# fawnliu/TRIS

Measured on AMD Instinct MI355X. Metric: Stage-1 training images/sec @320px bs48 (TRIS clip-RN50, 3 negatives), higher is better.
Workload: dtype f32 storage/accumulate; products h2 = 2 x f16 pieces; 1 GPU; Stage-1 train step, RefCOCOg-shaped synthetic batch: 48 img/GPU 320x320, 20-token query + 3 negative queries per image, clip-RN50 trunk + frozen aux CLIP ViT-B/32, AdamW (BASELINE.json configs[2]/[3]); per_gpu_batch=48, global_batch=48, size=320, query_len=20, negative_samples=3, parallelism=dp1, sync_bn=False

## Files before the change

### include/tris_hip.h

```cpp
#ifndef TRIS_HIP_H
#define TRIS_HIP_H

#ifdef __cplusplus
extern "C" {
#endif

int tris_gemm_f32(const float* A, const float* B, float* C, int M, int N, int K, long lda, long ldb, long ldc,
                  int transA, int transB, int batch, long strideA, long strideB, long strideC, const float* bias,
                  int bias_mode, const float* resid, long ldr, long strideR, int act, float alpha, float* workspace,
                  long workspace_bytes, void* stream);

int tris_gemm_epilogue_next(float* pre_out, const float* dact_x);

int tris_splitk_tickets_next(int* tickets, int count);
long tris_splitk_fused_launches(void);

int tris_set_gemm_mode(int mode);
int tris_set_gemm_mode_thread(int mode);
int tris_set_option(const char* name, const char* value);
int tris_set_conv_direct_thread(int value);

int tris_set_autotune(int on);
int tris_get_autotune(void);
int tris_get_gemm_mode(void);
// ... 41 lines not shown
int tris_amax_next(unsigned* out);
int tris_h2_next(const unsigned* amaxA, const unsigned* amaxB, float scaleA, float scaleB);
int tris_bn_mask_next(unsigned char* mask);
int tris_h2_planes_f32(const float* x, float* planes_out, long n, const unsigned* word, void* stream);
int tris_h2_planes_segments_f32(const float* base, const long* offs, const long* sizes, const long* slot_index, int nseg,
                                const unsigned* slots, float* out_base, void* stream);
int tris_h2_planes_t_segments_f32(const float* base, const long* offs, const long* rows, const long* cols, const long* slot_index,
                                  int nseg, const unsigned* slots, float* out_base, void* stream);
int tris_h2_unplanes_f32(const float* planes, float* out, long n, const unsigned* word, void* stream);
int tris_h2_next_planes(const unsigned* amaxA, const unsigned* amaxB, int flags);
int tris_bn_apply_pl_f32(const float* X, const float* mean, const float* invstd, const float* gamma, const float* beta,
                         const float* resid, int resid_kind, const unsigned* resid_word, float* Ypl, const unsigned* out_word, long M,
                         int C, int relu, void* stream);
int tris_bn_bwd_reduce_pl_f32(const float* dY, const float* Ypl, const float* X, const float* mean, const float* invstd, long M, int C,
                              float* sum_dz, float* sum_dzx, float* workspace, float* dz_out, void* stream);
int tris_bn_apply_pool_pl_f32(const float* X, const float* mean, const float* invstd, const float* gamma, const float* beta,
                              float* Ypl, const unsigned* out_word, int B, int H, int W, int C, void* stream);
int tris_avgpool2_fwd_pl_f32(const float* Xpl, float* Ypl, const unsigned* word, int B, int H, int W, int C, void* stream);
int tris_bn_bwd_apply_pl_f32(const float* dY, const float* Ypl, const float* X, const float* mean, const float* invstd,
                             const float* gamma, const float* sum_dz, const float* sum_dzx, float inv_count, float* dXpl,
                             const unsigned* out_word, float* dZ, long M, int C, const float* beta_mask, void* stream);
int tris_bn_bwd_apply_pool_pl_f32(const float* dYp, const float* X, const float* mean, const float* invstd, const float* gamma,
                                  const float* beta, const float* sum_dz, const float* sum_dzx, float inv_count, float* dXpl,
                                  const unsigned* out_word, int B, int H, int W, int C, void* stream);
int tris_bn_out_bound2_f32(const float* gamma, const float* beta, int C, float xhat_max, const unsigned* add_word, unsigned* out,
                           void* stream);
int tris_bn_finalize_bound_f32(const double* part, int rows, long M, int C, float eps, float momentum, float* stats,
                               float* running_mean, float* running_var, const float* gamma, const float* beta, float xhat_max,
                               const unsigned* add_word, unsigned* bound_out, void* stream);
int tris_part_finalize_bound_f32(const double* part, int rows, int C, float* out0, float* out1, const float* gamma, const float* invstd,
                                 float inv_count, float xhat_max, const unsigned* dz_word, unsigned* bound_out, void* stream);
int tris_bn_bwd_bound_f32(const float* gamma, const float* invstd, const float* sum_dz, const float* sum_dzx, int C, float inv_count,
                          float xhat_max, const unsigned* dz_word, unsigned* out, void* stream);
int tris_bn_out_bound_f32(const float* gamma, const float* beta, int C, float xhat_max, unsigned* out, void* stream);
int tris_bn_bwd_reduce_f32(const float* dY, const float* Y, const float* X, const float* mean, const float* invstd,
                           long M, int C, float* sum_dz, float* sum_dzx, float* workspace, const float* gamma_mask,
                           const float* beta_mask, float* dz_out, void* stream);
int tris_bn_bwd_apply_f32(const float* dY, const float* Y, const float* X, const float* mean, const float* invstd,
                          const float* gamma, const float* sum_dz, const float* sum_dzx, float inv_count, float* dX,
                          float* dZ, long M, int C, const float* beta_mask, void* stream);
int tris_colsum_f32(const float* X, long M, int N, long ld, float* out, float* workspace, void* stream);

int tris_instnorm_fwd_f32(const float* X, const float* gamma, const float* beta, float* Y, float* mean, float* invstd,
                          int B, int P, int C, float eps, int relu, void* stream);
int tris_instnorm_bwd_f32(const float* dY, const float* Y, const float* X, const float* gamma, const float* mean,
                          const float* invstd, float* dX, float* dgamma_part , float* dbeta_part ,
                          int B, int P, int C, int relu, void* stream);

int tris_layernorm_fwd_f32(const float* X, const float* gamma, const float* beta, float* Y, float* mean, float* rstd,
                           long rows, int W, float eps, void* stream);
long tris_layernorm_bwd_workspace_bytes(long rows, int W);
int tris_layernorm_bwd_f32(const float* dY, const float* X, const float* gamma, const float* mean, const float* rstd,
                           float* dX, float* dgamma, float* dbeta, long rows, int W, float* workspace, const float* extra , void* stream);

int tris_bn_apply_pool_f32(const float* X, const float* mean, const float* invstd, const float* gamma, const float* beta,
                           float* Yp, int B, int H, int W, int C, void* stream);
int tris_bn_bwd_reduce_pool_f32(const float* dYp, const float* X, const float* mean, const float* invstd, int B, int H, int W,
                                int C, float* sum_dz, float* sum_dzx, float* workspace, const float* gamma, const float* beta,
                                void* stream);
int tris_bn_bwd_apply_pool_f32(const float* dYp, const float* X, const float* mean, const float* invstd, const float* gamma,
                               const float* beta, const float* sum_dz, const float* sum_dzx, float inv_count, float* dX, int B,
                               int H, int W, int C, void* stream);
int tris_avgpool2_fwd_f32(const float* X, float* Y, int B, int H, int W, int C, void* stream);
int tris_avgpool2_bwd_f32(const float* dY, float* dX, int B, int H, int W, int C, void* stream);
#define TRIS_EW_ADD 0
#define TRIS_EW_AXPY 1
#define TRIS_EW_RELU_BWD 2
#define TRIS_EW_QGELU 3
#define TRIS_EW_QGELU_BWD 4
#define TRIS_EW_MUL 5
#define TRIS_EW_SCALE 6
#define TRIS_EW_RELU 7
int tris_elementwise_f32(int op, const float* A, const float* B, float* O, long n, float s, void* stream);
int tris_elementwise_bcast_f32(int op, const float* A, const float* B, float* O, long n, long nb, float s, void* stream);
int tris_scale_exp_fwd_f32(const float* X, const float* ls, float* O, float* e_out, long n, void* stream);
long tris_scale_exp_workspace_bytes(void);
int tris_scale_exp_bwd_f32(const float* dO, const float* O, const float* ls, float* dX, float* dls, float* workspace, long n,
                           void* stream);
int tris_nchw_to_nhwc_f32(const float* X, float* Y, int B, int C, int H, int W, void* stream);

int tris_mha_fwd_f32(const float* qkv, float* out, int N, int L, int W, int heads, int causal, void* stream);
int tris_mha_bwd_f32(const float* qkv, const float* dout, float* dqkv, int N, int L, int W, int heads, int causal,
                     void* stream);
int tris_mha_mfma_fwd_f32(const float* qkv, float* out, float* lse, int N, int L, int W, int heads, int causal,
                          void* stream);
int tris_mha_mfma_bwd_f32(const float* qkv, const float* out, const float* dout, const float* lse, float* delta,
                          float* dqkv, int N, int L, int W, int heads, int causal, void* stream);
int tris_mha_h2_fwd_f32(const float* qkv, float* out, float* lse, const unsigned* amax_qkv, int N, int L, int W, int heads,
                        int causal, void* stream);
int tris_mha_h2_bwd_f32(const float* qkv, const float* out, const float* dout, const float* lse, float* delta, float* dqkv,
                        const unsigned* amax_qkv, const unsigned* amax_dout, int N, int L, int W, int heads, int causal,
                        void* stream);
int tris_text_pack_plan_i64(const long* ids, int N, int L, int* plan, void* stream);
int tris_embed_packed_fwd_f32(const long* ids, const float* tok, const float* pos, const int* plan, float* out, int N, int L, int W,
                              void* stream);
int tris_mha_packed_fwd_f32(const float* qkv, float* out, const int* plan, int N, int Lmax, int W, int heads, int causal, void* stream);
int tris_eot_gather_packed_f32(const float* x, const int* plan, float* out, int N, int W, void* stream);
int tris_rows_limit_thread(const int* limit);
int tris_embed_fwd_f32(const long* ids, const float* tok, const float* pos, float* out, int N, int L, int W,
                       void* stream);
int tris_embed_bwd_f32(const long* ids, const float* dout, float* dtok, float* dpos, int N, int L, int W, void* stream);
int tris_embed_rows_bwd_f32(const long* ids, const float* rows, float* dtok, int R, int W, float scale, void* stream);
int tris_concat_i64(const long* a, long na, const long* b, long nb, long* out, void* stream);
int tris_eot_gather_fwd_f32(const long* ids, const float* x, float* out, int N, int L, int W, void* stream);
int tris_eot_gather_bwd_f32(const long* ids, const float* dout, float* dx, int N, int L, int W, void* stream);

int tris_l2norm_fwd_f32(const float* X, float* Y, float* inv_norm, long rows, int C, void* stream);
int tris_l2norm_bwd_f32(const float* dY, const float* Y, const float* inv_norm, float* dX, long rows, int C,
                        void* stream);
int tris_softmax_fwd_f32(const float* X, float* Y, long rows, int n, float scale, void* stream);
int tris_softmax_bwd_f32(const float* dY, const float* Y, float* dX, long rows, int n, float scale, void* stream);
int tris_xattn_fwd_f32(const float* Qv, const float* Kv, const float* Vv, const float* Qt, const float* Kt,
                       const float* Vt, float* new_vis, float* new_lan, float* probs, int B, int P, int N, int C,
                       void* stream);
#define TRIS_DECLINED (-2)
long tris_xattn_fused_ws_bytes(int B, int N, int C);
long tris_xattn_fused_sync_words(int B);
int tris_xattn_fused_fwd_f32(const float* Qv, const float* Kv, const float* Vv, const float* Qt, const float* Kt,
                             const float* Vt, float* new_vis, float* new_lan, float* probs, int B, int P, int N, int C,
                             float* ws, long ws_bytes, unsigned* sync, void* stream);
long tris_xattn_px_ws_bytes(int B, int N, int C);
long tris_xattn_px_sync_words(int B);
long tris_xattn_px_bwd_ws_bytes(int B, int N, int C);
int tris_xattn_px_bwd_f32(const float* d_vis, const float* d_lan, const float* Vv, const float* Qt, const float* Kt,
                          const float* Vt, const float* probs, float* dQv, float* dKv, float* dVv, float* dS, int B, int P,
                          int N, int C, float* ws, long ws_bytes, unsigned* sync, unsigned* amax_dQv, unsigned* amax_dKv,
                          unsigned* amax_dVv, void* stream);
long tris_xattn_px_last_form(void);
int tris_xattn_amax_next(const unsigned* qv, const unsigned* kv, const unsigned* vv, const unsigned* qt, const unsigned* kt,
                         const unsigned* vt);
long tris_xattn_px_slots(int B, int P, int C, int cus);
int tris_xattn_px_fwd_f32(const float* Qv, const float* Kv, const float* Vv, const float* Qt, const float* Kt,
                          const float* Vt, float* new_vis, float* new_lan, float* probs, int B, int P, int N, int C,
                          float* ws, long ws_bytes, unsigned* sync, void* stream);
int tris_softmax_col_bwd_f32(const float* dY, const float* Y, float* dX, int B, int P, int N, float scale,
                             void* stream);
int tris_cls_head_fwd_f32(const float* score, float* cls_out, float* cls_fg, int B, int P, int N, float focal_p,
                          float focal_c, void* stream);
int tris_cls_head_bwd_f32(const float* score, const float* g_cls_out, float* dscore, int B, int P, int N, float focal_p,
                          float focal_c, void* stream);
int tris_maps_fwd_f32(const float* score, float* relu_map, float* sig_map, int B, int h, int w, int N, int S,
                      void* stream);
int tris_maps_bwd_f32(const float* score, const float* d_relu, const float* d_sig, float* dscore, int B, int h, int w,
                      int N, int S, void* stream);
int tris_resize_bilinear_fwd_f32(const float* X, float* Y, int planes, int Hi, int Wi, int Ho, int Wo,
// ... 120 lines not shown
```

### tris_amd/CLIP/clip/model.py

```python
from collections import OrderedDict


import numpy as np
import torch
from torch import nn

from ... import ops
from ...config import cfg


class Conv2d(nn.Module):

    def __init__(self, cin, cout, k, stride=1, bias=False):
        super().__init__()
        self.cin, self.cout, self.k, self.stride = cin, cout, k, stride
        w = torch.empty(cout, cin, k, k).contiguous(memory_format=torch.channels_last)
        nn.init.kaiming_uniform_(w, a=5 ** 0.5)
        self.weight = nn.Parameter(w)
        self.bias = nn.Parameter(torch.zeros(cout)) if bias else None

    def forward(self, x, stats=False, grad_box=None, grad_box_out=None):
        if self.k == 1:
            return ops.linear(x, self.weight, self.bias, stats=stats and self.bias is None, grad_box=grad_box,
                              grad_box_out=grad_box_out)
# ... 171 lines not shown
                hooks[stage]()
        return tuple(outs)

    def forward(self, x):
        outs = [ops.unplanes(o).permute(0, 3, 1, 2) for o in self.forward_cl(x)]
        outs.append(None)
        return tuple(outs)


class LayerNorm(nn.Module):
    def __init__(self, w, eps=1e-5):
        super().__init__()
        self.eps = eps
        self.weight = nn.Parameter(torch.ones(w))
        self.bias = nn.Parameter(torch.zeros(w))

    def forward(self, x, grad_box=None):
        return ops.layer_norm(x, self.weight, self.bias, self.eps, grad_box)


class QuickGELU(nn.Module):
    def forward(self, x):
        return ops.quick_gelu(x)


class MultiheadAttention(nn.Module):

    def __init__(self, d_model, n_head):
        super().__init__()
        self.embed_dim, self.num_heads = d_model, n_head
        self.in_proj_weight = nn.Parameter(torch.empty(3 * d_model, d_model))
        self.in_proj_bias = nn.Parameter(torch.zeros(3 * d_model))
        self.out_proj = Linear(d_model, d_model)
        nn.init.xavier_uniform_(self.in_proj_weight)


class ResidualAttentionBlock(nn.Module):
    def __init__(self, d_model, n_head, attn_mask=None):
        super().__init__()
        self.attn = MultiheadAttention(d_model, n_head)
        self.ln_1 = LayerNorm(d_model)
        self.mlp = nn.Sequential(OrderedDict([
            ("c_fc", Linear(d_model, d_model * 4)),
            ("gelu", QuickGELU()),
            ("c_proj", Linear(d_model * 4, d_model)),
        ]))
        self.ln_2 = LayerNorm(d_model)
        self.causal = attn_mask is not None

    def forward(self, x):
        use_box = torch.is_grad_enabled() and x.requires_grad and cfg.grad_box
        b1 = ops.GradBox() if use_box else None
        b2 = ops.GradBox() if use_box else None
        h = self.ln_1(x, b1)
        qkv = ops.linear(h, self.attn.in_proj_weight, self.attn.in_proj_bias)
        a = ops.mha(qkv, self.attn.num_heads, self.causal)
        x = self.attn.out_proj(a, resid=x, grad_box_res=b1)
        h = self.ln_2(x, b2)
        if torch.is_grad_enabled() and cfg.mlp_fuse:
            f = ops.linear_qgelu(h, self.mlp.c_fc.weight, self.mlp.c_fc.bias)
            return ops.linear(f, self.mlp.c_proj.weight, self.mlp.c_proj.bias, x, 0, grad_box_res=b2, act_link=True)
        if torch.is_grad_enabled():
            return self.mlp.c_proj(self.mlp.gelu(self.mlp.c_fc(h)), resid=x, grad_box_res=b2)
        f = self.mlp.c_fc(h, act=2)
        return self.mlp.c_proj(f, resid=x, grad_box_res=b2)


    def forward_packed(self, x, plan, N, L):
        h = self.ln_1(x)
        qkv = ops.linear(h, self.attn.in_proj_weight, self.attn.in_proj_bias)
        a = ops.mha_packed(qkv, plan, N, L, self.attn.num_heads, self.causal)
        x = self.attn.out_proj(a, resid=x)
        h = self.ln_2(x)
        return self.mlp.c_proj(self.mlp.c_fc(h, act=2), resid=x)

    def forward_token0(self, x):
        h = self.ln_1(x)
        qkv = ops.linear(h, self.attn.in_proj_weight, self.attn.in_proj_bias)
        a = ops.token0(ops.mha(qkv, self.attn.num_heads, self.causal))
        x0 = self.attn.out_proj(a, resid=ops.token0(x))
        h = self.ln_2(x0)
        if torch.is_grad_enabled() and cfg.mlp_fuse:
            f = ops.linear_qgelu(h, self.mlp.c_fc.weight, self.mlp.c_fc.bias)
            return ops.linear(f, self.mlp.c_proj.weight, self.mlp.c_proj.bias, x0, 0, act_link=True)
        if torch.is_grad_enabled():
            return self.mlp.c_proj(self.mlp.gelu(self.mlp.c_fc(h)), resid=x0)
        return self.mlp.c_proj(self.mlp.c_fc(h, act=2), resid=x0)


class Transformer(nn.Module):
    def __init__(self, width, layers, heads, attn_mask=None):
        super().__init__()
        self.width, self.layers = width, layers
        self.resblocks = nn.Sequential(*[ResidualAttentionBlock(width, heads, attn_mask) for _ in range(layers)])

    def forward(self, x):
        for blk in self.resblocks:
            x = ops.cut(blk(x))
        return x

    def forward_token0(self, x):
        blocks = list(self.resblocks)
        for blk in blocks[:-1]:
            x = ops.cut(blk(x))
        return blocks[-1].forward_token0(x)


class VisionTransformer(nn.Module):
    def __init__(self, input_resolution, patch_size, width, layers, heads, output_dim):
        super().__init__()
        self.input_resolution, self.output_dim, self.patch_size = input_resolution, output_dim, patch_size
        self.conv1 = nn.Module()
        self.conv1.weight = nn.Parameter(torch.randn(width, 3, patch_size, patch_size) * 0.02)
        scale = width ** -0.5
        self.class_embedding = nn.Parameter(scale * torch.randn(width))
        self.positional_embedding = nn.Parameter(scale * torch.randn((input_resolution // patch_size) ** 2 + 1, width))
        self.ln_pre = LayerNorm(width)
        self.transformer = Transformer(width, layers, heads)
        for blk in self.transformer.resblocks:
            for w in (blk.attn.in_proj_weight, blk.attn.out_proj.weight, blk.mlp.c_fc.weight, blk.mlp.c_proj.weight):
                w._tris_linear_w = True
        self.ln_post = LayerNorm(width)
        self.proj = nn.Parameter(scale * torch.randn(width, output_dim))
        self.spacial_dim = 7
        self.class_embedding._tris_accumulates = True
        self.positional_embedding._tris_accumulates = True

    def forward_patches(self, patches):
        emb = ops.linear(patches, self.conv1.weight)
        x = ops.vit_assemble(emb, self.class_embedding, self.positional_embedding)
        x = self.ln_pre(x)
        if cfg.vit_token0:
            cls = self.ln_post(self.transformer.forward_token0(x))
        else:
# ... 166 lines not shown
```

### tris_amd/_lib.py

```python
import ctypes
import os
import re

import torch

_HERE = os.path.dirname(os.path.abspath(__file__))
_ROOT = os.path.dirname(_HERE)
HEADER = os.path.join(_ROOT, "include", "tris_hip.h")
LIBPATH = os.environ.get("TRIS_HIP_LIB") or os.path.join(_HERE, "libtris_hip.so")

_CT = {
    "int": ctypes.c_int,
    "long": ctypes.c_long,
    "float": ctypes.c_float,
}


def parse_header(path=HEADER):
    src = open(path).read()
    consts = {m.group(1): int(m.group(2)) for m in re.finditer(r"#define\s+(TRIS_\w+)\s+(\d+)", src)}
    src = re.sub(r"/\*.*?\*/", " ", src, flags=re.S)
    decls = {}
    for m in re.finditer(r"\b(int|long)\s+(tris_\w+)\s*\(([^)]*)\)\s*;", src):
        ret, name, args = m.group(1), m.group(2), m.group(3)
        types = []
        for a in args.split(","):
            a = a.strip()
            if a in ("", "void"):
                continue
            if "*" in a:
                types.append(ctypes.c_void_p)
            else:
                base = a.split()[0] if a.split()[0] != "const" else a.split()[1]
                types.append(_CT[base])
        decls[name] = (_CT[ret], types)
    return decls, consts


DECLS, CONSTS = parse_header()
_lib = None


class TrisHipError(RuntimeError):
    pass


def load():
    global _lib
    if _lib is None:
        if not os.path.exists(LIBPATH):
            raise TrisHipError(
                f"{LIBPATH} not found: build it with `python -c 'import __graft_entry__ as g; g.build()'` "
                "(tris_amd has no CPU or eager fallback by design)")
        lib = ctypes.CDLL(LIBPATH)
        for name, (ret, args) in DECLS.items():
            fn = getattr(lib, name)
            fn.restype = ret
            fn.argtypes = args
        _lib = lib
    return _lib


_FN = {}


def call(name, *args):
    fn = _FN.get(name)
    if fn is None:
        fn = _FN[name] = getattr(load(), name)
    err = fn(*args)
    if err != 0:
        raise TrisHipError(f"{name} failed with hipError_t {err}")


def query(name, *args):
    return getattr(load(), name)(*args)
```

### tris_amd/config.py

```python
import contextlib
import os


def _flag(name, default):
    v = os.environ.get(name)
    return default if v is None or v == "" else v != "0"


class _Config:
    def __setattr__(self, name, value):
        if name == "step_graph" and "step_graph" in self.__dict__:
            self.__dict__["step_graph_chosen"] = True
        self.__dict__[name] = value

    def __init__(self):
        e = os.environ.get
        self.step_graph = e("TRIS_STEP_GRAPH", "0")
        self.step_graph_chosen = "TRIS_STEP_GRAPH" in os.environ
        self.hipgraph = _flag("TRIS_HIPGRAPH", True)
        self.text_stream = _flag("TRIS_TEXT_STREAM", True)
        self.wgrad_stream = _flag("TRIS_WGRAD_STREAM", True)
        self.stream_probe = _flag("TRIS_STREAM_PROBE", True)
        self.stream_probe_log = e("TRIS_STREAM_PROBE_LOG") == "1"
        self.text_at = e("TRIS_TEXT_AT", "layer4")
        self.bn_bwd_fuse = _flag("TRIS_BN_BWD_FUSE", True)
        self.bn_pool = _flag("TRIS_BN_POOL", True)
        self.grad_box = _flag("TRIS_GRAD_BOX", True)
        self.mlp_fuse = _flag("TRIS_MLP_FUSE", True)
        self.mha = e("TRIS_MHA", "auto")
        self.mha_h2 = _flag("TRIS_MHA_H2", True)
        self.ddp_seg_opt = _flag("TRIS_DDP_SEG_OPT", True)
        self.ddp_seg_poison = _flag("TRIS_DDP_SEG_POISON", False)
        self.syncbn_bound = _flag("TRIS_SYNCBN_BOUND", True)
        self.xattn_fused = _flag("TRIS_XATTN_FUSED", True)
        self.xattn_px = _flag("TRIS_XATTN_PX", True)
        self.xattn_h2 = _flag("TRIS_XATTN_H2", True)
        self.xattn_bwd_px = _flag("TRIS_XATTN_BWD_PX", True)
        self.hbm_loader = _flag("TRIS_HBM_LOADER", True)
        self.eval_group = max(1, int(e("TRIS_EVAL_GROUP", "16")))
        self.mbox_spin = int(e("TRIS_MBOX_SPIN", "40000000"))
        self.syncbn_comm = e("TRIS_SYNCBN_COMM", "mailbox")
        self.ddp_check = e("TRIS_DDP_CHECK") == "1"
        self.ddp_sparse_embed = _flag("TRIS_DDP_SPARSE_EMBED", True)
        self.random_init = e("TRIS_RANDOM_INIT") == "1"
        self.h2_planes = _flag("TRIS_H2_PLANES", True)
        self.own_stream = _flag("TRIS_OWN_STREAM", True)
        self.fuse_splitk = _flag("TRIS_FUSE_SPLITK_PY", False)
        self.aux_text_early = _flag("TRIS_AUX_TEXT_EARLY", True)
        self.text_pack = _flag("TRIS_TEXT_PACK", True)
        self.bn_bitmask = _flag("TRIS_BN_BITMASK", True)
        self.gemm_convert = int(e("TRIS_GEMM_CONVERT", "0"))
        self.step_graph_rerecord = int(e("TRIS_STEP_GRAPH_RERECORD", "3"))
        self.side_param_grads = _flag("TRIS_SIDE_PARAM_GRADS", True)
        self.vit_token0 = _flag("TRIS_VIT_TOKEN0", True)

    @contextlib.contextmanager
    def override(self, **kw):
        old = {k: getattr(self, k) for k in kw}
        try:
            for k, v in kw.items():
                setattr(self, k, v)
            yield self
        finally:
            for k, v in old.items():
                setattr(self, k, v)

    def key(self):
        return tuple(sorted((k, v) for k, v in self.__dict__.items() if k not in ("step_graph_chosen", "step_graph_rerecord")))


cfg = _Config()
```

### tris_amd/csrc/attn_h2.hip

```cpp
#include "common.h"
#include "tris_hip.h"
#include "x3_split.h"

namespace {

#include "amax.h"

constexpr int HD = 64;
constexpr int RS = 144;
constexpr int PLB = 64 * RS;
constexpr float PS = 8192.f;

typedef float f4v __attribute__((ext_vector_type(4)));
typedef short s16x4 __attribute__((ext_vector_type(4)));
typedef short s16x8 __attribute__((ext_vector_type(8)));
typedef unsigned u32x4v __attribute__((ext_vector_type(4)));

struct H8 { f16x8 hi, lo; };

__device__ __forceinline__ float4 ldg4(const float* p) { return *reinterpret_cast<const float4*>(p); }
__device__ __forceinline__ H8 split8(const float4 u, const float4 w, const float s) {
  const Split4 p = split4h(u, s), q = split4h(w, s);
  H8 o;
  o.hi = __builtin_bit_cast(f16x8, (u32x4v){p.hi.x, p.hi.y, q.hi.x, q.hi.y});
// ... 92 lines not shown
            const int key = key0 + 8 * kg + i;
            const float v = (sc[i >> 2][i & 3] + sx[i >> 2][i & 3] * (1.0f / 2048.0f)) * inv_s;
            sv[i] = (full || (key < L && !(causal && key > q0 + r))) ? v : -INFINITY;
            mx = fmaxf(mx, sv[i]);
          }
          mx = fmaxf(mx, __shfl_xor(mx, 16, 64));
          mx = fmaxf(mx, __shfl_xor(mx, 32, 64));
          const float mn = fmaxf(m, mx);
          float p[8], rs = 0.f;
#pragma unroll
          for (int i = 0; i < 8; ++i) { p[i] = mn == -INFINITY ? 0.f : __expf(sv[i] - mn); rs += p[i]; }
          rs += __shfl_xor(rs, 16, 64);
          rs += __shfl_xor(rs, 32, 64);
          const float alpha = mn == -INFINITY ? 1.f : __expf(m - mn);
          l = l * alpha + rs;
          m = mn;
          if (__builtin_amdgcn_ballot_w64(alpha != 1.f) != 0ull) {
#pragma unroll
            for (int t = 0; t < 4; ++t) {
              const float ar = __shfl(alpha, 4 * kg + t, 64);
#pragma unroll
              for (int j = 0; j < 4; ++j) { oc[j][t] *= ar; ox[j][t] *= ar; }
            }
          }
          const H8 pf = split8(make_float4(p[0], p[1], p[2], p[3]), make_float4(p[4], p[5], p[6], p[7]), PS);
#pragma unroll
          for (int ct = 0; ct < 4; ++ct) mm3(pf, bfrag(Vp, 32 * pr, ct, r, kg), oc[ct], ox[ct]);
        }
      }
    }
  }
  unsigned am = 0u;
  if (q0 < L) {
    const float linv = 1.f / l;
    float* ob = out + (long)n * L * W + h * HD;
#pragma unroll
    for (int t = 0; t < 4; ++t) {
      const float li = __shfl(linv, 4 * kg + t, 64) * inv_o;
      const int q = q0 + 4 * kg + t;
      if (q < L) {
#pragma unroll
        for (int j = 0; j < 4; ++j) {
          const float o = (oc[j][t] + ox[j][t] * (1.0f / 2048.0f)) * li;
          ob[(long)q * W + 16 * j + r] = o;
          am = max(am, __builtin_bit_cast(unsigned, o) & 0x7fffffffu);
        }
      }
    }
    if (kg == 0 && q0 + r < L) lse[((long)n * H + h) * L + q0 + r] = m + __logf(l);
  }
  if (amax != nullptr) amax_commit(am, amax);
}

__global__ __launch_bounds__(256) void mha_h2_dq_kernel(const float* __restrict__ qkv, const float* __restrict__ out,
                                                        const float* __restrict__ dout, const float* __restrict__ lse,
                                                        float* __restrict__ delta, float* __restrict__ dqkv, int L, int W, int causal,
                                                        float scale, const unsigned* __restrict__ am_qkv,
                                                        const unsigned* __restrict__ am_do, unsigned* __restrict__ amax) {
  __shared__ __attribute__((aligned(16))) char Kp[2 * PLB];
  __shared__ __attribute__((aligned(16))) char Vp[2 * PLB];
  const int tid = threadIdx.x, lane = tid & 63, wave = tid >> 6, r = lane & 15, kg = lane >> 4;
  const int h = blockIdx.y, n = blockIdx.z, H = gridDim.y;
  const int qb = blockIdx.x * 64, q0 = qb + wave * 16;
  const float s = h2_scale_from_bits(h2_amax_of(am_qkv, lane)), sg = h2_scale_from_bits(h2_amax_of(am_do, lane));
  const float inv_s = scale / (s * s), inv_p = 1.0f / (s * sg);
  const float* base = qkv + (long)n * L * 3 * W + h * HD;
  const int qrow = min(q0 + r, L - 1);
  H8 qf[2], gf[2];
  resident(qf, base + (long)qrow * 3 * W + 8 * kg, s);
  float dl = 0.f;
  {
    const float* gp = dout + ((long)n * L + qrow) * W + h * HD + 8 * kg;
    const float* op = out + ((long)n * L + qrow) * W + h * HD + 8 * kg;
#pragma unroll
    for (int ks = 0; ks < 2; ++ks) {
      const float4 g0 = ldg4(gp + 32 * ks), g1 = ldg4(gp + 32 * ks + 4), o0 = ldg4(op + 32 * ks), o1 = ldg4(op + 32 * ks + 4);
      gf[ks] = split8(g0, g1, sg);
      dl += g0.x * o0.x + g0.y * o0.y + g0.z * o0.z + g0.w * o0.w + g1.x * o1.x + g1.y * o1.y + g1.z * o1.z + g1.w * o1.w;
    }
    dl += __shfl_xor(dl, 16, 64);
    dl += __shfl_xor(dl, 32, 64);
    if (kg == 0 && q0 + r < L) delta[((long)n * H + h) * L + q0 + r] = dl;
  }
  const float ls = lse[((long)n * H + h) * L + qrow];
  f4v acc[4];
#pragma unroll
  for (int j = 0; j < 4; ++j) acc[j] = (f4v){0.f, 0.f, 0.f, 0.f};
  const int kend = causal ? min(L, qb + 64) : L;
  for (int kb = 0; kb < kend; kb += 64) {
    __syncthreads();
    stage64(Kp, base + W, 3L * W, kb, L, tid, s);
    stage64(Vp, base + 2 * W, 3L * W, kb, L, tid, s);
    __syncthreads();
    if (q0 < L) {
#pragma unroll
      for (int pr = 0; pr < 2; ++pr) {
        const int key0 = kb + 32 * pr;
        if (key0 < kend && !(causal && key0 > q0 + 15)) {
          f4v sc[2], sx[2], pc[2], px[2];
#pragma unroll
          for (int j = 0; j < 2; ++j) {
            sc[j] = sx[j] = pc[j] = px[j] = (f4v){0.f, 0.f, 0.f, 0.f};
            const int row = 32 * pr + trow(r, j);
#pragma unroll
            for (int ks = 0; ks < 2; ++ks) {
              mm3(afrag(Kp, row, ks, kg), qf[ks], sc[j], sx[j]);
              mm3(afrag(Vp, row, ks, kg), gf[ks], pc[j], px[j]);
            }
          }
          float ds[8], mx = 0.f;
          const bool full = key0 + 32 <= L && !(causal && key0 + 31 > q0);
#pragma unroll
          for (int i = 0; i < 8; ++i) {
            const int key = key0 + 8 * kg + i;
            const bool ok = full || (key < L && !(causal && key > q0 + r));
            const float sv = (sc[i >> 2][i & 3] + sx[i >> 2][i & 3] * (1.0f / 2048.0f)) * inv_s;
            const float dp = (pc[i >> 2][i & 3] + px[i >> 2][i & 3] * (1.0f / 2048.0f)) * inv_p;
            ds[i] = ok ? __expf(sv - ls) * (dp - dl) * scale : 0.f;
            mx = fmaxf(mx, fabsf(ds[i]));
          }
          const float sd = wave_scale_of(mx);
          const H8 df = split8(make_float4(ds[0], ds[1], ds[2], ds[3]), make_float4(ds[4], ds[5], ds[6], ds[7]), sd);
          const float inv_d = 1.0f / (sd * s);
#pragma unroll
          for (int ct = 0; ct < 4; ++ct) {
            f4v tc = {0.f, 0.f, 0.f, 0.f}, tx = {0.f, 0.f, 0.f, 0.f};
            mm3(df, bfrag(Kp, 32 * pr, ct, r, kg), tc, tx);
            acc[ct] += join(tc, tx) * inv_d;
          }
        }
      }
    }
  }
  unsigned am = 0u;
  if (q0 < L) {
    float* ob = dqkv + (long)n * L * 3 * W + h * HD;
#pragma unroll
    for (int t = 0; t < 4; ++t) {
      const int q = q0 + 4 * kg + t;
      if (q < L) {
#pragma unroll
        for (int j = 0; j < 4; ++j) {
          ob[(long)q * 3 * W + 16 * j + r] = acc[j][t];
          am = max(am, __builtin_bit_cast(unsigned, acc[j][t]) & 0x7fffffffu);
        }
      }
    }
  }
  if (amax != nullptr) amax_commit(am, amax);
}

__global__ __launch_bounds__(256) void mha_h2_dkv_kernel(const float* __restrict__ qkv, const float* __restrict__ dout,
                                                         const float* __restrict__ lse, const float* __restrict__ delta,
                                                         float* __restrict__ dqkv, int L, int W, int causal, float scale,
                                                         const unsigned* __restrict__ am_qkv, const unsigned* __restrict__ am_do,
                                                         unsigned* __restrict__ amax) {
  __shared__ __attribute__((aligned(16))) char Qp[2 * PLB];
  __shared__ __attribute__((aligned(16))) char Gp[2 * PLB];
  __shared__ float Ls[64], Ds[64];
  const int tid = threadIdx.x, lane = tid & 63, wave = tid >> 6, r = lane & 15, kg = lane >> 4;
  const int h = blockIdx.y, n = blockIdx.z, H = gridDim.y;
  const int kb0 = blockIdx.x * 64, k0 = kb0 + wave * 16;
  const float s = h2_scale_from_bits(h2_amax_of(am_qkv, lane)), sg = h2_scale_from_bits(h2_amax_of(am_do, lane));
  const float inv_s = scale / (s * s), inv_p = 1.0f / (s * sg), inv_v = 1.0f / (PS * sg);
  const float* base = qkv + (long)n * L * 3 * W + h * HD;
  const int krow = min(k0 + r, L - 1);
  H8 kf[2], vf[2];
  resident(kf, base + W + (long)krow * 3 * W + 8 * kg, s);
  resident(vf, base + 2 * W + (long)krow * 3 * W + 8 * kg, s);
  f4v dk[4], vc[4], vx[4];
#pragma unroll
  for (int j = 0; j < 4; ++j) dk[j] = vc[j] = vx[j] = (f4v){0.f, 0.f, 0.f, 0.f};
  const int qstart = causal ? kb0 : 0;
  for (int qb = qstart; qb < L; qb += 64) {
    __syncthreads();
    stage64(Qp, base, 3L * W, qb, L, tid, s);
    stage64(Gp, dout + (long)n * L * W + h * HD, (long)W, qb, L, tid, sg);
    if (tid < 64) {
      const int q = min(qb + tid, L - 1);
      Ls[tid] = lse[((long)n * H + h) * L + q];
      Ds[tid] = delta[((long)n * H + h) * L + q];
    }
    __syncthreads();
    if (k0 < L) {
#pragma unroll
      for (int pr = 0; pr < 2; ++pr) {
        const int qs0 = qb + 32 * pr;
        if (qs0 < L && !(causal && qs0 + 31 < k0)) {
          f4v sc[2], sx[2], pc[2], px[2];
#pragma unroll
          for (int j = 0; j < 2; ++j) {
            sc[j] = sx[j] = pc[j] = px[j] = (f4v){0.f, 0.f, 0.f, 0.f};
            const int row = 32 * pr + trow(r, j);
#pragma unroll
            for (int ks = 0; ks < 2; ++ks) {
              mm3(afrag(Qp, row, ks, kg), kf[ks], sc[j], sx[j]);
              mm3(afrag(Gp, row, ks, kg), vf[ks], pc[j], px[j]);
            }
          }
          float p[8], ds[8], mx = 0.f;
          const bool full = qs0 + 32 <= L && !(causal && k0 + 15 > qs0);
#pragma unroll
          for (int i = 0; i < 8; ++i) {
            const int ql = 32 * pr + 8 * kg + i, q = qb + ql;
            const bool ok = full || (q < L && !(causal && k0 + r > q));
            const float sv = (sc[i >> 2][i & 3] + sx[i >> 2][i & 3] * (1.0f / 2048.0f)) * inv_s;
            const float dp = (pc[i >> 2][i & 3] + px[i >> 2][i & 3] * (1.0f / 2048.0f)) * inv_p;
            p[i] = ok ? __expf(sv - Ls[ql]) : 0.f;
            ds[i] = p[i] * (dp - Ds[ql]) * scale;
            mx = fmaxf(mx, fabsf(ds[i]));
          }
          const float sd = wave_scale_of(mx);
          const H8 pf = split8(make_float4(p[0], p[1], p[2], p[3]), make_float4(p[4], p[5], p[6], p[7]), PS);
          const H8 df = split8(make_float4(ds[0], ds[1], ds[2], ds[3]), make_float4(ds[4], ds[5], ds[6], ds[7]), sd);
          const float inv_d = 1.0f / (sd * s);
#pragma unroll
          for (int ct = 0; ct < 4; ++ct) {
            mm3(pf, bfrag(Gp, 32 * pr, ct, r, kg), vc[ct], vx[ct]);
            f4v tc = {0.f, 0.f, 0.f, 0.f}, tx = {0.f, 0.f, 0.f, 0.f};
            mm3(df, bfrag(Qp, 32 * pr, ct, r, kg), tc, tx);
            dk[ct] += join(tc, tx) * inv_d;
          }
        }
      }
    }
  }
  unsigned am = 0u;
  if (k0 < L) {
    float* ob = dqkv + (long)n * L * 3 * W + h * HD;
#pragma unroll
    for (int t = 0; t < 4; ++t) {
      const int k = k0 + 4 * kg + t;
      if (k < L) {
#pragma unroll
        for (int j = 0; j < 4; ++j) {
          const float dv = (vc[j][t] + vx[j][t] * (1.0f / 2048.0f)) * inv_v;
          ob[(long)k * 3 * W + W + 16 * j + r] = dk[j][t];
          ob[(long)k * 3 * W + 2 * W + 16 * j + r] = dv;
          am = max(am, max(__builtin_bit_cast(unsigned, dk[j][t]) & 0x7fffffffu, __builtin_bit_cast(unsigned, dv) & 0x7fffffffu));
        }
      }
    }
  }
  if (amax != nullptr) amax_commit(am, amax);
}

}

extern "C" __attribute__((visibility("hidden"))) unsigned* tris_internal_take_amax_next();

extern "C" int tris_mha_h2_fwd_f32(const float* qkv, float* out, float* lse, const unsigned* amax_qkv, int N, int L, int W, int heads,
                                   int causal, void* stream) {
  if (W != heads * HD || L < 1 || N < 1 || (((uintptr_t)qkv) & 15) || amax_qkv == nullptr) return (int)hipErrorInvalidValue;
  hipLaunchKernelGGL(mha_h2_fwd_kernel, dim3(cdiv(L, 64), heads, N), dim3(256), 0, (hipStream_t)stream, qkv, out, lse, L, W, causal,
                     1.0f / sqrtf((float)HD), amax_qkv, tris_internal_take_amax_next());
  TRIS_LAUNCH_CHECK();
  return 0;
}

extern "C" int tris_mha_h2_bwd_f32(const float* qkv, const float* out, const float* dout, const float* lse, float* delta, float* dqkv,
                                   const unsigned* amax_qkv, const unsigned* amax_dout, int N, int L, int W, int heads, int causal,
                                   void* stream) {
  if (W != heads * HD || L < 1 || N < 1 || amax_qkv == nullptr || amax_dout == nullptr || (((uintptr_t)qkv) & 15) ||
      (((uintptr_t)dout) & 15) || (((uintptr_t)out) & 15))
    return (int)hipErrorInvalidValue;
  const float scale = 1.0f / sqrtf((float)HD);
  const dim3 grid(cdiv(L, 64), heads, N);
  unsigned* amax = tris_internal_take_amax_next();
  hipLaunchKernelGGL(mha_h2_dq_kernel, grid, dim3(256), 0, (hipStream_t)stream, qkv, out, dout, lse, delta, dqkv, L, W, causal, scale,
                     amax_qkv, amax_dout, amax);
  TRIS_LAUNCH_CHECK();
  hipLaunchKernelGGL(mha_h2_dkv_kernel, grid, dim3(256), 0, (hipStream_t)stream, qkv, dout, lse, delta, dqkv, L, W, causal, scale,
                     amax_qkv, amax_dout, amax);
  TRIS_LAUNCH_CHECK();
  return 0;
}
```

### tris_amd/csrc/conv_direct.hip

```cpp
#include <algorithm>
#include <cstdlib>
#include <cstring>

#include "common.h"
#include "tris_hip.h"

namespace {

#include "gemm_params.h"
#include "gemm_fast.h"
#include "conv_direct_cfg.h"

__global__ __launch_bounds__(256) void stem_conv1_kernel(const float* __restrict__ X, const float* __restrict__ Wt,
                                                         float* __restrict__ Y, double* __restrict__ stat_part, int Bn, int H,
                                                         int W, int Cin, int Cout, int Ho, int Wo, int stride, int tiles_per_wave) {
  __shared__ double red[4][2][32];
  const int lane = threadIdx.x & 63, wave = threadIdx.x >> 6;
  const int mn = lane & 31, kh = lane >> 5;
  const int K = 9 * Cin;
  const long total = (long)Bn * Ho * Wo;
  float wreg[14];
  int ky[14], kx[14], kc[14];
#pragma unroll
  for (int s = 0; s < 14; ++s) {
    const int k = 2 * s + kh;
    const int tap = k / Cin;
    wreg[s] = (k < K && mn < Cout) ? Wt[mn * K + k] : 0.f;
    ky[s] = k < K ? tap / 3 : -100000;
    kx[s] = tap - (tap / 3) * 3;
    kc[s] = k - tap * Cin;
  }
  double s1 = 0.0, s2 = 0.0;
  const long tile0 = ((long)blockIdx.x * 4 + wave) * tiles_per_wave;
  for (int t = 0; t < tiles_per_wave; ++t) {
    const long p0 = (tile0 + t) * 32;
    if (p0 >= total) break;
    const long p = min(p0 + mn, total - 1);
    const int b = (int)(p / ((long)Ho * Wo));
    const int r = (int)(p - (long)b * Ho * Wo);
    const int oy = r / Wo, ox = r - oy * Wo;
    const int iy0 = oy * stride - 1, ix0 = ox * stride - 1;
    float a[14];
#pragma unroll
    for (int s = 0; s < 14; ++s) {
      const int iy = iy0 + ky[s], ix = ix0 + kx[s];
      const bool inb = (unsigned)iy < (unsigned)H && (unsigned)ix < (unsigned)W;
      a[s] = inb ? X[(((long)b * H + iy) * W + ix) * Cin + kc[s]] : 0.f;
    }
    f32x16 acc;
#pragma unroll
    for (int q = 0; q < 16; ++q) acc[q] = 0.f;
#pragma unroll
    for (int s = 0; s < 14; ++s) acc = __builtin_amdgcn_mfma_f32_32x32x2f32(a[s], wreg[s], acc, 0, 0, 0);
#pragma unroll
    for (int q = 0; q < 16; ++q) {
      const long pix = p0 + (q & 3) + 8 * (q >> 2) + 4 * kh;
      if (pix < total && mn < Cout) {
        const float v = acc[q];
// ... 345 lines not shown
```

### tris_amd/csrc/gemm_conv.hip

```cpp
#include <algorithm>
#include <cstdlib>
#include <cstring>
#include <map>
#include <mutex>
#include <tuple>

#include "common.h"
#include "tris_hip.h"

extern "C" {
extern __attribute__((visibility("hidden"))) int tris_internal_stream_form;
extern __attribute__((visibility("hidden"))) int tris_internal_col_blocks;
extern __attribute__((visibility("hidden"))) int tris_internal_ln_bwd_blocks;
extern __attribute__((visibility("hidden"))) int tris_internal_fin_block;
__attribute__((visibility("hidden"))) int tris_internal_reduce_wide = 4;
__attribute__((visibility("hidden"))) int tris_internal_xcd_order = -1;
__attribute__((visibility("hidden"))) int tris_internal_red_grid = 0;
__attribute__((visibility("hidden"))) int tris_internal_fuse_splitk = 16;
__attribute__((visibility("hidden"))) long tris_internal_fused_count = 0;
extern __attribute__((visibility("hidden"))) int tris_internal_xattn_px_slots;
}

namespace {

#include "gemm_params.h"

static int stream_nt(const GemmParams& p, int batch) {
  if (!tris_internal_stream_form) return 0;
  const long streams = 1 + (p.resid ? 1 : 0) + (p.bnb_x ? 1 : 0) + (p.bnb_y ? 1 : 0);
  return (long)p.M * p.N * 4 * batch * streams > ((long)tris_internal_stream_form << 20) ? 1 : 0;
}

struct Options {
  int force_tile = 0;
  int force_pipe = -1;
  int pipe_default = -1;
  int conv_direct = -1;
  int wgrad_direct = -1;
  int bn_fold = 1;
  int stem_conv1 = 1;
  int wg_blocks = 256;
  char tune_log[256] = {0};
};
static int parse_tile(const char* e) {
  return !e ? 0 : (!strcmp(e, "128x128") ? 1 : !strcmp(e, "128x64") ? 2 : !strcmp(e, "64x64") ? 3 : !strcmp(e, "128x32") ? 4
                   : !strcmp(e, "256x128") ? 5 : 0);
}
static bool set_option(Options& o, const char* name, const char* v) {
  const bool unset = (v == nullptr || v[0] == 0);
  if (!strcmp(name, "FORCE_TILE")) o.force_tile = parse_tile(v);
  else if (!strcmp(name, "FORCE_PIPE")) o.force_pipe = unset ? -1 : std::min(5, std::max(0, atoi(v)));
  else if (!strcmp(name, "PIPE")) o.pipe_default = unset ? -1 : (v[0] == '0' ? 0 : 1);
  else if (!strcmp(name, "CONV_DIRECT")) o.conv_direct = unset ? -1 : atoi(v);
  else if (!strcmp(name, "WGRAD_DIRECT")) o.wgrad_direct = unset ? -1 : atoi(v);
  else if (!strcmp(name, "BN_FOLD")) o.bn_fold = unset ? 1 : (v[0] != '0');
  else if (!strcmp(name, "STEM_CONV1")) o.stem_conv1 = unset ? 1 : (v[0] != '0');
  else if (!strcmp(name, "WG_BLOCKS")) o.wg_blocks = unset ? 256 : std::max(1, atoi(v));
  else if (!strcmp(name, "STREAM_FORM")) tris_internal_stream_form = unset ? 256 : (atoi(v) == 1 ? 256 : std::max(0, atoi(v)));
  else if (!strcmp(name, "COL_BLOCKS")) tris_internal_col_blocks = unset ? 512 : std::max(1, atoi(v));
  else if (!strcmp(name, "LN_BWD_BLOCKS")) tris_internal_ln_bwd_blocks = unset ? 512 : std::min(512, std::max(1, atoi(v)));
  else if (!strcmp(name, "FIN_BLOCK")) tris_internal_fin_block = unset ? 256 : (atoi(v) >= 1024 ? 1024 : atoi(v) >= 512 ? 512 : 256);
  else if (!strcmp(name, "REDUCE_WIDE")) tris_internal_reduce_wide = unset ? 4 : std::max(0, atoi(v));
  else if (!strcmp(name, "RED_GRID")) tris_internal_red_grid = unset ? 0 : std::max(0, atoi(v));
  else if (!strcmp(name, "XCD_ORDER")) tris_internal_xcd_order = unset ? -1 : std::min(2, std::max(0, atoi(v)));
  else if (!strcmp(name, "FUSE_SPLITK")) tris_internal_fuse_splitk = unset ? TRIS_FUSE_SPLITK_DEFAULT : std::max(0, atoi(v));
  else if (!strcmp(name, "XATTN_PX_SLOTS")) tris_internal_xattn_px_slots = unset ? 0 : std::max(0, atoi(v));
  else if (!strcmp(name, "TUNE_LOG")) { strncpy(o.tune_log, unset ? "" : v, sizeof(o.tune_log) - 1); o.tune_log[sizeof(o.tune_log) - 1] = 0; }
  else return false;
  return true;
}
static Options init_options() {
  Options o;
  for (const char* n : {"FORCE_TILE", "FORCE_PIPE", "PIPE", "CONV_DIRECT", "WGRAD_DIRECT", "BN_FOLD", "STEM_CONV1", "WG_BLOCKS", "STREAM_FORM", "COL_BLOCKS", "XATTN_PX_SLOTS", "LN_BWD_BLOCKS", "FIN_BLOCK", "REDUCE_WIDE", "XCD_ORDER", "FUSE_SPLITK", "RED_GRID", "TUNE_LOG"}) {
    char env[64];
    snprintf(env, sizeof(env), "TRIS_%s", n);
    if (const char* v = getenv(env)) set_option(o, n, v);
  }
  return o;
}
static Options g_opt = init_options();

static int g_mode_default = 1;
static thread_local int g_mode_thread = -1;
#define g_gemm_mode (g_mode_thread >= 0 ? g_mode_thread : g_mode_default)
static inline bool mode_h2() { return g_gemm_mode == 3 || g_gemm_mode == 4; }

}
extern "C" __attribute__((visibility("hidden"))) unsigned* tris_internal_take_amax_next();
#define TRIS_RUN_DECL(AK_, BK_)                                                                                                   \
  extern "C" __attribute__((visibility("hidden"))) int tris_internal_run_cfg_##AK_##BK_(const void* params, int batch, float* ws, \
                                                                                         void* stream, const void* cfg, int mode);
TRIS_RUN_DECL(0, 0) TRIS_RUN_DECL(0, 1) TRIS_RUN_DECL(1, 0) TRIS_RUN_DECL(1, 1) TRIS_RUN_DECL(2, 0) TRIS_RUN_DECL(2, 2) TRIS_RUN_DECL(1, 3)
#undef TRIS_RUN_DECL
namespace {
template <int AK, int BKIND>
int run_cfg(const GemmParams& p0, int batch, float* ws, hipStream_t st, const Cfg& cfg) {
  const int mode = g_gemm_mode;
  GemmParams p = p0;
  p.nt = stream_nt(p, batch);
  if (AK == A_ROWK && BKIND == B_NK) return tris_internal_run_cfg_00(&p, batch, ws, st, &cfg, mode);
  if (AK == A_ROWK && BKIND == B_KN) return tris_internal_run_cfg_01(&p, batch, ws, st, &cfg, mode);
  if (AK == A_COLK && BKIND == B_NK) return tris_internal_run_cfg_10(&p, batch, ws, st, &cfg, mode);
  if (AK == A_COLK && BKIND == B_KN) return tris_internal_run_cfg_11(&p, batch, ws, st, &cfg, mode);
  if (AK == A_IM2COL && BKIND == B_NK) return tris_internal_run_cfg_20(&p, batch, ws, st, &cfg, mode);
  if (AK == A_IM2COL && BKIND == B_KN_DGRAD) return tris_internal_run_cfg_22(&p, batch, ws, st, &cfg, mode);
  if (AK == A_COLK && BKIND == B_KN_IM2COL) return tris_internal_run_cfg_13(&p, batch, ws, st, &cfg, mode);
  return (int)hipErrorInvalidValue;
}

struct H2Next { const unsigned* a; const unsigned* b; float sa, sb; bool armed; bool planes; int flags; };
static thread_local H2Next g_h2_next = {nullptr, nullptr, 0.f, 0.f, false, false, 0};
static H2Next h2_take() {
  H2Next n = g_h2_next;
  g_h2_next.armed = false;
  return n;
}
struct H2Guard {
  int saved;
  bool on;
  bool bad;
  H2Guard(GemmParams& p, const H2Next& n) : saved(g_mode_thread), on(false), bad(false) {
    if (!n.armed) return;
    if (!gemm_fast_ok(p)) { bad = n.planes; return; }
    p.h2_amaxA = n.a; p.h2_amaxB = n.b; p.h2_sA = n.sa; p.h2_sB = n.sb;
    g_mode_thread = n.planes ? 4 : 3;
    p.bnb_y_pl = (n.planes && (n.flags & 4)) ? 2 : (n.planes && (n.flags & 1)) ? 1 : 0;
// ... 6 lines not shown
static int default_pipe(const GemmParams& p, int bm, int bn, int splitk) {
  if (!pipe_ok(p) || bn == 32) return 0;
  if (g_opt.force_pipe >= 0) return g_opt.force_pipe;
  if (g_opt.pipe_default >= 0) return g_opt.pipe_default;
  if (mode_h2()) return 0;
  return p.gC >= 128 ? 1 : 0;
}

static Cfg heuristic_cfg(const GemmParams& p, int batch, const float* ws, long ws_bytes) {
  const bool can_split = (batch == 1 && ws != nullptr && p.K >= 512);
  int bm = 64, bn = 64, splitk = 1;
  if (p.stat_part != nullptr) {
    bm = 128;
    bn = p.N <= 32 ? 32 : p.N <= 64 ? 64 : 128;
  } else if (can_split && p.K >= 4096) {
    if (p.N <= 64) { bn = 64; bm = p.M >= 128 ? 128 : 64; }
    else if (p.M >= 128 && p.N >= 128) { bm = bn = 128; }
    const long tiles = (long)cdiv(p.M, bm) * cdiv(p.N, bn);
    splitk = (int)min((long)cdiv(512, tiles), (long)(p.K / 256));
    const long per = (long)p.M * p.N * (long)sizeof(float);
    if ((long)splitk * per > ws_bytes) splitk = (int)(ws_bytes / per);
    if (splitk < 2) splitk = 1;
  } else {
    static const int cand[4][2] = {{128, 128}, {128, 64}, {64, 64}, {128, 32}};
    static const double pen[4] = {1.0, 1.08, 1.2, 1.15};
    const bool fastk = gemm_fast_ok(p);
    double best = 1e30;
    for (int c = 0; c < 4; ++c) {
      const int cbm = cand[c][0], cbn = cand[c][1];
      if (c != 2 && p.M < 96) continue;
      if (c == 0 && p.N <= 64) continue;
      if (c == 3 && !(p.N <= 32 && fastk)) continue;
      const long tiles = (long)cdiv(p.M, cbm) * cdiv(p.N, cbn) * batch;
      const double per_k32 = (cbm / 64) * (cbn / 64.0) * (g_gemm_mode == 1 ? 384.0 + 250.0 : mode_h2() ? 192.0 + 200.0 : 1024.0) * pen[c];
      const int smax = can_split ? (int)min((long)64, (long)(p.K / 256)) : 1;
      for (int sk = 1; sk <= smax; sk = (sk < 4 ? sk + 1 : sk + sk / 2)) {
        if (sk > 1 && (long)sk * p.M * p.N * (long)sizeof(float) > ws_bytes) break;
        const double ksteps = (double)cdiv(cdiv(p.K, sk), 32);
        const double blocks = (double)tiles * sk;
        double t = (ksteps * per_k32 + 3000.0) * (blocks <= 256.0 ? 1.0 : blocks / 256.0);
        if (sk > 1) t += 14000.0 + 2.0 * sk * (double)p.M * p.N * 4.0 / 2000.0;
        if (t < best) { best = t; bm = cbm; bn = cbn; splitk = sk; }
      }
    }
  }
  {
    const int forced = g_opt.force_tile;
    if (forced == 1 && p.N > 64) { bm = 128; bn = 128; }
    if (forced == 2) { bm = 128; bn = 64; }
    if (forced == 3) { bm = 64; bn = 64; }
    if (forced == 4 && p.N <= 32) { bm = 128; bn = 32; }
    if (forced == 5 && p.N > 64 && p.M >= 256 && p.stat_part == nullptr) { bm = 256; bn = 128; }
  }
  Cfg c = {bm, bn, splitk, default_pipe(p, bm, bn, splitk)};
  return c;
}

struct TuneKey {
  int ak, bk, M, N, K, batch, mode;
  bool operator<(const TuneKey& o) const {
    return std::tie(ak, bk, M, N, K, batch, mode) < std::tie(o.ak, o.bk, o.M, o.N, o.K, o.batch, o.mode);
  }
};
static std::map<TuneKey, Cfg> g_tuned;
static std::mutex g_tune_mu;

static int g_autotune = -1;
static bool autotune_enabled() {
  if (g_autotune < 0) { const char* e = getenv("TRIS_AUTOTUNE"); g_autotune = (e && e[0] == '0') ? 0 : 1; }
  return g_autotune == 1;
}

template <int AK, int BKIND>
int launch_cfg(GemmParams& p, int batch, float* ws, long ws_bytes, hipStream_t st) {
  Cfg h = heuristic_cfg(p, batch, ws, ws_bytes);
  if (!autotune_enabled() || g_opt.force_tile) return run_cfg<AK, BKIND>(p, batch, ws, st, h);
  const bool stat = p.stat_part != nullptr;
  const TuneKey key = {AK, BKIND + (stat ? 16 : 0) + (p.bnb_x != nullptr ? 32 : 0), p.M, p.N, p.K, batch, g_gemm_mode};
  {
    std::lock_guard<std::mutex> lk(g_tune_mu);
    auto it = g_tuned.find(key);
    if (it != g_tuned.end()) return run_cfg<AK, BKIND>(p, batch, ws, st, it->second);
  }
  hipStreamCaptureStatus cap = hipStreamCaptureStatusNone;
  if (hipStreamIsCapturing(st, &cap) != hipSuccess || cap != hipStreamCaptureStatusNone)
    return run_cfg<AK, BKIND>(p, batch, ws, st, h);
  static const int tiles[5][2] = {{128, 128}, {128, 64}, {64, 64}, {128, 32}, {256, 128}};
  const bool fastk = gemm_fast_ok(p);
  static const int sks[] = {1, 2, 3, 4, 6, 8, 12, 16, 24, 32, 48, 64, 96, 128};
  const bool can_split = (batch == 1 && ws != nullptr && p.K >= 512) && !stat;
  const bool can_pipe = pipe_ok(p) && g_opt.force_pipe != 0;
  hipEvent_t e0, e1;
  if (hipEventCreate(&e0) != hipSuccess || hipEventCreate(&e1) != hipSuccess) return run_cfg<AK, BKIND>(p, batch, ws, st, h);
  (void)hipDeviceSynchronize();
  Cfg best = h;
  float best_ms = 1e30f;
  auto time_cfg = [&](Cfg c) -> float {
    float ms_min = 1e30f;
    for (int rep = 0; rep < 2; ++rep) {
      (void)hipEventRecord(e0, st);
      if (run_cfg<AK, BKIND>(p, batch, ws, st, c) != 0) return 1e30f;
      (void)hipEventRecord(e1, st);
      if (hipEventSynchronize(e1) != hipSuccess) return 1e30f;
      float ms = 1e30f;
      (void)hipEventElapsedTime(&ms, e0, e1);
      ms_min = ms < ms_min ? ms : ms_min;
    }
    return ms_min;
  };
  for (int t = 0; t < 5; ++t) {
    const int cbm = tiles[t][0], cbn = tiles[t][1];
    if (t != 2 && p.M < 96) continue;
    if ((t == 0 || t == 4) && p.N <= 64) continue;
    if (t == 3 && !(p.N <= 32 && fastk)) continue;
    if (t == 4 && (!can_pipe || p.M < 256)) continue;
    if (stat && cbm != 128) continue;
    const long ntiles = (long)cdiv(p.M, cbm) * cdiv(p.N, cbn) * batch;
    for (int sk : sks) {
      if (sk > 1 && (!can_split || sk > p.K / 256 || (long)sk * p.M * p.N * (long)sizeof(float) > ws_bytes)) break;
      if (sk > 1 && ntiles * sk > 1536) break;
      if (sk * 8 < h.splitk && ntiles * sk < 256) continue;
      for (int pipe = (can_pipe && t != 3) ? 1 : 0; pipe >= (t == 4 || g_opt.force_pipe == 1 ? (can_pipe && t != 3 ? 1 : 0) : 0); --pipe) {
        const Cfg c = {cbm, cbn, sk, pipe};
        const float ms = time_cfg(c);
        if (ms < best_ms) { best_ms = ms; best = c; }
      }
      if (g_gemm_mode == 4 && AK == A_ROWK && BKIND == B_NK && t != 3 && fastk && g_opt.force_pipe < 0) {
        for (int gp : {2, 3, 4, 5}) {
          if ((gp == 3 || gp == 5) && t != 0) continue;
          const Cfg c = {cbm, cbn, sk, gp};
          const float ms = time_cfg(c);
          if (ms < best_ms) { best_ms = ms; best = c; }
        }
      }
    }
  }
  (void)hipEventDestroy(e0);
  (void)hipEventDestroy(e1);
  {
    std::lock_guard<std::mutex> lk(g_tune_mu);
    g_tuned[key] = best;
    if (g_opt.tune_log[0]) {
      if (FILE* f = fopen(g_opt.tune_log, "a")) {
        fprintf(f, "ak=%d bkind=%d M=%d N=%d K=%d batch=%d mode=%d -> %dx%d sk=%d pipe=%d  %.1f us  %.1f TFLOP/s\n", AK, key.bk,
                p.M, p.N, p.K, batch, g_gemm_mode, best.bm, best.bn, best.splitk, best.pipe, best_ms * 1e3f,
                2.0 * p.M * p.N * p.K * batch / (best_ms * 1e-3) * 1e-12);
        fclose(f);
      }
    }
  }
  return run_cfg<AK, BKIND>(p, batch, ws, st, best);
}





static long g_direct_launches[2] = {0, 0};
static thread_local int g_conv_direct_thread = -1;
#include "conv_direct_cfg.h"

}
#define TRIS_DIRECT_DECL(P_)                                                                                                          \
  extern "C" __attribute__((visibility("hidden"))) int tris_internal_run_halo_p##P_(const void* params, int id, int dgrad, void* stream); \
  extern "C" __attribute__((visibility("hidden"))) int tris_internal_run_wgrad_direct_p##P_(                                            \
      int id, const float* X, const float* dY, float* dW, int B, int H, int W, int Ci, int Co, float* ws, long ws_bytes, int blocks,    \
      void* stream, const float* mean, const float* invstd, const float* gamma, const float* beta, const unsigned* amax_dy,            \
      const unsigned* amax_x);
TRIS_DIRECT_DECL(1) TRIS_DIRECT_DECL(3) TRIS_DIRECT_DECL(4)
#undef TRIS_DIRECT_DECL
extern "C" __attribute__((visibility("hidden"))) int tris_internal_stem_conv1(const float* X, const float* Wt, float* Y, int B, int H, int W,
    int Cin, int Cout, int stride, double* stat_part, void* stream);
namespace {
template <int BKIND>
int run_halo(const GemmParams& p0, int id, hipStream_t st) {
  const int dg = BKIND == B_KN_DGRAD ? 1 : 0;
  GemmParams p = p0;
  p.nt = stream_nt(p, 1);
  const int rc = g_gemm_mode == 4 ? tris_internal_run_halo_p4(&p, id, dg, st)
                 : g_gemm_mode == 3 ? tris_internal_run_halo_p3(&p, id, dg, st) : tris_internal_run_halo_p1(&p, id, dg, st);
  if (rc == 0) ++g_direct_launches[0];
  return rc;
}
static int run_wgrad_direct(int id, const float* X, const float* dY, float* dW, int B, int H, int W, int Ci, int Co, float* ws,
                            long ws_bytes, hipStream_t st, BnIn bn = BnIn{nullptr, nullptr, nullptr, nullptr},
                            const unsigned* amax_dy = nullptr, const unsigned* amax_x = nullptr) {
  const int rc = g_gemm_mode == 4 ? tris_internal_run_wgrad_direct_p4(id, X, dY, dW, B, H, W, Ci, Co, ws, ws_bytes, g_opt.wg_blocks, st,
                                                                      nullptr, nullptr, nullptr, nullptr, amax_dy, amax_x)
                 : g_gemm_mode == 3 ? tris_internal_run_wgrad_direct_p3(id, X, dY, dW, B, H, W, Ci, Co, ws, ws_bytes, g_opt.wg_blocks, st,
                                                                      bn.mean, bn.invstd, bn.gamma, bn.beta, amax_dy, amax_x)
                                  : tris_internal_run_wgrad_direct_p1(id, X, dY, dW, B, H, W, Ci, Co, ws, ws_bytes, g_opt.wg_blocks, st,
                                                                      bn.mean, bn.invstd, bn.gamma, bn.beta, nullptr, nullptr);
  if (rc == 0) ++g_direct_launches[1];
  return rc;
}
static int run_stem_conv1(const float* X, const float* Wt, float* Y, int B, int H, int W, int Cin, int Cout, int stride,
                          double* stat_part, hipStream_t st) {
  if (!g_opt.stem_conv1) return 0;
  return tris_internal_stem_conv1(X, Wt, Y, B, H, W, Cin, Cout, stride, stat_part, st);
}

static bool halo_shape_ok(const GemmParams& p) {
  return (g_gemm_mode == 1 || mode_h2()) && p.gStride == 1 && p.gC % 16 == 0 && p.fastB && al16(p.A) && al16(p.B) && p.N % 4 == 0 &&
         p.gHo == p.gH && p.gWo == p.gW && (long)p.gB * p.gH * p.gW * p.gC < (1L << 31);
// ... 52 lines not shown
      if (hipEventSynchronize(e1) != hipSuccess) return 1e30f;
      float ms = 1e30f;
      (void)hipEventElapsedTime(&ms, e0, e1);
      best = ms < best ? ms : best;
    }
    return best;
  };
  int best_id = 0;
  const float t_im2col = timed(0);
  float best_ms = t_im2col;
  for (int id = 1; id < kHaloN; ++id) {
    if (!halo_ok(p, id)) continue;
    const float ms = timed(id);
    if (ms < best_ms) { best_ms = ms; best_id = id; }
  }
  (void)hipEventDestroy(e0);
  (void)hipEventDestroy(e1);
  {
    std::lock_guard<std::mutex> lk(g_tune_mu);
    g_tuned[key] = Cfg{best_id, 0, 1, 0};
    if (g_opt.tune_log[0]) {
      if (FILE* f = fopen(g_opt.tune_log, "a")) {
        fprintf(f, "conv3x3 bkind=%d M=%d N=%d K=%d HxW=%dx%d -> %s %d  %.1f us  %.1f TFLOP/s  (implicit GEMM %.1f us) mode=%d\n", key.bk,
                p.M, p.N, p.K, p.gH, p.gW, best_id ? "direct" : "implicit", best_id, best_ms * 1e3f,
                2.0 * p.M * p.N * p.K / (best_ms * 1e-3) * 1e-12, t_im2col * 1e3f, g_gemm_mode);
        fclose(f);
      }
    }
  }
  return best_id ? direct(best_id) : im2col();
}


}

static bool stats_eligible(const GemmParams& p) { return gemm_fast_ok(p) && p.M >= 128; }

struct EpiNext { float* pre; const float* dact; bool armed; };
static thread_local EpiNext g_epi_next = {nullptr, nullptr, false};
extern "C" __attribute__((visibility("hidden"))) const int* tris_internal_rows_limit();
extern "C" int tris_gemm_epilogue_next(float* pre_out, const float* dact_x) {
  g_epi_next = {pre_out, dact_x, pre_out != nullptr || dact_x != nullptr};
  return 0;
}

struct TicketsNext { int* t; int n; };
static thread_local TicketsNext g_tickets_next = {nullptr, 0};
extern "C" long tris_splitk_fused_launches(void) { return __atomic_load_n(&tris_internal_fused_count, __ATOMIC_RELAXED); }
extern "C" int tris_splitk_tickets_next(int* tickets, int count) {
  g_tickets_next = {count > 0 ? tickets : nullptr, count > 0 ? count : 0};
  return 0;
}

extern "C" int tris_gemm_f32(const float* A, const float* B, float* C, int M, int N, int K, long lda, long ldb,
                             long ldc, int transA, int transB, int batch, long sA, long sB, long sC,
                             const float* bias, int bias_mode, const float* resid, long ldr, long sR, int act,
                             float alpha, float* workspace, long ws_bytes, void* stream) {
  const H2Next h2n = h2_take();
  unsigned* amax_out = tris_internal_take_amax_next();
  const EpiNext epi = g_epi_next;
  g_epi_next.armed = false;
  const TicketsNext tkn = g_tickets_next;
  g_tickets_next = {nullptr, 0};
  if (M <= 0 || N <= 0 || batch <= 0) return 0;
  if (K <= 0) return (int)hipErrorInvalidValue;
  GemmParams p = {};
  p.amax_out = amax_out;
  p.tickets = tkn.t;
  p.tickets_n = tkn.n;
  if (!transA && batch == 1) p.m_limit = tris_internal_rows_limit();
  if (epi.armed) { p.pre_out = epi.pre; p.dact_x = epi.dact; }
  p.A = A; p.B = B; p.C = C; p.M = M; p.N = N; p.K = K;
  p.lda = lda; p.ldb = ldb; p.ldc = ldc; p.sA = sA; p.sB = sB; p.sC = sC;
  p.bias = bias; p.bias_mode = bias ? bias_mode : 0;
  p.resid = resid; p.ldr = ldr; p.sR = sR; p.act = act; p.alpha = alpha;
  p.vecA = al16(A) && (lda % 4 == 0) && (sA % 4 == 0);
  p.vecB = al16(B) && (ldb % 4 == 0) && (sB % 4 == 0);
  p.fastA = p.vecA && (!transA || M % 4 == 0);
  p.fastB = p.vecB && (transB || N % 4 == 0);
  if (transA && !transB && K % 32 != 0 && K > 32 && p.fastA && p.fastB && M >= 4 && N >= 4 && !epi.armed) {
    p.Kv = K;
    p.K = (K + 31) & ~31;
  }
  hipStream_t st = (hipStream_t)stream;
  if (epi.armed) {
    if (batch != 1 || transA || !gemm_fast_ok(p)) return TRIS_DECLINED;
    workspace = nullptr;
    ws_bytes = 0;
  }
  H2Guard h2(p, h2n);
  if (h2.bad) return (int)hipErrorInvalidValue;
  if (!transA && transB) return launch_cfg<A_ROWK, B_NK>(p, batch, workspace, ws_bytes, st);
  if (!transA && !transB) return launch_cfg<A_ROWK, B_KN>(p, batch, workspace, ws_bytes, st);
  if (transA && !transB) return launch_cfg<A_COLK, B_KN>(p, batch, workspace, ws_bytes, st);
  return launch_cfg<A_COLK, B_NK>(p, batch, workspace, ws_bytes, st);
}

extern "C" int tris_conv3x3_fwd_f32(const float* X, const float* Wt, float* Y, int B, int H, int W, int Cin, int Cout,
                                    int stride, void* stream) {
  const H2Next h2n = h2_take();
  int Ho = (H + 2 - 3) / stride + 1, Wo = (W + 2 - 3) / stride + 1;
  GemmParams p = {};
  p.A = X; p.B = Wt; p.C = Y;
  p.M = B * Ho * Wo; p.N = Cout; p.K = 9 * Cin;
  p.ldb = 9L * Cin; p.ldc = Cout; p.alpha = 1.f;
  p.gH = H; p.gW = W; p.gC = Cin; p.gHo = Ho; p.gWo = Wo; p.gStride = stride; p.gB = B;
  p.vecA = al16(X) && (Cin % 16 == 0);
  p.vecB = al16(Wt) && ((9 * Cin) % 4 == 0);
  p.fastA = al16(X) && (Cin % 32 == 0);
  p.fastB = p.vecB;
  if (const int rows = run_stem_conv1(X, Wt, Y, B, H, W, Cin, Cout, stride, nullptr, (hipStream_t)stream))
    return rows > 0 ? 0 : (int)hipErrorLaunchFailure;
  H2Guard h2(p, h2n);
  if (h2.bad) return (int)hipErrorInvalidValue;
  return conv3_dispatch<B_NK>(p, (hipStream_t)stream, nullptr);
}

extern "C" int tris_conv3x3_dgrad_f32(const float* dY, const float* Wt, float* dX, int B, int H, int W, int Cin,
                                      int Cout, void* stream) {
  const H2Next h2n = h2_take();
  GemmParams p = {};
  p.A = dY; p.B = Wt; p.C = dX;
  p.M = B * H * W; p.N = Cin; p.K = 9 * Cout;
  p.ldc = Cin; p.alpha = 1.f;
  p.gH = H; p.gW = W; p.gC = Cout; p.gHo = H; p.gWo = W; p.gStride = 1; p.gB = B;
  p.wCin = Cin; p.wCout = Cout;
  p.vecA = al16(dY) && (Cout % 16 == 0);
  p.vecB = al16(Wt) && (Cin % 4 == 0);
  p.fastA = al16(dY) && (Cout % 32 == 0);
  p.fastB = p.vecB;
  if (Cout % 16 != 0) return (int)hipErrorInvalidValue;
  H2Guard h2(p, h2n);
  if (h2.bad) return (int)hipErrorInvalidValue;
  return conv3_dispatch<B_KN_DGRAD>(p, (hipStream_t)stream, nullptr);
}

extern "C" int tris_conv3x3_dgrad_bnbwd_f32(const float* dY, const float* Wt, float* dZ, int B, int H, int W, int Cin, int Cout,
                                            const float* bn_x, const float* mean, const float* invstd, const float* gamma,
                                            const float* beta, double* part, int* part_rows, void* stream) {
  const H2Next h2n = h2_take();
  unsigned* amax_out = tris_internal_take_amax_next();
  *part_rows = 0;
  if (bn_x == nullptr || part == nullptr || gamma == nullptr || beta == nullptr) return (int)hipErrorInvalidValue;
  GemmParams p = {};
// ... 382 lines not shown
```

### tris_amd/csrc/gemm_core.h

```cpp
#pragma once
#include <algorithm>
#include <cstdlib>
#include <cstring>

#include "common.h"
#include "tris_hip.h"

namespace {

#include "gemm_params.h"
#include "amax.h"

constexpr int BK = 16;
constexpr int PAD = 4;

template <int BM, int BN, int AK, int BKIND, int EPI>
__global__ __launch_bounds__(256) void gemm_kernel(GemmParams p) {
  constexpr int WM = BM / 2, WN = BN / 2;
  constexpr int FM = WM / 32, FN = WN / 32;
  constexpr int PA = BM / 64, PB = BN / 64;
  __shared__ float As[BK][BM + PAD];
  __shared__ float Bs[BK][BN + PAD];

  const int tid = threadIdx.x;
  const int lane = tid & 63, wave = tid >> 6;
  const int wm = wave >> 1, wn = wave & 1;
  const int tile = blockIdx.x;
  const int m0 = (tile / p.tiles_n) * BM;
  const int n0 = (tile % p.tiles_n) * BN;
  if (p.m_limit != nullptr && m0 >= *p.m_limit) return;
  const int zb = blockIdx.z / p.splitk;
  const int zs = blockIdx.z % p.splitk;
  const int kbeg = zs * p.kchunk;
  const int kend = min(p.K, kbeg + p.kchunk);

  const float* __restrict__ A = p.A + (long)zb * p.sA;
  const float* __restrict__ Bp = p.B + (long)zb * p.sB;

  int a_b[PA], a_iy0[PA], a_ix0[PA];
  bool a_ok[PA];
  if (AK == A_IM2COL) {
#pragma unroll
    for (int q = 0; q < PA; ++q) {
      int m = m0 + (tid >> 2) + q * 64;
      a_ok[q] = m < p.M;
      int mm = a_ok[q] ? m : 0;
      int hw = p.gHo * p.gWo;
      a_b[q] = mm / hw;
      int r = mm - a_b[q] * hw;
      int oy = r / p.gWo, ox = r - oy * p.gWo;
      a_iy0[q] = oy * p.gStride - 1;
      a_ix0[q] = ox * p.gStride - 1;
    }
  }
  int bj_tap = 0, bj_ci = 0;
  if (BKIND == B_KN_IM2COL) {
    constexpr int F4 = BN / 4;
    int j = n0 + (tid % F4) * 4;
    bj_tap = j / p.gC;
// ... 468 lines not shown
    }                                                            \
  } while (0)
#define TRIS_GLDS_GO(BM_, BN_, NW_, NWM_)                                                                                          \
  do {                                                                                                                           \
    if (splitk > 1) {                                                                                                            \
      p.C = ws;                                                                                                                  \
      hipLaunchKernelGGL((gemm_fast_kernel<BM_, BN_, AK, BKIND, EPI_SLAB, 4, NW_, 32, 4, NWM_>), grid, dim3(NW_ * 64), 0, st, p); \
    } else {                                                                                                                     \
      hipLaunchKernelGGL((gemm_fast_kernel<BM_, BN_, AK, BKIND, EPI_STD, 4, NW_, 32, 4, NWM_>), grid, dim3(NW_ * 64), 0, st, p);  \
    }                                                                                                                            \
  } while (0)
  bool launched = false;
  if constexpr (AK == A_ROWK && BKIND == B_NK) {
    if (glds) {
      launched = true;
      if (bm == 256 && bn == 128) TRIS_GLDS_GO(256, 128, 8, 4);
      else if (bm == 128 && bn == 128 && gform == 3) TRIS_GLDS_GO(128, 128, 4, 2);
      else if (bm == 128 && bn == 128) TRIS_GLDS_GO(128, 128, 8, 2);
      else if (bm == 128 && bn == 64) TRIS_GLDS_GO(128, 64, 4, 2);
      else TRIS_GLDS_GO(64, 64, 4, 2);
    }
  }
#undef TRIS_GLDS_GO
  if (launched) {
  } else
  if (pipe) {
    if (bm == 256 && bn == 128) TRIS_PIPE_GO(256, 128, 8, 4);
    else if (bm == 128 && bn == 128) TRIS_PIPE_GO(128, 128, 8, 2);
    else if (bm == 128 && bn == 64) TRIS_PIPE_GO(128, 64, 4, 2);
    else TRIS_PIPE_GO(64, 64, 4, 2);
  } else if (bm == 128 && bn == 128) TRIS_GO(128, 128, true);
  else if (bm == 128 && bn == 64) TRIS_GO(128, 64, true);
  else if (bm == 128 && bn == 32) TRIS_GO(128, 32, false);
  else TRIS_GO(64, 64, true);
#undef TRIS_GO
#undef TRIS_PIPE_GO
#undef TRIS_PIPE_ONE
#undef TRIS_FAST_EPI
#undef TRIS_FAST
#undef TRIS_NW
  TRIS_LAUNCH_CHECK();
  if (splitk > 1 && !fuse) {
    p.C = Cfinal;
    long total = (long)p.M * p.N;
    if ((p.N & 3) == 0 && al16(ws) && al16(p.C) && splitk >= 8 && total / 4 < 128 * 256 && tris_internal_reduce_wide)
    {
      if (tris_internal_reduce_wide >= 16)
        hipLaunchKernelGGL(splitk_reduce_wide_kernel<16>, dim3(cdiv(total / 4, 64)), dim3(1024), 0, st, ws, splitk, p);
      else if (tris_internal_reduce_wide >= 8)
        hipLaunchKernelGGL(splitk_reduce_wide_kernel<8>, dim3(cdiv(total / 4, 64)), dim3(512), 0, st, ws, splitk, p);
      else
        hipLaunchKernelGGL(splitk_reduce_wide_kernel<4>, dim3(cdiv(total / 4, 64)), dim3(256), 0, st, ws, splitk, p);
    }
    else if ((p.N & 3) == 0 && al16(ws) && al16(p.C))
      hipLaunchKernelGGL(splitk_reduce_kernel<4>, dim3(red_blocks(cdiv(total / 4, 256))), dim3(256), 0, st, ws, splitk, p);
    else
      hipLaunchKernelGGL(splitk_reduce_kernel<1>, dim3(red_blocks(cdiv(total, 256))), dim3(256), 0, st, ws, splitk, p);
    TRIS_LAUNCH_CHECK();
  }
  return 0;
}

}
```

### tris_amd/csrc/gemm_params.h

```cpp
#pragma once

enum { A_ROWK = 0, A_COLK = 1, A_IM2COL = 2, A_HALO = 3 };
enum { B_NK = 0, B_KN = 1, B_KN_DGRAD = 2, B_KN_IM2COL = 3 };
enum { EPI_STD = 0, EPI_SLAB = 1, EPI_XTRA = 2 };

struct GemmParams {
  const float* A;
  const float* B;
  float* C;
  int M, N, K;
  int Kv;
  long lda, ldb, ldc;
  long sA, sB, sC;
  const float* bias;
  int bias_mode;
  const float* resid;
  long ldr, sR;
  int act;
  float alpha;
  int vecA, vecB;
  int fastA, fastB;
  int vecC;
  double* stat_part;
  int kchunk, splitk;
  int tiles_n;
  int gH, gW, gC, gHo, gWo, gStride;
  int xcd_remap;
  int gB;
  int wCin, wCout;
  int hmode;
  const float *in_mean, *in_invstd, *in_gamma, *in_beta;
  const float *bnb_x, *bnb_y, *bnb_mean, *bnb_invstd, *bnb_gamma, *bnb_beta;
  int bnb_y_pl;
  const unsigned *h2_amaxA, *h2_amaxB;
  float h2_sA, h2_sB;
  unsigned* amax_out;
  float* pre_out;
  const float* dact_x;
  int nt;
  const int* m_limit;
  int* tickets;
  int tickets_n;
  float* Cfin;
  int vecCfin;
  int fin_groups;
};
#define TRIS_FUSE_SPLITK_MAX 16
#define TRIS_FUSE_SPLITK_DEFAULT 16

__device__ __forceinline__ float4 ld4(const float* p) { return *reinterpret_cast<const float4*>(p); }
typedef float gp_f32x4 __attribute__((ext_vector_type(4)));
__device__ __forceinline__ float4 ld4s(const float* p, bool nt) {
  if (nt) { const gp_f32x4 v = __builtin_nontemporal_load(reinterpret_cast<const gp_f32x4*>(p)); return make_float4(v.x, v.y, v.z, v.w); }
  return ld4(p);
}
__device__ __forceinline__ void st4s(float* p, float4 v, bool nt) {
  if (nt) { const gp_f32x4 w = {v.x, v.y, v.z, v.w}; __builtin_nontemporal_store(w, reinterpret_cast<gp_f32x4*>(p)); }
  else *reinterpret_cast<float4*>(p) = v;
}
inline bool al16(const void* p) { return (((uintptr_t)p) & 15) == 0; }

__device__ __forceinline__ float qgelu_grad(float b) {
  const float sg = 1.0f / (1.0f + expf(-1.702f * b));
  return sg + 1.702f * b * sg * (1.f - sg);
}
struct Cfg { int bm, bn, splitk, pipe; };
inline bool gemm_fast_ok(const GemmParams& p) { return p.fastA && p.fastB && (p.K % 32 == 0) && p.M >= 4 && p.N >= 4; }
```

### tris_amd/csrc/norm.hip

```cpp
#include <cstdlib>

#include "common.h"
#include "tris_hip.h"

extern "C" {
__attribute__((visibility("hidden"))) int tris_internal_stream_form = 256;
__attribute__((visibility("hidden"))) int tris_internal_col_blocks = 512;
}

namespace {

#include "amax.h"

__device__ __forceinline__ float4 ld4(const float* p) { return *reinterpret_cast<const float4*>(p); }
__device__ __forceinline__ void st4(float* p, float4 v) { *reinterpret_cast<float4*>(p) = v; }
typedef float f32x4_t __attribute__((ext_vector_type(4)));
__device__ __forceinline__ float4 ld4nt(const float* p) {
  const f32x4_t v = __builtin_nontemporal_load(reinterpret_cast<const f32x4_t*>(p));
  return make_float4(v.x, v.y, v.z, v.w);
}
__device__ __forceinline__ void st4nt(float* p, float4 v) {
  const f32x4_t w = {v.x, v.y, v.z, v.w};
  __builtin_nontemporal_store(w, reinterpret_cast<f32x4_t*>(p));
}
constexpr int BIG_U = 4;
constexpr long BIG_PIECE = 256L * BIG_U;
inline bool big_form(long n4, int C, int streams) { return tris_internal_stream_form && C >= 4 && 1024 % C == 0 && n4 * 16 * streams > ((long)tris_internal_stream_form << 20) && n4 >= 4 * BIG_PIECE; }
inline int big_grid(long n4) { return (int)((n4 + BIG_PIECE - 1) / BIG_PIECE); }

struct d4 { double x, y, z, w; };
__device__ __forceinline__ d4 d4zero() { d4 r; r.x = r.y = r.z = r.w = 0.0; return r; }
__device__ __forceinline__ void st4d(double* p, d4 v) { p[0] = v.x; p[1] = v.y; p[2] = v.z; p[3] = v.w; }

__device__ __forceinline__ long pooled_row(long r, int H, int W) {
  const int w = (int)(r % W);
  const long t = r / W;
  const int h = (int)(t % H);
  const long b = t / H;
  return (b * (H >> 1) + (h >> 1)) * (W >> 1) + (w >> 1);
}

template <int MODE, bool POOL = false>
__global__ __launch_bounds__(256) void col_partial_kernel(const float* __restrict__ X, const float* __restrict__ dY,
                                                          const float* __restrict__ Y, const float* __restrict__ mean,
                                                          const float* __restrict__ invstd, long M, int C, long ld,
                                                          long rows_per_block, double* __restrict__ part,
                                                          const float* __restrict__ gamma = nullptr,
                                                          const float* __restrict__ beta = nullptr,
                                                          float* __restrict__ dZ = nullptr, int pool_h = 0, int pool_w = 0,
                                                          int y_pl = 0, unsigned* __restrict__ amax = nullptr) {
  unsigned am = 0u;
  auto ldy = [&](long o) -> float4 {
    if (!y_pl) return ld4(Y + o);
    const char* yb = reinterpret_cast<const char*>(Y + (o & ~7L)) + (o & 4) * 2;
    const uint2 h = *reinterpret_cast<const uint2*>(yb), l = *reinterpret_cast<const uint2*>(yb + 16);
    const unsigned m0 = (h.x | l.x) & 0x7fff7fffu, m1 = (h.y | l.y) & 0x7fff7fffu;
// ... 406 lines not shown
    float* y = Y + (long)b * P * C + c;
    for (int p = pg; p < P; p += 4) {
      float o = (x[(long)p * C] - mean) * is * g + be;
      if (relu) o = fmaxf(o, 0.f);
      y[(long)p * C] = o;
      am = max(am, __builtin_bit_cast(unsigned, o) & 0x7fffffffu);
    }
    if (pg == 0) { mean_out[(long)b * C + c] = mean; invstd_out[(long)b * C + c] = is; }
  }
  if (amax != nullptr) amax_commit(am, amax);
}

__global__ __launch_bounds__(256) void instnorm_bwd_kernel(const float* __restrict__ dY, const float* __restrict__ Y,
                                                           const float* __restrict__ X, const float* __restrict__ gamma,
                                                           const float* __restrict__ mean_in,
                                                           const float* __restrict__ invstd_in, float* __restrict__ dX,
                                                           float* __restrict__ dgamma_part, float* __restrict__ dbeta_part,
                                                           int P, int C, int relu, unsigned* __restrict__ amax = nullptr) {
  __shared__ float r0[4][64];
  __shared__ float r1[4][64];
  const int b = blockIdx.y, cl = threadIdx.x & 63, c = blockIdx.x * 64 + cl, pg = threadIdx.x >> 6;
  const bool ok = c < C;
  const long base = (long)b * P * C + c;
  float mean = ok ? mean_in[(long)b * C + c] : 0.f, is = ok ? invstd_in[(long)b * C + c] : 0.f;
  float s0 = 0.f, s1 = 0.f;
  if (ok)
    for (int p = pg; p < P; p += 4) {
      float g = dY[base + (long)p * C];
      if (relu && !(Y[base + (long)p * C] > 0.f)) g = 0.f;
      s0 += g;
      s1 += g * (X[base + (long)p * C] - mean) * is;
    }
  r0[pg][cl] = s0;
  r1[pg][cl] = s1;
  __syncthreads();
  s0 = r0[0][cl] + r0[1][cl] + r0[2][cl] + r0[3][cl];
  s1 = r1[0][cl] + r1[1][cl] + r1[2][cl] + r1[3][cl];
  unsigned am = 0u;
  if (ok) {
    float ga = gamma[c], ip = 1.0f / (float)P;
    for (int p = pg; p < P; p += 4) {
      float g = dY[base + (long)p * C];
      if (relu && !(Y[base + (long)p * C] > 0.f)) g = 0.f;
      float xh = (X[base + (long)p * C] - mean) * is;
      const float d = ga * is * (g - s0 * ip - xh * s1 * ip);
      dX[base + (long)p * C] = d;
      am = max(am, __builtin_bit_cast(unsigned, d) & 0x7fffffffu);
    }
    if (pg == 0) { dgamma_part[(long)b * C + c] = s1; dbeta_part[(long)b * C + c] = s0; }
  }
  if (amax != nullptr) amax_commit(am, amax);
}

__global__ __launch_bounds__(256) void layernorm_fwd_kernel(const float* __restrict__ X, const float* __restrict__ gamma,
                                                            const float* __restrict__ beta, float* __restrict__ Y,
                                                            float* __restrict__ mean_out, float* __restrict__ rstd_out,
                                                            long rows, int W, float eps, unsigned* __restrict__ amax = nullptr,
                                                            const int* __restrict__ limit = nullptr) {
  const int lane = threadIdx.x & 63;
  const long row = (long)blockIdx.x * 4 + (threadIdx.x >> 6);
  if (row >= rows) return;
  if (limit != nullptr && row >= (long)*limit) return;
  unsigned am = 0u;
  const int W4 = W >> 2;
  float4 v[4];
  float s = 0.f;
#pragma unroll
  for (int q = 0; q < 4; ++q) {
    int i = lane + q * 64;
    v[q] = make_float4(0, 0, 0, 0);
    if (i < W4) { v[q] = ld4(X + row * W + i * 4); s += v[q].x + v[q].y + v[q].z + v[q].w; }
  }
  float mean = wave_sum(s) / (float)W;
  float s2 = 0.f;
#pragma unroll
  for (int q = 0; q < 4; ++q) {
    int i = lane + q * 64;
    if (i < W4) {
      float a = v[q].x - mean, b = v[q].y - mean, c = v[q].z - mean, d = v[q].w - mean;
      s2 += a * a + b * b + c * c + d * d;
    }
  }
  float rstd = rsqrtf(wave_sum(s2) / (float)W + eps);
#pragma unroll
  for (int q = 0; q < 4; ++q) {
    int i = lane + q * 64;
    if (i < W4) {
      float4 g = ld4(gamma + i * 4), b = ld4(beta + i * 4), o;
      o.x = (v[q].x - mean) * rstd * g.x + b.x;
      o.y = (v[q].y - mean) * rstd * g.y + b.y;
      o.z = (v[q].z - mean) * rstd * g.z + b.z;
      o.w = (v[q].w - mean) * rstd * g.w + b.w;
      st4(Y + row * W + i * 4, o);
      am = max(am, abits4(o));
    }
  }
  if (amax != nullptr) amax_commit(am, amax);
  if (lane == 0 && mean_out) { mean_out[row] = mean; rstd_out[row] = rstd; }
}

__global__ __launch_bounds__(256) void layernorm_bwd_kernel(const float* __restrict__ dY, const float* __restrict__ X,
                                                            const float* __restrict__ gamma,
                                                            const float* __restrict__ mean_in,
                                                            const float* __restrict__ rstd_in, float* __restrict__ dX,
                                                            float* __restrict__ part, long rows, int W,
                                                            long rows_per_block, const float* __restrict__ extra,
                                                            unsigned* __restrict__ amax = nullptr) {
  unsigned am = 0u;
  __shared__ float4 lg[4][256];
  __shared__ float4 lb[4][256];
  const int lane = threadIdx.x & 63, wv = threadIdx.x >> 6;
  const int W4 = W >> 2;
  float4 ag[4], ab[4];
#pragma unroll
  for (int q = 0; q < 4; ++q) ag[q] = ab[q] = make_float4(0, 0, 0, 0);
  const long rbeg = (long)blockIdx.x * rows_per_block, rend = min(rows, rbeg + rows_per_block);
  for (long row = rbeg + wv; row < rend; row += 4) {
    const float mean = mean_in[row], rstd = rstd_in[row];
    float4 xh[4], dh[4];
    float c1 = 0.f, c2 = 0.f;
#pragma unroll
    for (int q = 0; q < 4; ++q) {
      int i = lane + q * 64;
      xh[q] = dh[q] = make_float4(0, 0, 0, 0);
      if (i < W4) {
        float4 x = ld4(X + row * W + i * 4), dy = ld4(dY + row * W + i * 4), g = ld4(gamma + i * 4);
        xh[q] = make_float4((x.x - mean) * rstd, (x.y - mean) * rstd, (x.z - mean) * rstd, (x.w - mean) * rstd);
        dh[q] = make_float4(dy.x * g.x, dy.y * g.y, dy.z * g.z, dy.w * g.w);
        c1 += dh[q].x + dh[q].y + dh[q].z + dh[q].w;
        c2 += dh[q].x * xh[q].x + dh[q].y * xh[q].y + dh[q].z * xh[q].z + dh[q].w * xh[q].w;
        ag[q].x += dy.x * xh[q].x; ag[q].y += dy.y * xh[q].y; ag[q].z += dy.z * xh[q].z; ag[q].w += dy.w * xh[q].w;
        ab[q].x += dy.x; ab[q].y += dy.y; ab[q].z += dy.z; ab[q].w += dy.w;
      }
    }
    c1 = wave_sum(c1) / (float)W;
    c2 = wave_sum(c2) / (float)W;
    if (dX) {
#pragma unroll
      for (int q = 0; q < 4; ++q) {
        int i = lane + q * 64;
        if (i < W4) {
          float4 o;
          o.x = rstd * (dh[q].x - c1 - xh[q].x * c2);
          o.y = rstd * (dh[q].y - c1 - xh[q].y * c2);
          o.z = rstd * (dh[q].z - c1 - xh[q].z * c2);
          o.w = rstd * (dh[q].w - c1 - xh[q].w * c2);
          if (extra) {
            const float4 e = ld4(extra + row * W + i * 4);
            o.x += e.x; o.y += e.y; o.z += e.z; o.w += e.w;
          }
          st4(dX + row * W + i * 4, o);
          am = max(am, abits4(o));
        }
      }
    }
  }
  if (amax != nullptr) amax_commit_block(am, amax);
  if (!part) return;
#pragma unroll
  for (int q = 0; q < 4; ++q) { lg[wv][lane + q * 64] = ag[q]; lb[wv][lane + q * 64] = ab[q]; }
  __syncthreads();
  if (wv == 0) {
    float* o = part + (long)blockIdx.x * 2 * W;
#pragma unroll
    for (int q = 0; q < 4; ++q) {
      int i = lane + q * 64;
      if (i < W4) {
        float4 g = lg[0][i], b = lb[0][i];
        for (int w = 1; w < 4; ++w) {
          float4 g2 = lg[w][i], b2 = lb[w][i];
          g.x += g2.x; g.y += g2.y; g.z += g2.z; g.w += g2.w;
          b.x += b2.x; b.y += b2.y; b.z += b2.z; b.w += b2.w;
        }
        st4(o + i * 4, g);
        st4(o + W + i * 4, b);
      }
    }
  }
}

__global__ void avgpool2_fwd_kernel(const float* __restrict__ X, float* __restrict__ Y, int B, int H, int W, int C) {
  const int Ho = H >> 1, Wo = W >> 1, C4 = C >> 2;
  long n = (long)B * Ho * Wo * C4;
  long i = (long)blockIdx.x * blockDim.x + threadIdx.x;
  const long stride = (long)gridDim.x * blockDim.x;
  for (; i < n; i += stride) {
    int c4 = (int)(i % C4);
    long t = i / C4;
    int ox = (int)(t % Wo);
    t /= Wo;
    int oy = (int)(t % Ho);
    int b = (int)(t / Ho);
    const float* p = X + (((long)b * H + oy * 2) * W + ox * 2) * C + c4 * 4;
    float4 a = ld4(p), b4 = ld4(p + C), c = ld4(p + (long)W * C), d = ld4(p + (long)W * C + C);
    st4(Y + i * 4, make_float4(0.25f * (a.x + b4.x + c.x + d.x), 0.25f * (a.y + b4.y + c.y + d.y),
                               0.25f * (a.z + b4.z + c.z + d.z), 0.25f * (a.w + b4.w + c.w + d.w)));
  }
}

__global__ void avgpool2_bwd_kernel(const float* __restrict__ dY, float* __restrict__ dX, int B, int H, int W, int C) {
  const int Ho = H >> 1, Wo = W >> 1, C4 = C >> 2;
  long n = (long)B * H * W * C4;
  long i = (long)blockIdx.x * blockDim.x + threadIdx.x;
  const long stride = (long)gridDim.x * blockDim.x;
  for (; i < n; i += stride) {
    int c4 = (int)(i % C4);
    long t = i / C4;
    int x = (int)(t % W);
    t /= W;
    int y = (int)(t % H);
// ... 324 lines not shown
  return 0;
}

extern "C" int tris_bn_bwd_apply_f32(const float* dY, const float* Y, const float* X, const float* mean,
                                     const float* invstd, const float* gamma, const float* sum_dz, const float* sum_dzx,
                                     float inv_count, float* dX, float* dZ, long M, int C, const float* beta_mask,
                                     void* stream) {
  long n4 = M * C / 4;
  const int streams = 3 + ((Y && !beta_mask) ? 1 : 0) + (dZ ? 1 : 0);
  if (big_form(n4, C, streams))
    hipLaunchKernelGGL((bn_bwd_apply_kernel<false, true>), dim3(big_grid(n4)), dim3(256), 0, (hipStream_t)stream, dY, Y, X, mean,
                       invstd, gamma, sum_dz, sum_dzx, inv_count, dX, dZ, n4, C, beta_mask, 0, 0, take_amax_next());
  else
    hipLaunchKernelGGL((bn_bwd_apply_kernel<false, false>), dim3(bn_grid(n4, C)), dim3(256), 0, (hipStream_t)stream, dY, Y, X, mean,
                       invstd, gamma, sum_dz, sum_dzx, inv_count, dX, dZ, n4, C, beta_mask, 0, 0, take_amax_next());
  TRIS_LAUNCH_CHECK();
  return 0;
}

extern "C" int tris_colsum_f32(const float* X, long M, int N, long ld, float* out, float* workspace, void* stream) {
  hipStream_t st = (hipStream_t)stream;
  if (N % 4 || ld % 4 || (((uintptr_t)X) & 15)) {
    hipLaunchKernelGGL(colsum_scalar_kernel, dim3(cdiv(N, 256)), dim3(256), 0, st, X, M, N, ld, out);
    TRIS_LAUNCH_CHECK();
    return 0;
  }
  ColPlan p = col_plan(M, N);
  hipLaunchKernelGGL(col_partial_kernel<2>, dim3(p.nb), dim3(256), 0, st, X, nullptr, nullptr, nullptr, nullptr, M, N,
                     ld, p.rpb, (double*)workspace);
  TRIS_LAUNCH_CHECK();
  hipLaunchKernelGGL(part_finalize_kernel<double>, dim3(fin_grid(N, p.nb)), dim3(fin_block(p.nb)), 0, st, (const double*)workspace, p.nb, N,
                     out, (float*)nullptr);
  TRIS_LAUNCH_CHECK();
  return 0;
}

extern "C" int tris_instnorm_fwd_f32(const float* X, const float* gamma, const float* beta, float* Y, float* mean,
                                     float* invstd, int B, int P, int C, float eps, int relu, void* stream) {
  hipLaunchKernelGGL(instnorm_fwd_kernel, dim3(cdiv(C, 64), B), dim3(256), 0, (hipStream_t)stream, X, gamma, beta, Y,
                     mean, invstd, P, C, eps, relu, take_amax_next());
  TRIS_LAUNCH_CHECK();
  return 0;
}

extern "C" int tris_instnorm_bwd_f32(const float* dY, const float* Y, const float* X, const float* gamma,
                                     const float* mean, const float* invstd, float* dX, float* dgamma_part,
                                     float* dbeta_part, int B, int P, int C, int relu, void* stream) {
  hipLaunchKernelGGL(instnorm_bwd_kernel, dim3(cdiv(C, 64), B), dim3(256), 0, (hipStream_t)stream, dY, Y, X, gamma,
                     mean, invstd, dX, dgamma_part, dbeta_part, P, C, relu, take_amax_next());
  TRIS_LAUNCH_CHECK();
  return 0;
}

extern "C" int tris_layernorm_fwd_f32(const float* X, const float* gamma, const float* beta, float* Y, float* mean,
                                      float* rstd, long rows, int W, float eps, void* stream) {
  if (W % 4 || W > 1024) return (int)hipErrorInvalidValue;
  hipLaunchKernelGGL(layernorm_fwd_kernel, dim3(cdiv(rows, 4)), dim3(256), 0, (hipStream_t)stream, X, gamma, beta, Y,
                     mean, rstd, rows, W, eps, take_amax_next(), g_rows_limit);
  TRIS_LAUNCH_CHECK();
  return 0;
}

extern "C" { __attribute__((visibility("hidden"))) int tris_internal_ln_bwd_blocks = 512; }
static long ln_bwd_rpb(long rows) {
  const long target = tris_internal_ln_bwd_blocks;
  long rpb = (rows + target - 1) / target;
  const long floor_ = target > 128 ? 4 : 8;
  return rpb < floor_ ? floor_ : rpb;
}
extern "C" long tris_layernorm_bwd_workspace_bytes(long rows, int W) {
  const long rpb = ln_bwd_rpb(rows);
  long nb = (rows + rpb - 1) / rpb;
  if (nb < 512) nb = 512;
  return nb * 2 * W * (long)sizeof(float);
}

extern "C" int tris_layernorm_bwd_f32(const float* dY, const float* X, const float* gamma, const float* mean,
                                      const float* rstd, float* dX, float* dgamma, float* dbeta, long rows, int W,
                                      float* workspace, const float* extra, void* stream) {
  if (W % 4 || W > 1024) return (int)hipErrorInvalidValue;
  hipStream_t st = (hipStream_t)stream;
  const long rpb = ln_bwd_rpb(rows);
  int nb = (int)((rows + rpb - 1) / rpb);
  float* part = dgamma ? workspace : nullptr;
  hipLaunchKernelGGL(layernorm_bwd_kernel, dim3(nb), dim3(256), 0, st, dY, X, gamma, mean, rstd, dX, part, rows, W,
                     rpb, extra, take_amax_next());
  TRIS_LAUNCH_CHECK();
  if (dgamma) {
    hipLaunchKernelGGL(part_finalize_kernel<float>, dim3(fin_grid(W, nb)), dim3(fin_block(nb)), 0, st, (const float*)workspace, nb, W, dgamma, dbeta);
    TRIS_LAUNCH_CHECK();
  }
  return 0;
}

extern "C" int tris_avgpool2_fwd_f32(const float* X, float* Y, int B, int H, int W, int C, void* stream) {
  if (C % 4) return (int)hipErrorInvalidValue;
  long n = (long)B * (H / 2) * (W / 2) * (C / 4);
  hipLaunchKernelGGL(avgpool2_fwd_kernel, dim3(grid_for(n)), dim3(256), 0, (hipStream_t)stream, X, Y, B, H, W, C);
  TRIS_LAUNCH_CHECK();
  return 0;
}

extern "C" int tris_avgpool2_bwd_f32(const float* dY, float* dX, int B, int H, int W, int C, void* stream) {
  if (C % 4) return (int)hipErrorInvalidValue;
  long n = (long)B * H * W * (C / 4);
  hipLaunchKernelGGL(avgpool2_bwd_kernel, dim3(grid_for(n)), dim3(256), 0, (hipStream_t)stream, dY, dX, B, H, W, C);
  TRIS_LAUNCH_CHECK();
  return 0;
}

extern "C" int tris_elementwise_f32(int op, const float* A, const float* B, float* O, long n, float s, void* stream) {
  hipLaunchKernelGGL(ew_kernel, dim3(grid_for((n + 3) / 4)), dim3(256), 0, (hipStream_t)stream, op, A, B, O, n, s,
                     take_amax_next());
  TRIS_LAUNCH_CHECK();
  return 0;
}

extern "C" int tris_elementwise_bcast_f32(int op, const float* A, const float* B, float* O, long n, long nb, float s,
                                          void* stream) {
  if (B == nullptr || nb < 4 || (nb & 3) || (n & 3) || n % nb) return (int)hipErrorInvalidValue;
  hipLaunchKernelGGL(ew_kernel, dim3(grid_for(n / 4)), dim3(256), 0, (hipStream_t)stream, op, A, B, O, n, s, take_amax_next(), nb);
  TRIS_LAUNCH_CHECK();
  return 0;
}

namespace {
__global__ __launch_bounds__(256) void scale_exp_fwd_kernel(const float* __restrict__ X, const float* __restrict__ ls,
                                                            float* __restrict__ O, float* __restrict__ e_out, long n) {
  const float e = expf(ls[0]);
  if (blockIdx.x == 0 && threadIdx.x == 0) e_out[0] = e;
  const long stride = (long)gridDim.x * blockDim.x;
  for (long i = (long)blockIdx.x * blockDim.x + threadIdx.x; i < n; i += stride) O[i] = X[i] * e;
}
__global__ __launch_bounds__(256) void scale_exp_bwd_kernel(const float* __restrict__ dO, const float* __restrict__ O,
                                                            const float* __restrict__ ls, float* __restrict__ dX,
                                                            double* __restrict__ part, long n) {
  __shared__ double red[256];
  const float e = expf(ls[0]);
  const long stride = (long)gridDim.x * blockDim.x;
  float acc = 0.f;
  for (long i = (long)blockIdx.x * blockDim.x + threadIdx.x; i < n; i += stride) {
    const float g = dO[i];
    if (dX) dX[i] = g * e;
    acc += g * O[i];
  }
// ... 39 lines not shown
```

### tris_amd/ops.py

```python
import math
import os

import torch

from . import _lib
from ._lib import CONSTS, call, query
from .config import cfg

EW = CONSTS


class NoGpuError(RuntimeError):
    pass


_RAW_STREAM = getattr(torch._C, "_cuda_getCurrentRawStream", None)


def _stream():
    if _RAW_STREAM is not None:
        return _RAW_STREAM(torch.cuda.current_device())
    return torch.cuda.current_stream().cuda_stream


# ... 320 lines not shown
_PROF_SHAPES = False


def profile_begin():
    global _PROF
    _PROF = []


def profile_end():
    global _PROF
    rec, _PROF = _PROF, None
    torch.cuda.synchronize()
    return [(k, f, a.elapsed_time(b), nb) for k, f, a, b, nb in rec]


def _shape_tag(text):
    return text if _PROF_SHAPES else None


def _timed(kind, flops, fn, tag=None, nbytes=0):
    if _PROF is None:
        return fn()
    a, b = torch.cuda.Event(enable_timing=True), torch.cuda.Event(enable_timing=True)
    a.record()
    r = fn()
    b.record()
    if r is not False:
        _PROF.append((kind if tag is None else f"{kind}:{tag}", flops, a, b, nbytes))
    return r


_BATCH_INVARIANT = 0


class batch_invariant:
    def __enter__(self):
        global _BATCH_INVARIANT
        _BATCH_INVARIANT += 1
        if _BATCH_INVARIANT == 1:
            call("tris_set_conv_direct_thread", 0)
        _H2["paused"] += 1
        return self

    def __exit__(self, *exc):
        global _BATCH_INVARIANT
        _BATCH_INVARIANT -= 1
        _H2["paused"] -= 1
        if _BATCH_INVARIANT == 0:
            call("tris_set_conv_direct_thread", -1)
        return False


def gemm(A, B, C, M, N, K, lda, ldb, ldc, tA, tB, batch=1, sA=0, sB=0, sC=0, bias=None, bias_mode=0, resid=None,
         ldr=0, sR=0, act=0, alpha=1.0, use_ws=True, pre_out=None, dact=None, w_a=False, w_b=False, w_bt=False, mark=True):
    _chk(A, B, C, bias, resid)
    if pre_out is not None or dact is not None or batch != 1 or _BATCH_INVARIANT:
        A, B = unplanes(A), unplanes(B)
    if pre_out is not None or dact is not None:
        if _BATCH_INVARIANT or batch != 1:
            return False
        h2_arm(A, B)
        h2_mark_next(C)
        call("tris_gemm_epilogue_next", P(pre_out), P(dact))
        return _timed("gemm", 2.0 * M * N * K, lambda: _declinable(
            "tris_gemm_f32", P(A), P(B), P(C), M, N, K, lda, ldb, ldc, int(tA), int(tB), 1, 0, 0, 0, P(bias), bias_mode, P(resid),
            ldr, sR, act, float(alpha), None, 0, _stream()),
            nbytes=4.0 * (M * K + K * N + M * N * (2 + int(resid is not None))))
    if _BATCH_INVARIANT and batch == 1 and not tA and M < 4 and lda == K and ldc == N and (resid is None or ldr == N) and bias_mode != 2:
        A4 = A.new_zeros(4, K)
        A4[:M].copy_(A.reshape(M, K))
        R4 = None
        if resid is not None:
            R4 = resid.new_zeros(4, N)
            R4[:M].copy_(resid.reshape(M, N))
        C4 = C.new_empty(4, N)
        gemm(A4, B, C4, 4, N, K, K, ldb, N, False, tB, bias=bias, bias_mode=bias_mode, resid=R4, ldr=N, act=act, alpha=alpha,
             use_ws=use_ws)
        C.reshape(M, N).copy_(C4[:M])
        return C
    ws = workspace(0) if (use_ws and batch == 1 and not _BATCH_INVARIANT) else None
    blind = _rows_limit_blind(A, tA, batch)
    if (w_b and batch == 1 and not tA and M >= cfg.gemm_convert and cfg.gemm_convert > 0 and K % 32 == 0 and lda == K and getattr(B, "_tris_linear_w", False)
            and planes_on() and pl_word(A) is None and A.is_contiguous() and A.data_ptr() % 16 == 0 and _pl_weight_ok(B) and not blind):
        A = _a_planes(A, M, K)
    if blind:
        PL_STATS["last"] = PL_STATS["last_t"] = False
        pA, pB = P(A), P(unplanes(B))
    else:
        pA, pB = h2_pp(A, B, w_a=w_a, w_b=w_b, k_red=K, w_bt=w_bt and not tB) if batch == 1 else (P(A), P(B))
    if batch == 1 and PL_STATS["last_t"]:
        tB, ldb = True, K
    if mark:
        h2_mark_next(C)
    if ws is not None and cfg.fuse_splitk:
        tk = splitk_tickets()
        if tk is not None:
            call("tris_splitk_tickets_next", tk.data_ptr(), tk.numel())
    _timed("gemm", 2.0 * M * N * K * batch, lambda: call(
        "tris_gemm_f32", pA, pB, P(C), M, N, K, lda, ldb, ldc, int(tA), int(tB), batch, sA, sB, sC, P(bias),
        bias_mode, P(resid), ldr, sR, act, float(alpha), P(ws), 0 if ws is None else ws.numel() * 4, _stream()),
        tag=(f"{'T' if tA else 'N'}{'T' if tB else 'N'} M{M} N{N} K{K} b{batch}" if _PROF_SHAPES else None),
        nbytes=4.0 * ((M * K if (sA == 0 and batch > 1) else batch * M * K) + batch * K * N
                      + batch * M * N * (2 if resid is not None else 1)))
    return C


def colsum(X, M, N, out):
    ws = workspace(query("tris_col_workspace_bytes", M, N))
    call("tris_colsum_f32", P(X), M, N, N, P(out), P(ws), _stream())
    return out


def ew(op, A, B=None, s=0.0, out=None):
    _chk(A, B)
    out = torch.empty_like(A) if out is None else out
    h2_mark_next(out)
    call("tris_elementwise_f32", EW[op], P(A), P(B), P(out), A.numel(), float(s), _stream())
    return out


def nchw_to_nhwc(x):
    _chk(x)
    if x.dim() == 4 and x.permute(0, 2, 3, 1).is_contiguous():
        return x.permute(0, 2, 3, 1)
    x = x.contiguous()
    B, C, H, W = x.shape
    y = torch.empty(B, H, W, C, device=x.device, dtype=x.dtype)
    call("tris_nchw_to_nhwc_f32", P(x), P(y), B, C, H, W, _stream())
    return y


def _launch_with_stats(y, M, N, launch):
    import ctypes
    part = torch.empty(((M + 127) // 128) * 2 * N, device=y.device, dtype=torch.float64)
    rows = ctypes.c_int(0)
    launch(part, ctypes.byref(rows))
    if rows.value > 0:
        y._bn_part = (part, rows.value)


def _declinable(name, *args):
    err = getattr(_lib.load(), name)(*args)
    if err == -2:
        return False
    if err != 0:
        raise _lib.TrisHipError(f"{name} failed with hipError_t {err}")
    return True


class GradBox:
    __slots__ = ("value", "consumed")

    def __init__(self):
        self.value = None
        self.consumed = False

# ... 454 lines not shown
    if A is None or B is None or a_slot is not None or b_slot is not None or not planes_on() or k_red % 32 != 0:
        if pl_word(A) is not None or pl_word(B) is not None:
            A, B = unplanes(A), unplanes(B)
        h2_arm(A, B, a_slot, b_slot)
        return P(A), P(B)
    wa, wb = pl_word(A), pl_word(B)
    if wa is not None or wb is not None:
        pa = (P(A), wa) if wa is not None else (_pl_weight(A) if w_a else None)
        pb = (P(B), wb) if wb is not None else (_pl_weight(B) if w_b else None)
        if w_bt and wb is None and pa is not None:
            tt = getattr(B, "_plwt", None)
            if tt is not None and tt[0] == _H2["step"]:
                pb = (tt[1], tt[2])
                PL_STATS["last_t"] = True
        if pa is not None and pb is not None:
            call("tris_h2_next_planes", pa[1], pb[1], (1 if y_planes else 0) | (2 if PL_STATS["last_t"] else 0) | (4 if y_mask else 0))
            PL_STATS["products"] += 1
            PL_STATS["last"] = True
            return pa[0], pb[0]
        PL_STATS["mixed"] += 1
        A, B = unplanes(A), unplanes(B)
    h2_arm(A, B)
    return P(A), P(B)


class _BnBwdLink:
    __slots__ = ("x", "mean", "invstd", "gamma", "beta", "from_y", "dz", "part", "rows", "dzw", "mask")

    def __init__(self, x, mean, invstd, gamma, beta, from_y):
        self.x, self.mean, self.invstd, self.gamma, self.beta, self.from_y = x, mean, invstd, gamma, beta, from_y
        self.dz = self.part = self.dzw = None
        self.rows = 0
        self.mask = None

    def fill(self, dz, part, rows, dzw=None):
        self.dz, self.part, self.rows, self.dzw = (dz.data_ptr(), dz._version, tuple(dz.shape)), part, rows, dzw

    def take(self, dy):
        dz, part, rows, dzw = self.dz, self.part, self.rows, self.dzw
        self.dz = self.part = self.dzw = None
        if dz is None or (dy.data_ptr(), dy._version, tuple(dy.shape)) != dz:
            return None
        return part, rows, dzw


def _bn_bwd_fuse_enabled():
    return cfg.bn_bwd_fuse


class LinearFn(torch.autograd.Function):

    @staticmethod
    def forward(ctx, x, w, b, resid, act, stats=False, grad_box=None, grad_box_out=None, grad_box_res=None, bn_link=None,
                act_link=None):
        _chk(x, w, b, resid)
        ctx.grad_box, ctx.grad_box_out, ctx.grad_box_res = grad_box, grad_box_out, grad_box_res
        ctx.act_link = act_link
        ctx.bn_link = bn_link if (bn_link is not None and x.is_contiguous() and bn_link.x.shape == x.shape) else None
        x = x.contiguous()
        K = x.shape[-1]
        N = w.numel() // K
        M = x.numel() // K
        y = torch.empty(*x.shape[:-1], N, device=x.device, dtype=torch.float32)
        if resid is not None:
            resid = resid.contiguous()
        want_stats = stats and b is None and resid is None and act == 0
        if want_stats:
            _launch_with_stats(y, M, N, lambda part, rows: _timed(
                "gemm", 2.0 * M * N * K, lambda: (lambda pp: call("tris_gemm_bnstat_f32", pp[0], pp[1], P(y), M, N, K,
                                                                  part.data_ptr(), rows, _stream()))(h2_pp(x, w, w_b=True, k_red=K)),
                nbytes=4.0 * (M * K + K * N + M * N), tag=_shape_tag(f"bnstat M{M} N{N} K{K}")))
        else:
            gemm(x, w, y, M, N, K, K, K, N, False, True, bias=b, bias_mode=1 if b is not None else 0, resid=resid,
                 ldr=N, act=act, w_b=True)
        ctx.act, ctx.dims = act, (M, N, K)
        ctx.has_b, ctx.has_r = b is not None, resid is not None
        ctx.params = (w, b)
        ctx.x_pl = getattr(x, "_pl", None)
        ctx.save_for_backward(x, w, b, y if act == 1 else None)
        return y

    @staticmethod
    def backward(ctx, dy):
        if ctx.act == 2:
            raise RuntimeError("fused QuickGELU epilogue is forward-only; use QGeluFn when gradients are needed")
        if ctx.act == 1 and ctx.has_r:
            raise RuntimeError("relu + residual epilogue is forward-only")
        x, w, b, y = ctx.saved_tensors
        pw, pb = ctx.params
        M, N, K = ctx.dims
        dy = pl_grad_in(dy.contiguous())
        _retag(x, ctx.x_pl)
        if pl_word(dy) is not None and (ctx.has_r or ctx.has_b or ctx.act == 1):
            dy = unplanes(dy)
        if pl_word(dy) is None:
            x = unplanes(x)
        d_res = dy if ctx.has_r and ctx.needs_input_grad[3] else None
        if d_res is not None and ctx.grad_box_res is not None and ctx.grad_box_res.deposit(d_res):
            d_res = None
        if d_res is not None and _wgrad_enabled() and ctx.needs_input_grad[1]:
            d_res = dy.clone()
        if ctx.act == 1:
            dy = ew("TRIS_EW_RELU_BWD", dy, y)
        dx = None
        box = ctx.grad_box
        extra = None
        if box is not None:
            box.consumed = True
            if box.value is not None:
                extra, box.value = box.value, None
        if ctx.needs_input_grad[0]:
            dx = torch.empty_like(x)
            link, fused = ctx.bn_link, False
            if link is not None and (box is None or extra is not None):
                import ctypes
                part = torch.empty(((M + 127) // 128) * 2 * K, device=x.device, dtype=torch.float64)
                rows = ctypes.c_int(0)
                ypl = link.from_y and pl_word(x) is not None
                if not ypl or pl_word(dy) is not None:
                    dzw = _h2_slot() if planes_on() else None

                    def launch():
                        bits = ypl and link.mask is not None
                        pp = h2_pp(dy, w, w_b=True, y_planes=ypl, k_red=N, w_bt=True, y_mask=bits)
                        if dzw is not None:
                            call("tris_amax_next", dzw)
                        by = (P(x) if (PL_STATS["last"] or not ypl) else P(unplanes(x))) if link.from_y else None
                        if bits and PL_STATS["last"]:
                            by = link.mask.data_ptr()
                        call("tris_gemm_bnbwd_f32", pp[0], pp[1], P(dx), M, K, N, P(extra), K, P(link.x), by,
                             P(link.mean), P(link.invstd), P(link.gamma), P(link.beta), part.data_ptr(), ctypes.byref(rows), _stream())
                        return rows.value > 0
                    _timed("gemm_bnbwd", 2.0 * M * N * K, launch, tag=_shape_tag(f"M{M} N{K} K{N}"),
                           nbytes=4.0 * (M * N + N * K + M * K * (2 + int(link.from_y) + int(extra is not None))))
                    if rows.value > 0:
                        fused = True
                        link.fill(dx, part, rows.value, dzw)
            alink = ctx.act_link
            if not fused and alink is not None and extra is None:
                if gemm(dy, w, dx, M, K, N, N, K, K, False, False, dact=alink.pre) is not False:
                    fused = alink.applied = True
            if not fused:
                gemm(dy, w, dx, M, K, N, N, K, K, False, False, resid=extra, ldr=K, w_b=True, w_bt=True)
        elif extra is not None:
            raise RuntimeError("a residual gradient was handed to a layer whose input needs no gradient")
        if dx is not None and ctx.grad_box_out is not None and ctx.grad_box_out.deposit(dx):
            dx = None
        dw = None
        if ctx.needs_input_grad[1]:
            if _sink(pw) is not None:
                on_wgrad_stream(lambda: gemm(dy, x, _sink(pw), N, K, M, N, K, K, True, False, mark=False), dy, x, sink=_sink(pw))
            else:
                dw = _emit(pw, lambda o: gemm(dy, x, o, N, K, M, N, K, K, True, False, mark=False), True)
        db = None
        if ctx.has_b:
            db = _emit(pb, lambda o: colsum(dy, M, N, o), ctx.needs_input_grad[2], reads=(dy,))
        return dx, dw, db, d_res, None, None, None, None, None, None, None


def linear(x, w, b=None, resid=None, act=0, stats=False, grad_box=None, grad_box_out=None, grad_box_res=None, act_link=False):
    link = getattr(x, "_bn_link", None)
    if link is not None and not (torch.is_grad_enabled() and x.requires_grad and _bn_bwd_fuse_enabled()):
        link = None
    alink = getattr(x, "_act_link", None) if (act_link and torch.is_grad_enabled() and x.requires_grad) else None
    return LinearFn.apply(x, w, b, resid, act, stats, grad_box, grad_box_out, grad_box_res, link, alink)


class _ActLink:
    __slots__ = ("pre", "applied")

    def __init__(self, pre):
        self.pre, self.applied = pre, False


class LinearQGeluFn(torch.autograd.Function):

    @staticmethod
    def forward(ctx, x, w, b):
        _chk(x, w, b)
        x = x.contiguous()
        K = x.shape[-1]
        N = w.numel() // K
        M = x.numel() // K
        y = torch.empty(*x.shape[:-1], N, device=x.device, dtype=torch.float32)
        pre = torch.empty_like(y)
        if gemm(x, w, y, M, N, K, K, K, N, False, True, bias=b, bias_mode=1 if b is not None else 0, act=2, pre_out=pre) is False:
            gemm(x, w, pre, M, N, K, K, K, N, False, True, bias=b, bias_mode=1 if b is not None else 0)
            ew("TRIS_EW_QGELU", pre, out=y)
        ctx.dims, ctx.has_b, ctx.params = (M, N, K), b is not None, (w, b)
        ctx.link = y._act_link = _ActLink(pre)
        ctx.save_for_backward(x, w, pre)
        return y

    @staticmethod
    def backward(ctx, dy):
        x, w, pre = ctx.saved_tensors
        pw, pb = ctx.params
        M, N, K = ctx.dims
        dy = dy.contiguous()
        dpre = dy if ctx.link.applied else ew("TRIS_EW_QGELU_BWD", dy, pre)
        dx = None
        if ctx.needs_input_grad[0]:
            dx = torch.empty_like(x)
            gemm(dpre, w, dx, M, K, N, N, K, K, False, False)
        dw = None
        if ctx.needs_input_grad[1]:
            if _sink(pw) is not None:
                on_wgrad_stream(lambda: gemm(dpre, x, _sink(pw), N, K, M, N, K, K, True, False, mark=False), dpre, x, sink=_sink(pw))
            else:
                dw = _emit(pw, lambda o: gemm(dpre, x, o, N, K, M, N, K, K, True, False, mark=False), True)
        db = None
        if ctx.has_b:
            db = _emit(pb, lambda o: colsum(dpre, M, N, o), ctx.needs_input_grad[2], reads=(dpre,))
        return dx, dw, db


def linear_qgelu(x, w, b=None):
    return LinearQGeluFn.apply(x, w, b)


class MatmulFn(torch.autograd.Function):

    @staticmethod
    def forward(ctx, A, B, tB):
        _chk(A, B)
        A, B = A.contiguous(), B.contiguous()
        K = A.shape[-1]
        M = A.numel() // K
        N = B.shape[0] if tB else B.shape[1]
        C = torch.empty(*A.shape[:-1], N, device=A.device, dtype=torch.float32)
        gemm(A, B, C, M, N, K, K, B.shape[1], N, False, tB)
        ctx.tB, ctx.dims = tB, (M, N, K)
        ctx.params = (B,)
        ctx.save_for_backward(A, B)
        return C

    @staticmethod
    def backward(ctx, dC):
        A, B = ctx.saved_tensors
        M, N, K = ctx.dims
        dC = dC.contiguous()
        dA = dB = None
        if ctx.needs_input_grad[0]:
            dA = torch.empty_like(A)
            if ctx.tB:
                gemm(dC, B, dA, M, K, N, N, K, K, False, False)
            else:
                gemm(dC, B, dA, M, K, N, N, N, K, False, True)
        if ctx.needs_input_grad[1]:
            if ctx.tB:
                dB = _emit(ctx.params[0], lambda o: gemm(dC, A, o, N, K, M, N, K, K, True, False, mark=False), True)
            else:
                dB = _emit(ctx.params[0], lambda o: gemm(A, dC, o, K, N, M, K, N, N, True, False, mark=False), True)
        return dA, dB, None


def matmul(A, B, tB=False):
    return MatmulFn.apply(A, B, tB)


class BmmFn(torch.autograd.Function):

    @staticmethod
    def forward(ctx, A, B, tB, alpha):
        _chk(A, B)
        A, B = A.contiguous(), B.contiguous()
        Bt = B.shape[0]
        shared = A.dim() == 2
        M, K = A.shape[-2], A.shape[-1]
        N = B.shape[1] if tB else B.shape[2]
        C = torch.empty(Bt, M, N, device=B.device, dtype=torch.float32)
# ... 447 lines not shown
class AvgPool2Fn(torch.autograd.Function):
    @staticmethod
    def forward(ctx, x, grad_box_out=None):
        _chk(x)
        ctx.grad_box_out = grad_box_out
        x = x.contiguous()
        B, H, W, C = x.shape
        y = torch.empty(B, H // 2, W // 2, C, device=x.device, dtype=torch.float32)
        w = pl_word(x)
        if w is not None and C % 8 == 0:
            call("tris_avgpool2_fwd_pl_f32", P(x), P(y), w, B, H, W, C, _stream())
            pl_tag(y, w)
        else:
            call("tris_avgpool2_fwd_f32", P(unplanes(x)), P(y), B, H, W, C, _stream())
        ctx.shape = (B, H, W, C)
        return y

    @staticmethod
    def backward(ctx, dy):
        B, H, W, C = ctx.shape
        dy = unplanes(pl_grad_in(dy.contiguous()))
        dx = torch.empty(B, H, W, C, device=dy.device, dtype=torch.float32)
        call("tris_avgpool2_bwd_f32", P(dy), P(dx), B, H, W, C, _stream())
        if ctx.grad_box_out is not None and ctx.grad_box_out.deposit(dx):
            dx = None
        return dx, None


def avgpool2(x, grad_box_out=None):
    return AvgPool2Fn.apply(x, grad_box_out)


class LayerNormFn(torch.autograd.Function):
    @staticmethod
    def forward(ctx, x, g, b, eps, grad_box=None):
        _chk(x, g, b)
        ctx.grad_box = grad_box
        x = x.contiguous()
        W = x.shape[-1]
        rows = x.numel() // W
        y = torch.empty_like(x)
        st = torch.empty(2, rows, device=x.device, dtype=torch.float32)
        h2_mark_next(y)
        call("tris_layernorm_fwd_f32", P(x), P(g), P(b), P(y), P(st), P(st, rows), rows, W, eps, _stream())
        ctx.dims = (rows, W)
        ctx.params = (g, b)
        ctx.save_for_backward(x, g, b, st)
        return y

    @staticmethod
    def backward(ctx, dy):
        x, g, b, st = ctx.saved_tensors
        rows, W = ctx.dims
        dy = dy.contiguous()
        dx = torch.empty_like(x) if ctx.needs_input_grad[0] else None
        box, extra = ctx.grad_box, None
        if box is not None:
            box.consumed = True
            if box.value is not None:
                extra, box.value = box.value.contiguous(), None
                if dx is None:
                    raise RuntimeError("a residual gradient was handed to a LayerNorm whose input needs no gradient")
        need_p = ctx.needs_input_grad[1] or ctx.needs_input_grad[2]
        ws = workspace(query("tris_layernorm_bwd_workspace_bytes", rows, W))
        sg, sb = _sink(ctx.params[0]), _sink(ctx.params[1])
        if need_p and sg is not None and sb is not None and sg.is_contiguous() and sb.is_contiguous():
            h2_mark_next(dx)
            call("tris_layernorm_bwd_f32", P(dy), P(x), P(g), P(st), P(st, rows), P(dx), P(sg), P(sb), rows, W, P(ws),
                 P(extra), _stream())
            return dx, None, None, None, None
        dgb = torch.empty(2, W, device=x.device, dtype=torch.float32) if need_p else None
        h2_mark_next(dx)
        call("tris_layernorm_bwd_f32", P(dy), P(x), P(g), P(st), P(st, rows), P(dx), P(dgb), P(dgb, W),
             rows, W, P(ws), P(extra), _stream())
        dg = _emit(ctx.params[0], lambda o: o.copy_(dgb[0]), ctx.needs_input_grad[1])
        db = _emit(ctx.params[1], lambda o: o.copy_(dgb[1]), ctx.needs_input_grad[2])
        return dx, dg, db, None, None


def layer_norm(x, g, b, eps=1e-5, grad_box=None):
    return LayerNormFn.apply(x, g, b, eps, grad_box)


class MhaFn(torch.autograd.Function):

    @staticmethod
    def forward(ctx, qkv, heads, causal):
        _chk(qkv)
        qkv = qkv.contiguous()
        N, L, W3 = qkv.shape
        W = W3 // 3
        out = torch.empty(N, L, W, device=qkv.device, dtype=torch.float32)
        h2_mark_next(out)
        call("tris_mha_fwd_f32", P(qkv), P(out), N, L, W, heads, int(causal), _stream())
        ctx.cfg = (N, L, W, heads, int(causal))
        ctx.save_for_backward(qkv)
        return out

    @staticmethod
    def backward(ctx, do):
        (qkv,) = ctx.saved_tensors
        N, L, W, heads, causal = ctx.cfg
        do = do.contiguous()
        dqkv = torch.empty_like(qkv)
        h2_mark_next(dqkv)
        call("tris_mha_bwd_f32", P(qkv), P(do), P(dqkv), N, L, W, heads, causal, _stream())
        return dqkv, None, None


MHA_STATS = {"last": None}


class MhaMfmaFn(torch.autograd.Function):

    @staticmethod
    def forward(ctx, qkv, heads, causal):
        _chk(qkv)
        qkv = qkv.contiguous()
        N, L, W3 = qkv.shape
        W = W3 // 3
        out = torch.empty(N, L, W, device=qkv.device, dtype=torch.float32)
        lse = torch.empty(N, heads, L, device=qkv.device, dtype=torch.float32)
        w_qkv = _h2_amax(qkv) if (h2_on() and cfg.mha_h2 and L >= 32) else None
        h2_mark_next(out)
        if w_qkv is not None:
            _timed("mha_fwd", 4.0 * N * heads * L * L * 64 * (0.5 if causal else 1.0),
                   lambda: call("tris_mha_h2_fwd_f32", P(qkv), P(out), P(lse), w_qkv, N, L, W, heads, int(causal), _stream()))
        else:
            _timed("mha_fwd", 4.0 * N * heads * L * L * 64 * (0.5 if causal else 1.0),
                   lambda: call("tris_mha_mfma_fwd_f32", P(qkv), P(out), P(lse), N, L, W, heads, int(causal), _stream()))
        MHA_STATS["last"] = "h2" if w_qkv is not None else "f32"
        ctx.h2 = w_qkv is not None
        ctx.cfg = (N, L, W, heads, int(causal))
        ctx.save_for_backward(qkv, out, lse)
        return out

    @staticmethod
    def backward(ctx, do):
        qkv, out, lse = ctx.saved_tensors
        N, L, W, heads, causal = ctx.cfg
        do = do.contiguous()
        dqkv = torch.empty_like(qkv)
        delta = torch.empty_like(lse)
        w_qkv = w_do = None
        if ctx.h2 and h2_on():
            w_qkv, w_do = _h2_amax(qkv), _h2_amax(do)
        h2_mark_next(dqkv)
        if w_qkv is not None and w_do is not None:
            call("tris_mha_h2_bwd_f32", P(qkv), P(out), P(do), P(lse), P(delta), P(dqkv), w_qkv, w_do, N, L, W, heads, causal, _stream())
        else:
            call("tris_mha_mfma_bwd_f32", P(qkv), P(out), P(do), P(lse), P(delta), P(dqkv), N, L, W, heads, causal, _stream())
        return dqkv, None, None


def _mha_impl(L):
    import os
    mode = cfg.mha
    if L > 64 or mode == "mfma":
        return "mfma"
    if mode == "valu":
        return "valu"
    return "valu" if L < 40 else "mfma"


def mha(qkv, heads, causal):
    if _mha_impl(qkv.shape[1]) == "valu":
        return MhaFn.apply(qkv, heads, causal)
    return MhaMfmaFn.apply(qkv, heads, causal)


class QGeluFn(torch.autograd.Function):
    @staticmethod
    def forward(ctx, x):
        x = x.contiguous()
        ctx.save_for_backward(x)
        return ew("TRIS_EW_QGELU", x)

    @staticmethod
    def backward(ctx, dy):
        (x,) = ctx.saved_tensors
        return ew("TRIS_EW_QGELU_BWD", dy.contiguous(), x)


def quick_gelu(x):
    return QGeluFn.apply(x)


class EmbedFn(torch.autograd.Function):

    @staticmethod
    def forward(ctx, ids, tok, pos, reducer=None):
        _chk(ids, tok, pos)
        ids = ids.contiguous()
        N, L = ids.shape
        W = tok.shape[1]
        out = torch.empty(N, L, W, device=tok.device, dtype=torch.float32)
        call("tris_embed_fwd_f32", P(ids), P(tok), P(pos), P(out), N, L, W, _stream())
        ctx.params = (tok, pos)
        ctx.reducer = reducer
        ctx.save_for_backward(ids, tok, pos)
        return out
# ... 1202 lines not shown
```

Measured before the change: 1359 img/s.

## Defer split-K slab reduction into LayerNorm and fuse MHA h2 backward kernels

```diff
diff --git a/include/tris_hip.h b/include/tris_hip.h
--- a/include/tris_hip.h
+++ b/include/tris_hip.h
@@ -117,6 +117,13 @@
 long tris_layernorm_bwd_workspace_bytes(long rows, int W);
 int tris_layernorm_bwd_f32(const float* dY, const float* X, const float* gamma, const float* mean, const float* rstd,
                            float* dX, float* dgamma, float* dbeta, long rows, int W, float* workspace, const float* extra , void* stream);
+int tris_splitk_defer_next(int arm);
+long tris_splitk_deferred(void);
+int tris_layernorm_fwd_slabs_f32(float* X, const float* gamma, const float* beta, float* Y, float* mean, float* rstd, long rows, int W,
+                                 float eps, void* stream);
+int tris_layernorm_bwd_slabs_f32(const float* dY, const float* X, const float* gamma, const float* mean, const float* rstd, float* dX,
+                                 float* dgamma, float* dbeta, long rows, int W, const float* extra, void* stream);
+long tris_chain_fused_launches(void);
 
 int tris_bn_apply_pool_f32(const float* X, const float* mean, const float* invstd, const float* gamma, const float* beta,
                            float* Yp, int B, int H, int W, int C, void* stream);
@@ -156,6 +163,7 @@
 int tris_mha_h2_bwd_f32(const float* qkv, const float* out, const float* dout, const float* lse, float* delta, float* dqkv,
                         const unsigned* amax_qkv, const unsigned* amax_dout, int N, int L, int W, int heads, int causal,
                         void* stream);
+int tris_mha_h2_bwd_split_next(void);
 int tris_text_pack_plan_i64(const long* ids, int N, int L, int* plan, void* stream);
 int tris_embed_packed_fwd_f32(const long* ids, const float* tok, const float* pos, const int* plan, float* out, int N, int L, int W,
                               void* stream);
diff --git a/tris_amd/CLIP/clip/model.py b/tris_amd/CLIP/clip/model.py
--- a/tris_amd/CLIP/clip/model.py
+++ b/tris_amd/CLIP/clip/model.py
@@ -247,11 +247,11 @@
         use_box = torch.is_grad_enabled() and x.requires_grad and cfg.grad_box
         b1 = ops.GradBox() if use_box else None
         b2 = ops.GradBox() if use_box else None
-        h = self.ln_1(x, b1)
+        h = ops.ln_sole(self.ln_1(x, b1))
         qkv = ops.linear(h, self.attn.in_proj_weight, self.attn.in_proj_bias)
         a = ops.mha(qkv, self.attn.num_heads, self.causal)
         x = self.attn.out_proj(a, resid=x, grad_box_res=b1)
-        h = self.ln_2(x, b2)
+        h = ops.ln_sole(self.ln_2(x, b2))
         if torch.is_grad_enabled() and cfg.mlp_fuse:
             f = ops.linear_qgelu(h, self.mlp.c_fc.weight, self.mlp.c_fc.bias)
             return ops.linear(f, self.mlp.c_proj.weight, self.mlp.c_proj.bias, x, 0, grad_box_res=b2, act_link=True)
@@ -270,11 +270,11 @@
         return self.mlp.c_proj(self.mlp.c_fc(h, act=2), resid=x)
 
     def forward_token0(self, x):
-        h = self.ln_1(x)
+        h = ops.ln_sole(self.ln_1(x))
         qkv = ops.linear(h, self.attn.in_proj_weight, self.attn.in_proj_bias)
         a = ops.token0(ops.mha(qkv, self.attn.num_heads, self.causal))
         x0 = self.attn.out_proj(a, resid=ops.token0(x))
-        h = self.ln_2(x0)
+        h = ops.ln_sole(self.ln_2(x0))
         if torch.is_grad_enabled() and cfg.mlp_fuse:
             f = ops.linear_qgelu(h, self.mlp.c_fc.weight, self.mlp.c_fc.bias)
             return ops.linear(f, self.mlp.c_proj.weight, self.mlp.c_proj.bias, x0, 0, act_link=True)
diff --git a/tris_amd/_lib.py b/tris_amd/_lib.py
--- a/tris_amd/_lib.py
+++ b/tris_amd/_lib.py
@@ -63,11 +63,26 @@
 
 _FN = {}
 
+DEFER = __import__("threading").local()
+_DEFER_CONSUMERS = frozenset(("tris_layernorm_fwd_slabs_f32", "tris_layernorm_bwd_slabs_f32"))
+_DEFER_PASS = frozenset(("tris_amax_next", "tris_splitk_defer_next"))
+
+
+def defer_fail(what):
+    DEFER.deferred = 0
+    load().tris_splitk_defer_next(0)
+    raise TrisHipError(f"{what} while a split-K product waits for the LayerNorm that sums its slabs: its output is unwritten "
+                       "(tris_splitk_defer_next)")
+
 
 def call(name, *args):
     fn = _FN.get(name)
     if fn is None:
         fn = _FN[name] = getattr(load(), name)
+    if getattr(DEFER, "deferred", 0) and name not in _DEFER_PASS:
+        if name not in _DEFER_CONSUMERS:
+            defer_fail(name)
+        DEFER.deferred = 0
     err = fn(*args)
     if err != 0:
         raise TrisHipError(f"{name} failed with hipError_t {err}")
diff --git a/tris_amd/config.py b/tris_amd/config.py
--- a/tris_amd/config.py
+++ b/tris_amd/config.py
@@ -53,6 +53,7 @@
         self.step_graph_rerecord = int(e("TRIS_STEP_GRAPH_RERECORD", "3"))
         self.side_param_grads = _flag("TRIS_SIDE_PARAM_GRADS", True)
         self.vit_token0 = _flag("TRIS_VIT_TOKEN0", True)
+        self.chain_fuse = _flag("TRIS_CHAIN_FUSE", True)
 
     @contextlib.contextmanager
     def override(self, **kw):
diff --git a/tris_amd/csrc/attn_h2.hip b/tris_amd/csrc/attn_h2.hip
--- a/tris_amd/csrc/attn_h2.hip
+++ b/tris_amd/csrc/attn_h2.hip
@@ -168,6 +168,209 @@
   if (amax != nullptr) amax_commit(am, amax);
 }
 
+__device__ __forceinline__ float delta_of_row(const float* gp, const float* op, float4 (&g)[4]) {
+  float dl = 0.f;
+#pragma unroll
+  for (int ks = 0; ks < 2; ++ks) {
+    const float4 g0 = ldg4(gp + 32 * ks), g1 = ldg4(gp + 32 * ks + 4), o0 = ldg4(op + 32 * ks), o1 = ldg4(op + 32 * ks + 4);
+    g[2 * ks] = g0;
+    g[2 * ks + 1] = g1;
+    dl += g0.x * o0.x + g0.y * o0.y + g0.z * o0.z + g0.w * o0.w + g1.x * o1.x + g1.y * o1.y + g1.z * o1.z + g1.w * o1.w;
+  }
+  dl += __shfl_xor(dl, 16, 64);
+  dl += __shfl_xor(dl, 32, 64);
+  return dl;
+}
+
+__device__ __forceinline__ void mha_h2_dq_block(const float* __restrict__ qkv, const float* __restrict__ out,
+                                                const float* __restrict__ dout, const float* __restrict__ lse,
+                                                float* __restrict__ delta, float* __restrict__ dqkv, int L, int W, int causal,
+                                                float scale, const unsigned* __restrict__ am_qkv,
+                                                const unsigned* __restrict__ am_do, unsigned* __restrict__ amax, int bx, char* Kp,
+                                                char* Vp) {
+  const int tid = threadIdx.x, lane = tid & 63, wave = tid >> 6, r = lane & 15, kg = lane >> 4;
+  const int h = blockIdx.y, n = blockIdx.z, H = gridDim.y;
+  const int qb = bx * 64, q0 = qb + wave * 16;
+  const float s = h2_scale_from_bits(h2_amax_of(am_qkv, lane)), sg = h2_scale_from_bits(h2_amax_of(am_do, lane));
+  const float inv_s = scale / (s * s), inv_p = 1.0f / (s * sg);
+  const float* base = qkv + (long)n * L * 3 * W + h * HD;
+  const int qrow = min(q0 + r, L - 1);
+  H8 qf[2], gf[2];
+  resident(qf, base + (long)qrow * 3 * W + 8 * kg, s);
+  float4 g[4];
+  const float dl = delta_of_row(dout + ((long)n * L + qrow) * W + h * HD + 8 * kg, out + ((long)n * L + qrow) * W + h * HD + 8 * kg, g);
+#pragma unroll
+  for (int ks = 0; ks < 2; ++ks) gf[ks] = split8(g[2 * ks], g[2 * ks + 1], sg);
+  if (kg == 0 && q0 + r < L) delta[((long)n * H + h) * L + q0 + r] = dl;
+  const float ls = lse[((long)n * H + h) * L + qrow];
+  f4v acc[4];
+#pragma unroll
+  for (int j = 0; j < 4; ++j) acc[j] = (f4v){0.f, 0.f, 0.f, 0.f};
+  const int kend = causal ? min(L, qb + 64) : L;
+  for (int kb = 0; kb < kend; kb += 64) {
+    __syncthreads();
+    stage64(Kp, base + W, 3L * W, kb, L, tid, s);
+    stage64(Vp, base + 2 * W, 3L * W, kb, L, tid, s);
+    __syncthreads();
+    if (q0 < L) {
+#pragma unroll
+      for (int pr = 0; pr < 2; ++pr) {
+        const int key0 = kb + 32 * pr;
+        if (key0 < kend && !(causal && key0 > q0 + 15)) {
+          f4v sc[2], sx[2], pc[2], px[2];
+#pragma unroll
+          for (int j = 0; j < 2; ++j) {
+            sc[j] = sx[j] = pc[j] = px[j] = (f4v){0.f, 0.f, 0.f, 0.f};
+            const int row = 32 * pr + trow(r, j);
+#pragma unroll
+            for (int ks = 0; ks < 2; ++ks) {
+              mm3(afrag(Kp, row, ks, kg), qf[ks], sc[j], sx[j]);
+              mm3(afrag(Vp, row, ks, kg), gf[ks], pc[j], px[j]);
+            }
+          }
+          float ds[8], mx = 0.f;
+          const bool full = key0 + 32 <= L && !(causal && key0 + 31 > q0);
+#pragma unroll
+          for (int i = 0; i < 8; ++i) {
+            const int key = key0 + 8 * kg + i;
+            const bool ok = full || (key < L && !(causal && key > q0 + r));
+            const float sv = (sc[i >> 2][i & 3] + sx[i >> 2][i & 3] * (1.0f / 2048.0f)) * inv_s;
+            const float dp = (pc[i >> 2][i & 3] + px[i >> 2][i & 3] * (1.0f / 2048.0f)) * inv_p;
+            ds[i] = ok ? __expf(sv - ls) * (dp - dl) * scale : 0.f;
+            mx = fmaxf(mx, fabsf(ds[i]));
+          }
+          const float sd = wave_scale_of(mx);
+          const H8 df = split8(make_float4(ds[0], ds[1], ds[2], ds[3]), make_float4(ds[4], ds[5], ds[6], ds[7]), sd);
+          const float inv_d = 1.0f / (sd * s);
+#pragma unroll
+          for (int ct = 0; ct < 4; ++ct) {
+            f4v tc = {0.f, 0.f, 0.f, 0.f}, tx = {0.f, 0.f, 0.f, 0.f};
+            mm3(df, bfrag(Kp, 32 * pr, ct, r, kg), tc, tx);
+            acc[ct] += join(tc, tx) * inv_d;
+          }
+        }
+      }
+    }
+  }
+  unsigned am = 0u;
+  if (q0 < L) {
+    float* ob = dqkv + (long)n * L * 3 * W + h * HD;
+#pragma unroll
+    for (int t = 0; t < 4; ++t) {
+      const int q = q0 + 4 * kg + t;
+      if (q < L) {
+#pragma unroll
+        for (int j = 0; j < 4; ++j) {
+          ob[(long)q * 3 * W + 16 * j + r] = acc[j][t];
+          am = max(am, __builtin_bit_cast(unsigned, acc[j][t]) & 0x7fffffffu);
+        }
+      }
+    }
+  }
+  if (amax != nullptr) amax_commit(am, amax);
+}
+
+template <bool OWN_DELTA>
+__device__ __forceinline__ void mha_h2_dkv_block(const float* __restrict__ qkv, const float* __restrict__ out,
+                                                 const float* __restrict__ dout, const float* __restrict__ lse,
+                                                 const float* __restrict__ delta, float* __restrict__ dqkv, int L, int W, int causal,
+                                                 float scale, const unsigned* __restrict__ am_qkv,
+                                                 const unsigned* __restrict__ am_do, unsigned* __restrict__ amax, int bx, char* Qp,
+                                                 char* Gp, float* Ls, float* Ds) {
+  const int tid = threadIdx.x, lane = tid & 63, wave = tid >> 6, r = lane & 15, kg = lane >> 4;
+  const int h = blockIdx.y, n = blockIdx.z, H = gridDim.y;
+  const int kb0 = bx * 64, k0 = kb0 + wave * 16;
+  const float s = h2_scale_from_bits(h2_amax_of(am_qkv, lane)), sg = h2_scale_from_bits(h2_amax_of(am_do, lane));
+  const float inv_s = scale / (s * s), inv_p = 1.0f / (s * sg), inv_v = 1.0f / (PS * sg);
+  const float* base = qkv + (long)n * L * 3 * W + h * HD;
+  const int krow = min(k0 + r, L - 1);
+  H8 kf[2], vf[2];
+  resident(kf, base + W + (long)krow * 3 * W + 8 * kg, s);
+  resident(vf, base + 2 * W + (long)krow * 3 * W + 8 * kg, s);
+  f4v dk[4], vc[4], vx[4];
+#pragma unroll
+  for (int j = 0; j < 4; ++j) dk[j] = vc[j] = vx[j] = (f4v){0.f, 0.f, 0.f, 0.f};
+  float own_dl = 0.f;
+  if (OWN_DELTA) {
+    const int qrow = min(wave * 16 + r, L - 1);
+    float4 g[4];
+    own_dl = delta_of_row(dout + ((long)n * L + qrow) * W + h * HD + 8 * kg, out + ((long)n * L + qrow) * W + h * HD + 8 * kg, g);
+  }
+  const int qstart = causal ? kb0 : 0;
+  for (int qb = qstart; qb < L; qb += 64) {
+    __syncthreads();
+    stage64(Qp, base, 3L * W, qb, L, tid, s);
+    stage64(Gp, dout + (long)n * L * W + h * HD, (long)W, qb, L, tid, sg);
+    if (tid < 64) {
+      const int q = min(qb + tid, L - 1);
+      Ls[tid] = lse[((long)n * H + h) * L + q];
+      if (!OWN_DELTA) Ds[tid] = delta[((long)n * H + h) * L + q];
+    }
+    if (OWN_DELTA && kg == 0) Ds[wave * 16 + r] = own_dl;
+    __syncthreads();
+    if (k0 < L) {
+#pragma unroll
+      for (int pr = 0; pr < 2; ++pr) {
+        const int qs0 = qb + 32 * pr;
+        if (qs0 < L && !(causal && qs0 + 31 < k0)) {
+          f4v sc[2], sx[2], pc[2], px[2];
+#pragma unroll
+          for (int j = 0; j < 2; ++j) {
+            sc[j] = sx[j] = pc[j] = px[j] = (f4v){0.f, 0.f, 0.f, 0.f};
+            const int row = 32 * pr + trow(r, j);
+#pragma unroll
+            for (int ks = 0; ks < 2; ++ks) {
+              mm3(afrag(Qp, row, ks, kg), kf[ks], sc[j], sx[j]);
+              mm3(afrag(Gp, row, ks, kg), vf[ks], pc[j], px[j]);
+            }
+          }
+          float p[8], ds[8], mx = 0.f;
+          const bool full = qs0 + 32 <= L && !(causal && k0 + 15 > qs0);
+#pragma unroll
+          for (int i = 0; i < 8; ++i) {
+            const int ql = 32 * pr + 8 * kg + i, q = qb + ql;
+            const bool ok = full || (q < L && !(causal && k0 + r > q));
+            const float sv = (sc[i >> 2][i & 3] + sx[i >> 2][i & 3] * (1.0f / 2048.0f)) * inv_s;
+            const float dp = (pc[i >> 2][i & 3] + px[i >> 2][i & 3] * (1.0f / 2048.0f)) * inv_p;
+            p[i] = ok ? __expf(sv - Ls[ql]) : 0.f;
+            ds[i] = p[i] * (dp - Ds[ql]) * scale;
+            mx = fmaxf(mx, fabsf(ds[i]));
+          }
+          const float sd = wave_scale_of(mx);
+          const H8 pf = split8(make_float4(p[0], p[1], p[2], p[3]), make_float4(p[4], p[5], p[6], p[7]), PS);
+          const H8 df = split8(make_float4(ds[0], ds[1], ds[2], ds[3]), make_float4(ds[4], ds[5], ds[6], ds[7]), sd);
+          const float inv_d = 1.0f / (sd * s);
+#pragma unroll
+          for (int ct = 0; ct < 4; ++ct) {
+            mm3(pf, bfrag(Gp, 32 * pr, ct, r, kg), vc[ct], vx[ct]);
+            f4v tc = {0.f, 0.f, 0.f, 0.f}, tx = {0.f, 0.f, 0.f, 0.f};
+            mm3(df, bfrag(Qp, 32 * pr, ct, r, kg), tc, tx);
+            dk[ct] += join(tc, tx) * inv_d;
+          }
+        }
+      }
+    }
+  }
+  unsigned am = 0u;
+  if (k0 < L) {
+    float* ob = dqkv + (long)n * L * 3 * W + h * HD;
+#pragma unroll
+    for (int t = 0; t < 4; ++t) {
+      const int k = k0 + 4 * kg + t;
+      if (k < L) {
+#pragma unroll
+        for (int j = 0; j < 4; ++j) {
+          const float dv = (vc[j][t] + vx[j][t] * (1.0f / 2048.0f)) * inv_v;
+          ob[(long)k * 3 * W + W + 16 * j + r] = dk[j][t];
+          ob[(long)k * 3 * W + 2 * W + 16 * j + r] = dv;
+          am = max(am, max(__builtin_bit_cast(unsigned, dk[j][t]) & 0x7fffffffu, __builtin_bit_cast(unsigned, dv) & 0x7fffffffu));
+        }
+      }
+    }
+  }
+  if (amax != nullptr) amax_commit(am, amax);
+}
+
 __global__ __launch_bounds__(256) void mha_h2_dq_kernel(const float* __restrict__ qkv, const float* __restrict__ out,
                                                         const float* __restrict__ dout, const float* __restrict__ lse,
                                                         float* __restrict__ delta, float* __restrict__ dqkv, int L, int W, int causal,
@@ -175,95 +378,7 @@
                                                         const unsigned* __restrict__ am_do, unsigned* __restrict__ amax) {
   __shared__ __attribute__((aligned(16))) char Kp[2 * PLB];
   __shared__ __attribute__((aligned(16))) char Vp[2 * PLB];
-  const int tid = threadIdx.x, lane = tid & 63, wave = tid >> 6, r = lane & 15, kg = lane >> 4;
-  const int h = blockIdx.y, n = blockIdx.z, H = gridDim.y;
-  const int qb = blockIdx.x * 64, q0 = qb + wave * 16;
-  const float s = h2_scale_from_bits(h2_amax_of(am_qkv, lane)), sg = h2_scale_from_bits(h2_amax_of(am_do, lane));
-  const float inv_s = scale / (s * s), inv_p = 1.0f / (s * sg);
-  const float* base = qkv + (long)n * L * 3 * W + h * HD;
-  const int qrow = min(q0 + r, L - 1);
-  H8 qf[2], gf[2];
-  resident(qf, base + (long)qrow * 3 * W + 8 * kg, s);
-  float dl = 0.f;
-  {
-    const float* gp = dout + ((long)n * L + qrow) * W + h * HD + 8 * kg;
-    const float* op = out + ((long)n * L + qrow) * W + h * HD + 8 * kg;
-#pragma unroll
-    for (int ks = 0; ks < 2; ++ks) {
-      const float4 g0 = ldg4(gp + 32 * ks), g1 = ldg4(gp + 32 * ks + 4), o0 = ldg4(op + 32 * ks), o1 = ldg4(op + 32 * ks + 4);
-      gf[ks] = split8(g0, g1, sg);
-      dl += g0.x * o0.x + g0.y * o0.y + g0.z * o0.z + g0.w * o0.w + g1.x * o1.x + g1.y * o1.y + g1.z * o1.z + g1.w * o1.w;
-    }
-    dl += __shfl_xor(dl, 16, 64);
-    dl += __shfl_xor(dl, 32, 64);
-    if (kg == 0 && q0 + r < L) delta[((long)n * H + h) * L + q0 + r] = dl;
-  }
-  const float ls = lse[((long)n * H + h) * L + qrow];
-  f4v acc[4];
-#pragma unroll
-  for (int j = 0; j < 4; ++j) acc[j] = (f4v){0.f, 0.f, 0.f, 0.f};
-  const int kend = causal ? min(L, qb + 64) : L;
-  for (int kb = 0; kb < kend; kb += 64) {
-    __syncthreads();
-    stage64(Kp, base + W, 3L * W, kb, L, tid, s);
-    stage64(Vp, base + 2 * W, 3L * W, kb, L, tid, s);
-    __syncthreads();
-    if (q0 < L) {
-#pragma unroll
-      for (int pr = 0; pr < 2; ++pr) {
-        const int key0 = kb + 32 * pr;
-        if (key0 < kend && !(causal && key0 > q0 + 15)) {
-          f4v sc[2], sx[2], pc[2], px[2];
-#pragma unroll
-          for (int j = 0; j < 2; ++j) {
-            sc[j] = sx[j] = pc[j] = px[j] = (f4v){0.f, 0.f, 0.f, 0.f};
-            const int row = 32 * pr + trow(r, j);
-#pragma unroll
-            for (int ks = 0; ks < 2; ++ks) {
-              mm3(afrag(Kp, row, ks, kg), qf[ks], sc[j], sx[j]);
-              mm3(afrag(Vp, row, ks, kg), gf[ks], pc[j], px[j]);
-            }
-          }
-          float ds[8], mx = 0.f;
-          const bool full = key0 + 32 <= L && !(causal && key0 + 31 > q0);
-#pragma unroll
-          for (int i = 0; i < 8; ++i) {
-            const int key = key0 + 8 * kg + i;
-            const bool ok = full || (key < L && !(causal && key > q0 + r));
-            const float sv = (sc[i >> 2][i & 3] + sx[i >> 2][i & 3] * (1.0f / 2048.0f)) * inv_s;
-            const float dp = (pc[i >> 2][i & 3] + px[i >> 2][i & 3] * (1.0f / 2048.0f)) * inv_p;
-            ds[i] = ok ? __expf(sv - ls) * (dp - dl) * scale : 0.f;
-            mx = fmaxf(mx, fabsf(ds[i]));
-          }
-          const float sd = wave_scale_of(mx);
-          const H8 df = split8(make_float4(ds[0], ds[1], ds[2], ds[3]), make_float4(ds[4], ds[5], ds[6], ds[7]), sd);
-          const float inv_d = 1.0f / (sd * s);
-#pragma unroll
-          for (int ct = 0; ct < 4; ++ct) {
-            f4v tc = {0.f, 0.f, 0.f, 0.f}, tx = {0.f, 0.f, 0.f, 0.f};
-            mm3(df, bfrag(Kp, 32 * pr, ct, r, kg), tc, tx);
-            acc[ct] += join(tc, tx) * inv_d;
-          }
-        }
-      }
-    }
-  }
-  unsigned am = 0u;
-  if (q0 < L) {
-    float* ob = dqkv + (long)n * L * 3 * W + h * HD;
-#pragma unroll
-    for (int t = 0; t < 4; ++t) {
-      const int q = q0 + 4 * kg + t;
-      if (q < L) {
-#pragma unroll
-        for (int j = 0; j < 4; ++j) {
-          ob[(long)q * 3 * W + 16 * j + r] = acc[j][t];
-          am = max(am, __builtin_bit_cast(unsigned, acc[j][t]) & 0x7fffffffu);
-        }
-      }
-    }
-  }
-  if (amax != nullptr) amax_commit(am, amax);
+  mha_h2_dq_block(qkv, out, dout, lse, delta, dqkv, L, W, causal, scale, am_qkv, am_do, amax, blockIdx.x, Kp, Vp);
 }
 
 __global__ __launch_bounds__(256) void mha_h2_dkv_kernel(const float* __restrict__ qkv, const float* __restrict__ dout,
@@ -274,96 +389,31 @@
   __shared__ __attribute__((aligned(16))) char Qp[2 * PLB];
   __shared__ __attribute__((aligned(16))) char Gp[2 * PLB];
   __shared__ float Ls[64], Ds[64];
-  const int tid = threadIdx.x, lane = tid & 63, wave = tid >> 6, r = lane & 15, kg = lane >> 4;
-  const int h = blockIdx.y, n = blockIdx.z, H = gridDim.y;
-  const int kb0 = blockIdx.x * 64, k0 = kb0 + wave * 16;
-  const float s = h2_scale_from_bits(h2_amax_of(am_qkv, lane)), sg = h2_scale_from_bits(h2_amax_of(am_do, lane));
-  const float inv_s = scale / (s * s), inv_p = 1.0f / (s * sg), inv_v = 1.0f / (PS * sg);
-  const float* base = qkv + (long)n * L * 3 * W + h * HD;
-  const int krow = min(k0 + r, L - 1);
-  H8 kf[2], vf[2];
-  resident(kf, base + W + (long)krow * 3 * W + 8 * kg, s);
-  resident(vf, base + 2 * W + (long)krow * 3 * W + 8 * kg, s);
-  f4v dk[4], vc[4], vx[4];
-#pragma unroll
-  for (int j = 0; j < 4; ++j) dk[j] = vc[j] = vx[j] = (f4v){0.f, 0.f, 0.f, 0.f};
-  const int qstart = causal ? kb0 : 0;
-  for (int qb = qstart; qb < L; qb += 64) {
-    __syncthreads();
-    stage64(Qp, base, 3L * W, qb, L, tid, s);
-    stage64(Gp, dout + (long)n * L * W + h * HD, (long)W, qb, L, tid, sg);
-    if (tid < 64) {
-      const int q = min(qb + tid, L - 1);
-      Ls[tid] = lse[((long)n * H + h) * L + q];
-      Ds[tid] = delta[((long)n * H + h) * L + q];
-    }
-    __syncthreads();
-    if (k0 < L) {
-#pragma unroll
-      for (int pr = 0; pr < 2; ++pr) {
-        const int qs0 = qb + 32 * pr;
-        if (qs0 < L && !(causal && qs0 + 31 < k0)) {
-          f4v sc[2], sx[2], pc[2], px[2];
-#pragma unroll
-          for (int j = 0; j < 2; ++j) {
-            sc[j] = sx[j] = pc[j] = px[j] = (f4v){0.f, 0.f, 0.f, 0.f};
-            const int row = 32 * pr + trow(r, j);
-#pragma unroll
-            for (int ks = 0; ks < 2; ++ks) {
-              mm3(afrag(Qp, row, ks, kg), kf[ks], sc[j], sx[j]);
-              mm3(afrag(Gp, row, ks, kg), vf[ks], pc[j], px[j]);
-            }
-          }
-          float p[8], ds[8], mx = 0.f;
-          const bool full = qs0 + 32 <= L && !(causal && k0 + 15 > qs0);
-#pragma unroll
-          for (int i = 0; i < 8; ++i) {
-            const int ql = 32 * pr + 8 * kg + i, q = qb + ql;
-            const bool ok = full || (q < L && !(causal && k0 + r > q));
-            const float sv = (sc[i >> 2][i & 3] + sx[i >> 2][i & 3] * (1.0f / 2048.0f)) * inv_s;
-            const float dp = (pc[i >> 2][i & 3] + px[i >> 2][i & 3] * (1.0f / 2048.0f)) * inv_p;
-            p[i] = ok ? __expf(sv - Ls[ql]) : 0.f;
-            ds[i] = p[i] * (dp - Ds[ql]) * scale;
-            mx = fmaxf(mx, fabsf(ds[i]));
-          }
-          const float sd = wave_scale_of(mx);
-          const H8 pf = split8(make_float4(p[0], p[1], p[2], p[3]), make_float4(p[4], p[5], p[6], p[7]), PS);
-          const H8 df = split8(make_float4(ds[0], ds[1], ds[2], ds[3]), make_float4(ds[4], ds[5], ds[6], ds[7]), sd);
-          const float inv_d = 1.0f / (sd * s);
-#pragma unroll
-          for (int ct = 0; ct < 4; ++ct) {
-            mm3(pf, bfrag(Gp, 32 * pr, ct, r, kg), vc[ct], vx[ct]);
-            f4v tc = {0.f, 0.f, 0.f, 0.f}, tx = {0.f, 0.f, 0.f, 0.f};
-            mm3(df, bfrag(Qp, 32 * pr, ct, r, kg), tc, tx);
-            dk[ct] += join(tc, tx) * inv_d;
-          }
-        }
-      }
-    }
-  }
-  unsigned am = 0u;
-  if (k0 < L) {
-    float* ob = dqkv + (long)n * L * 3 * W + h * HD;
-#pragma unroll
-    for (int t = 0; t < 4; ++t) {
-      const int k = k0 + 4 * kg + t;
-      if (k < L) {
-#pragma unroll
-        for (int j = 0; j < 4; ++j) {
-          const float dv = (vc[j][t] + vx[j][t] * (1.0f / 2048.0f)) * inv_v;
-          ob[(long)k * 3 * W + W + 16 * j + r] = dk[j][t];
-          ob[(long)k * 3 * W + 2 * W + 16 * j + r] = dv;
-          am = max(am, max(__builtin_bit_cast(unsigned, dk[j][t]) & 0x7fffffffu, __builtin_bit_cast(unsigned, dv) & 0x7fffffffu));
-        }
-      }
-    }
-  }
-  if (amax != nullptr) amax_commit(am, amax);
+  mha_h2_dkv_block<false>(qkv, nullptr, dout, lse, delta, dqkv, L, W, causal, scale, am_qkv, am_do, amax, blockIdx.x, Qp, Gp, Ls, Ds);
+}
+
+__global__ __launch_bounds__(256, 3) void mha_h2_bwd1_kernel(const float* __restrict__ qkv, const float* __restrict__ out,
+                                                          const float* __restrict__ dout, const float* __restrict__ lse,
+                                                          float* __restrict__ delta, float* __restrict__ dqkv, int L, int W, int causal,
+                                                          float scale, const unsigned* __restrict__ am_qkv,
+                                                          const unsigned* __restrict__ am_do, unsigned* __restrict__ amax) {
+  __shared__ __attribute__((aligned(16))) char Ap[2 * PLB];
+  __shared__ __attribute__((aligned(16))) char Bp[2 * PLB];
+  __shared__ float Ls[64], Ds[64];
+  if (blockIdx.x == 0) mha_h2_dq_block(qkv, out, dout, lse, delta, dqkv, L, W, causal, scale, am_qkv, am_do, amax, 0, Ap, Bp);
+  else mha_h2_dkv_block<true>(qkv, out, dout, lse, nullptr, dqkv, L, W, causal, scale, am_qkv, am_do, amax, 0, Ap, Bp, Ls, Ds);
 }
 
 }
 
 extern "C" __attribute__((visibility("hidden"))) unsigned* tris_internal_take_amax_next();
+extern "C" __attribute__((visibility("hidden"))) void tris_internal_chain_fused();
+
+static thread_local bool g_bwd_split_next = false;
+extern "C" int tris_mha_h2_bwd_split_next(void) {
+  g_bwd_split_next = true;
+  return 0;
+}
 
 extern "C" int tris_mha_h2_fwd_f32(const float* qkv, float* out, float* lse, const unsigned* amax_qkv, int N, int L, int W, int heads,
                                    int causal, void* stream) {
@@ -383,6 +433,15 @@
   const float scale = 1.0f / sqrtf((float)HD);
   const dim3 grid(cdiv(L, 64), heads, N);
   unsigned* amax = tris_internal_take_amax_next();
+  const bool split = g_bwd_split_next;
+  g_bwd_split_next = false;
+  if (grid.x == 1 && !split) {
+    hipLaunchKernelGGL(mha_h2_bwd1_kernel, dim3(2, heads, N), dim3(256), 0, (hipStream_t)stream, qkv, out, dout, lse, delta, dqkv, L, W,
+                       causal, scale, amax_qkv, amax_dout, amax);
+    TRIS_LAUNCH_CHECK();
+    tris_internal_chain_fused();
+    return 0;
+  }
   hipLaunchKernelGGL(mha_h2_dq_kernel, grid, dim3(256), 0, (hipStream_t)stream, qkv, out, dout, lse, delta, dqkv, L, W, causal, scale,
                      amax_qkv, amax_dout, amax);
   TRIS_LAUNCH_CHECK();
diff --git a/tris_amd/csrc/conv_direct.hip b/tris_amd/csrc/conv_direct.hip
--- a/tris_amd/csrc/conv_direct.hip
+++ b/tris_amd/csrc/conv_direct.hip
@@ -4,6 +4,7 @@
 
 #include "common.h"
 #include "tris_hip.h"
+#include "splitk_defer.h"
 
 namespace {
 
diff --git a/tris_amd/csrc/gemm_conv.hip b/tris_amd/csrc/gemm_conv.hip
--- a/tris_amd/csrc/gemm_conv.hip
+++ b/tris_amd/csrc/gemm_conv.hip
@@ -7,6 +7,7 @@
 
 #include "common.h"
 #include "tris_hip.h"
+#include "splitk_defer.h"
 
 extern "C" {
 extern __attribute__((visibility("hidden"))) int tris_internal_stream_form;
@@ -34,6 +35,7 @@
 struct Options {
   int force_tile = 0;
   int force_pipe = -1;
+  int force_splitk = 0;
   int pipe_default = -1;
   int conv_direct = -1;
   int wgrad_direct = -1;
@@ -50,6 +52,7 @@
   const bool unset = (v == nullptr || v[0] == 0);
   if (!strcmp(name, "FORCE_TILE")) o.force_tile = parse_tile(v);
   else if (!strcmp(name, "FORCE_PIPE")) o.force_pipe = unset ? -1 : std::min(5, std::max(0, atoi(v)));
+  else if (!strcmp(name, "FORCE_SPLITK")) o.force_splitk = unset ? 0 : std::max(0, atoi(v));
   else if (!strcmp(name, "PIPE")) o.pipe_default = unset ? -1 : (v[0] == '0' ? 0 : 1);
   else if (!strcmp(name, "CONV_DIRECT")) o.conv_direct = unset ? -1 : atoi(v);
   else if (!strcmp(name, "WGRAD_DIRECT")) o.wgrad_direct = unset ? -1 : atoi(v);
@@ -71,7 +74,7 @@
 }
 static Options init_options() {
   Options o;
-  for (const char* n : {"FORCE_TILE", "FORCE_PIPE", "PIPE", "CONV_DIRECT", "WGRAD_DIRECT", "BN_FOLD", "STEM_CONV1", "WG_BLOCKS", "STREAM_FORM", "COL_BLOCKS", "XATTN_PX_SLOTS", "LN_BWD_BLOCKS", "FIN_BLOCK", "REDUCE_WIDE", "XCD_ORDER", "FUSE_SPLITK", "RED_GRID", "TUNE_LOG"}) {
+  for (const char* n : {"FORCE_TILE", "FORCE_PIPE", "FORCE_SPLITK", "PIPE", "CONV_DIRECT", "WGRAD_DIRECT", "BN_FOLD", "STEM_CONV1", "WG_BLOCKS", "STREAM_FORM", "COL_BLOCKS", "XATTN_PX_SLOTS", "LN_BWD_BLOCKS", "FIN_BLOCK", "REDUCE_WIDE", "XCD_ORDER", "FUSE_SPLITK", "RED_GRID", "TUNE_LOG"}) {
     char env[64];
     snprintf(env, sizeof(env), "TRIS_%s", n);
     if (const char* v = getenv(env)) set_option(o, n, v);
@@ -184,6 +187,9 @@
     if (forced == 4 && p.N <= 32) { bm = 128; bn = 32; }
     if (forced == 5 && p.N > 64 && p.M >= 256 && p.stat_part == nullptr) { bm = 256; bn = 128; }
   }
+  if (g_opt.force_splitk > 0 && batch == 1 && ws != nullptr && p.stat_part == nullptr && p.K >= 64 * g_opt.force_splitk &&
+      (long)g_opt.force_splitk * p.M * p.N * (long)sizeof(float) <= ws_bytes)
+    splitk = g_opt.force_splitk;
   Cfg c = {bm, bn, splitk, default_pipe(p, bm, bn, splitk)};
   return c;
 }
@@ -206,24 +212,27 @@
 template <int AK, int BKIND>
 int launch_cfg(GemmParams& p, int batch, float* ws, long ws_bytes, hipStream_t st) {
   Cfg h = heuristic_cfg(p, batch, ws, ws_bytes);
-  if (!autotune_enabled() || g_opt.force_tile) return run_cfg<AK, BKIND>(p, batch, ws, st, h);
+  TrisSplitkDefer* const dfr = p.defer;
+  p.defer = nullptr;
+  auto run_final = [&](const Cfg& c) { p.defer = dfr; return run_cfg<AK, BKIND>(p, batch, ws, st, c); };
+  if (!autotune_enabled() || g_opt.force_tile || g_opt.force_splitk) return run_final(h);
   const bool stat = p.stat_part != nullptr;
   const TuneKey key = {AK, BKIND + (stat ? 16 : 0) + (p.bnb_x != nullptr ? 32 : 0), p.M, p.N, p.K, batch, g_gemm_mode};
   {
     std::lock_guard<std::mutex> lk(g_tune_mu);
     auto it = g_tuned.find(key);
-    if (it != g_tuned.end()) return run_cfg<AK, BKIND>(p, batch, ws, st, it->second);
+    if (it != g_tuned.end()) return run_final(it->second);
   }
   hipStreamCaptureStatus cap = hipStreamCaptureStatusNone;
   if (hipStreamIsCapturing(st, &cap) != hipSuccess || cap != hipStreamCaptureStatusNone)
-    return run_cfg<AK, BKIND>(p, batch, ws, st, h);
+    return run_final(h);
   static const int tiles[5][2] = {{128, 128}, {128, 64}, {64, 64}, {128, 32}, {256, 128}};
   const bool fastk = gemm_fast_ok(p);
   static const int sks[] = {1, 2, 3, 4, 6, 8, 12, 16, 24, 32, 48, 64, 96, 128};
   const bool can_split = (batch == 1 && ws != nullptr && p.K >= 512) && !stat;
   const bool can_pipe = pipe_ok(p) && g_opt.force_pipe != 0;
   hipEvent_t e0, e1;
-  if (hipEventCreate(&e0) != hipSuccess || hipEventCreate(&e1) != hipSuccess) return run_cfg<AK, BKIND>(p, batch, ws, st, h);
+  if (hipEventCreate(&e0) != hipSuccess || hipEventCreate(&e1) != hipSuccess) return run_final(h);
   (void)hipDeviceSynchronize();
   Cfg best = h;
   float best_ms = 1e30f;
@@ -281,7 +290,7 @@
       }
     }
   }
-  return run_cfg<AK, BKIND>(p, batch, ws, st, best);
+  return run_final(best);
 }
 
 
@@ -440,6 +449,18 @@
   return 0;
 }
 
+static thread_local TrisSplitkDefer g_defer = {};
+extern "C" __attribute__((visibility("hidden"))) TrisSplitkDefer* tris_internal_splitk_defer() { return &g_defer; }
+static long g_chain_fused = 0;
+extern "C" __attribute__((visibility("hidden"))) void tris_internal_chain_fused() { __atomic_fetch_add(&g_chain_fused, 1L, __ATOMIC_RELAXED); }
+extern "C" long tris_chain_fused_launches(void) { return __atomic_load_n(&g_chain_fused, __ATOMIC_RELAXED); }
+extern "C" int tris_splitk_defer_next(int arm) {
+  g_defer.armed = arm ? 1 : 0;
+  if (!arm) g_defer.pending = 0;
+  return 0;
+}
+extern "C" long tris_splitk_deferred(void) { return g_defer.pending ? (long)(uintptr_t)g_defer.C : 0L; }
+
 extern "C" int tris_gemm_f32(const float* A, const float* B, float* C, int M, int N, int K, long lda, long ldb,
                              long ldc, int transA, int transB, int batch, long sA, long sB, long sC,
                              const float* bias, int bias_mode, const float* resid, long ldr, long sR, int act,
@@ -450,6 +471,12 @@
   g_epi_next.armed = false;
   const TicketsNext tkn = g_tickets_next;
   g_tickets_next = {nullptr, 0};
+  const bool defer = g_defer.armed != 0;
+  g_defer.armed = 0;
+  if (g_defer.pending) {
+    g_defer.pending = 0;
+    return (int)hipErrorIllegalState;
+  }
   if (M <= 0 || N <= 0 || batch <= 0) return 0;
   if (K <= 0) return (int)hipErrorInvalidValue;
   GemmParams p = {};
@@ -478,6 +505,10 @@
   }
   H2Guard h2(p, h2n);
   if (h2.bad) return (int)hipErrorInvalidValue;
+  if (defer && batch == 1 && workspace != nullptr) {
+    g_defer.ws_bytes = ws_bytes;
+    p.defer = &g_defer;
+  }
   if (!transA && transB) return launch_cfg<A_ROWK, B_NK>(p, batch, workspace, ws_bytes, st);
   if (!transA && !transB) return launch_cfg<A_ROWK, B_KN>(p, batch, workspace, ws_bytes, st);
   if (transA && !transB) return launch_cfg<A_COLK, B_KN>(p, batch, workspace, ws_bytes, st);
diff --git a/tris_amd/csrc/gemm_core.h b/tris_amd/csrc/gemm_core.h
--- a/tris_amd/csrc/gemm_core.h
+++ b/tris_amd/csrc/gemm_core.h
@@ -5,6 +5,7 @@
 
 #include "common.h"
 #include "tris_hip.h"
+#include "splitk_defer.h"
 
 namespace {
 
@@ -579,8 +580,18 @@
       else
         hipLaunchKernelGGL(splitk_reduce_wide_kernel<4>, dim3(cdiv(total / 4, 64)), dim3(256), 0, st, ws, splitk, p);
     }
-    else if ((p.N & 3) == 0 && al16(ws) && al16(p.C))
-      hipLaunchKernelGGL(splitk_reduce_kernel<4>, dim3(red_blocks(cdiv(total / 4, 256))), dim3(256), 0, st, ws, splitk, p);
+    else if ((p.N & 3) == 0 && al16(ws) && al16(p.C)) {
+      TrisSplitkDefer* const d = p.defer;
+      if (d != nullptr && batch == 1 && vec_fin && p.ldc == p.N && p.N <= 1024 && p.bias_mode != 2 &&
+          ((long)splitk * total + (1L << 20)) * (long)sizeof(float) <= d->ws_bytes) {
+        d->ws = ws; d->S = splitk; d->M = p.M; d->N = p.N; d->ldc = p.ldc; d->alpha = p.alpha; d->bias = p.bias;
+        d->bias_mode = p.bias_mode; d->act = p.act; d->resid = p.resid; d->ldr = p.ldr; d->C = p.C; d->amax = p.amax_out;
+        d->m_limit = p.m_limit; d->stream = (void*)st;
+        d->pending = 1;
+      } else {
+        hipLaunchKernelGGL(splitk_reduce_kernel<4>, dim3(red_blocks(cdiv(total / 4, 256))), dim3(256), 0, st, ws, splitk, p);
+      }
+    }
     else
       hipLaunchKernelGGL(splitk_reduce_kernel<1>, dim3(red_blocks(cdiv(total, 256))), dim3(256), 0, st, ws, splitk, p);
     TRIS_LAUNCH_CHECK();
diff --git a/tris_amd/csrc/gemm_params.h b/tris_amd/csrc/gemm_params.h
--- a/tris_amd/csrc/gemm_params.h
+++ b/tris_amd/csrc/gemm_params.h
@@ -44,6 +44,7 @@
   float* Cfin;
   int vecCfin;
   int fin_groups;
+  TrisSplitkDefer* defer;
 };
 #define TRIS_FUSE_SPLITK_MAX 16
 #define TRIS_FUSE_SPLITK_DEFAULT 16
diff --git a/tris_amd/csrc/norm.hip b/tris_amd/csrc/norm.hip
--- a/tris_amd/csrc/norm.hip
+++ b/tris_amd/csrc/norm.hip
@@ -2,6 +2,7 @@
 
 #include "common.h"
 #include "tris_hip.h"
+#include "splitk_defer.h"
 
 extern "C" {
 __attribute__((visibility("hidden"))) int tris_internal_stream_form = 256;
@@ -514,16 +515,17 @@
   if (amax != nullptr) amax_commit(am, amax);
 }
 
+template <bool SLABS>
 __global__ __launch_bounds__(256) void layernorm_fwd_kernel(const float* __restrict__ X, const float* __restrict__ gamma,
                                                             const float* __restrict__ beta, float* __restrict__ Y,
                                                             float* __restrict__ mean_out, float* __restrict__ rstd_out,
-                                                            long rows, int W, float eps, unsigned* __restrict__ amax = nullptr,
-                                                            const int* __restrict__ limit = nullptr) {
+                                                            long rows, int W, float eps, unsigned* __restrict__ amax,
+                                                            const int* __restrict__ limit, const TrisSlabIn sl) {
   const int lane = threadIdx.x & 63;
   const long row = (long)blockIdx.x * 4 + (threadIdx.x >> 6);
   if (row >= rows) return;
   if (limit != nullptr && row >= (long)*limit) return;
-  unsigned am = 0u;
+  unsigned am = 0u, am_c = 0u;
   const int W4 = W >> 2;
   float4 v[4];
   float s = 0.f;
@@ -531,8 +533,18 @@
   for (int q = 0; q < 4; ++q) {
     int i = lane + q * 64;
     v[q] = make_float4(0, 0, 0, 0);
-    if (i < W4) { v[q] = ld4(X + row * W + i * 4); s += v[q].x + v[q].y + v[q].z + v[q].w; }
-  }
+    if (i < W4) {
+      if (SLABS) {
+        v[q] = slab_row4(sl, row, i * 4);
+        st4(sl.C + row * W + i * 4, v[q]);
+        am_c = max(am_c, abits4(v[q]));
+      } else {
+        v[q] = ld4(X + row * W + i * 4);
+      }
+      s += v[q].x + v[q].y + v[q].z + v[q].w;
+    }
+  }
+  if (SLABS && sl.amax != nullptr) amax_commit(am_c, sl.amax);
   float mean = wave_sum(s) / (float)W;
   float s2 = 0.f;
 #pragma unroll
@@ -561,14 +573,15 @@
   if (lane == 0 && mean_out) { mean_out[row] = mean; rstd_out[row] = rstd; }
 }
 
+template <bool SLABS>
 __global__ __launch_bounds__(256) void layernorm_bwd_kernel(const float* __restrict__ dY, const float* __restrict__ X,
                                                             const float* __restrict__ gamma,
                                                             const float* __restrict__ mean_in,
                                                             const float* __restrict__ rstd_in, float* __restrict__ dX,
                                                             float* __restrict__ part, long rows, int W,
                                                             long rows_per_block, const float* __restrict__ extra,
-                                                            unsigned* __restrict__ amax = nullptr) {
-  unsigned am = 0u;
+                                                            unsigned* __restrict__ amax, const TrisSlabIn sl) {
+  unsigned am = 0u, am_dy = 0u;
   __shared__ float4 lg[4][256];
   __shared__ float4 lb[4][256];
   const int lane = threadIdx.x & 63, wv = threadIdx.x >> 6;
@@ -586,7 +599,9 @@
       int i = lane + q * 64;
       xh[q] = dh[q] = make_float4(0, 0, 0, 0);
       if (i < W4) {
-        float4 x = ld4(X + row * W + i * 4), dy = ld4(dY + row * W + i * 4), g = ld4(gamma + i * 4);
+        float4 x = ld4(X + row * W + i * 4), dy, g = ld4(gamma + i * 4);
+        if (SLABS) { dy = slab_row4(sl, row, i * 4); am_dy = max(am_dy, abits4(dy)); }
+        else dy = ld4(dY + row * W + i * 4);
         xh[q] = make_float4((x.x - mean) * rstd, (x.y - mean) * rstd, (x.z - mean) * rstd, (x.w - mean) * rstd);
         dh[q] = make_float4(dy.x * g.x, dy.y * g.y, dy.z * g.z, dy.w * g.w);
         c1 += dh[q].x + dh[q].y + dh[q].z + dh[q].w;
@@ -618,6 +633,7 @@
     }
   }
   if (amax != nullptr) amax_commit_block(am, amax);
+  if (SLABS && sl.amax != nullptr) amax_commit(am_dy, sl.amax);
   if (!part) return;
 #pragma unroll
   for (int q = 0; q < 4; ++q) { lg[wv][lane + q * 64] = ag[q]; lb[wv][lane + q * 64] = ab[q]; }
@@ -1048,12 +1064,46 @@
   return 0;
 }
 
+extern "C" __attribute__((visibility("hidden"))) TrisSplitkDefer* tris_internal_splitk_defer();
+extern "C" __attribute__((visibility("hidden"))) void tris_internal_chain_fused();
+static bool defer_stray() {
+  TrisSplitkDefer* d = tris_internal_splitk_defer();
+  if (!d->pending) return false;
+  d->pending = 0;
+  return true;
+}
+static bool defer_take(const float* in, long rows, int W, void* stream, TrisSlabIn& sl) {
+  TrisSplitkDefer* d = tris_internal_splitk_defer();
+  if (!d->pending) return false;
+  d->pending = 0;
+  if (d->C != in || (long)d->M != rows || d->N != W || d->ldc != (long)W || d->stream != stream || d->S < 2) return false;
+  sl.ws = d->ws; sl.total = (long)d->M * d->N; sl.S = d->S; sl.N = d->N; sl.alpha = d->alpha; sl.bias = d->bias;
+  sl.bias_mode = d->bias_mode; sl.act = d->act; sl.resid = d->resid; sl.ldr = d->ldr; sl.C = d->C; sl.amax = d->amax;
+  return true;
+}
+
 extern "C" int tris_layernorm_fwd_f32(const float* X, const float* gamma, const float* beta, float* Y, float* mean,
                                       float* rstd, long rows, int W, float eps, void* stream) {
+  unsigned* amax = take_amax_next();
+  if (defer_stray()) return (int)hipErrorIllegalState;
   if (W % 4 || W > 1024) return (int)hipErrorInvalidValue;
-  hipLaunchKernelGGL(layernorm_fwd_kernel, dim3(cdiv(rows, 4)), dim3(256), 0, (hipStream_t)stream, X, gamma, beta, Y,
-                     mean, rstd, rows, W, eps, take_amax_next(), g_rows_limit);
-  TRIS_LAUNCH_CHECK();
+  hipLaunchKernelGGL(layernorm_fwd_kernel<false>, dim3(cdiv(rows, 4)), dim3(256), 0, (hipStream_t)stream, X, gamma, beta, Y,
+                     mean, rstd, rows, W, eps, amax, g_rows_limit, TrisSlabIn{});
+  TRIS_LAUNCH_CHECK();
+  return 0;
+}
+
+extern "C" int tris_layernorm_fwd_slabs_f32(float* X, const float* gamma, const float* beta, float* Y, float* mean, float* rstd,
+                                            long rows, int W, float eps, void* stream) {
+  unsigned* amax = take_amax_next();
+  TrisSlabIn sl = {};
+  const int* lim = tris_internal_splitk_defer()->m_limit;
+  if (!defer_take(X, rows, W, stream, sl) || lim != g_rows_limit) return (int)hipErrorIllegalState;
+  if (W % 4 || W > 1024) return (int)hipErrorInvalidValue;
+  hipLaunchKernelGGL(layernorm_fwd_kernel<true>, dim3(cdiv(rows, 4)), dim3(256), 0, (hipStream_t)stream, (const float*)nullptr, gamma,
+                     beta, Y, mean, rstd, rows, W, eps, amax, g_rows_limit, sl);
+  TRIS_LAUNCH_CHECK();
+  tris_internal_chain_fused();
   return 0;
 }
 
@@ -1071,22 +1121,46 @@
   return nb * 2 * W * (long)sizeof(float);
 }
 
-extern "C" int tris_layernorm_bwd_f32(const float* dY, const float* X, const float* gamma, const float* mean,
-                                      const float* rstd, float* dX, float* dgamma, float* dbeta, long rows, int W,
-                                      float* workspace, const float* extra, void* stream) {
+static int ln_bwd_launch(const float* dY, const float* X, const float* gamma, const float* mean, const float* rstd, float* dX,
+                         float* dgamma, float* dbeta, long rows, int W, float* workspace, const float* extra, void* stream, bool slabs) {
+  unsigned* amax = take_amax_next();
+  TrisSlabIn sl = {};
+  if (slabs) {
+    if (!defer_take(dY, rows, W, stream, sl)) return (int)hipErrorIllegalState;
+    workspace = const_cast<float*>(sl.ws) + (long)sl.S * sl.total;
+  } else if (defer_stray()) {
+    return (int)hipErrorIllegalState;
+  }
   if (W % 4 || W > 1024) return (int)hipErrorInvalidValue;
   hipStream_t st = (hipStream_t)stream;
   const long rpb = ln_bwd_rpb(rows);
   int nb = (int)((rows + rpb - 1) / rpb);
   float* part = dgamma ? workspace : nullptr;
-  hipLaunchKernelGGL(layernorm_bwd_kernel, dim3(nb), dim3(256), 0, st, dY, X, gamma, mean, rstd, dX, part, rows, W,
-                     rpb, extra, take_amax_next());
+  if (slabs)
+    hipLaunchKernelGGL(layernorm_bwd_kernel<true>, dim3(nb), dim3(256), 0, st, (const float*)nullptr, X, gamma, mean, rstd, dX, part, rows,
+                       W, rpb, extra, amax, sl);
+  else
+    hipLaunchKernelGGL(layernorm_bwd_kernel<false>, dim3(nb), dim3(256), 0, st, dY, X, gamma, mean, rstd, dX, part, rows, W, rpb, extra,
+                       amax, sl);
   TRIS_LAUNCH_CHECK();
   if (dgamma) {
     hipLaunchKernelGGL(part_finalize_kernel<float>, dim3(fin_grid(W, nb)), dim3(fin_block(nb)), 0, st, (const float*)workspace, nb, W, dgamma, dbeta);
     TRIS_LAUNCH_CHECK();
   }
-  return 0;
+  if (slabs) tris_internal_chain_fused();
+  return 0;
+}
+
+extern "C" int tris_layernorm_bwd_f32(const float* dY, const float* X, const float* gamma, const float* mean,
+                                      const float* rstd, float* dX, float* dgamma, float* dbeta, long rows, int W,
+                                      float* workspace, const float* extra, void* stream) {
+  return ln_bwd_launch(dY, X, gamma, mean, rstd, dX, dgamma, dbeta, rows, W, workspace, extra, stream, false);
+}
+
+extern "C" int tris_layernorm_bwd_slabs_f32(const float* dY, const float* X, const float* gamma, const float* mean, const float* rstd,
+                                            float* dX, float* dgamma, float* dbeta, long rows, int W, const float* extra,
+                                            void* stream) {
+  return ln_bwd_launch(dY, X, gamma, mean, rstd, dX, dgamma, dbeta, rows, W, nullptr, extra, stream, true);
 }
 
 extern "C" int tris_avgpool2_fwd_f32(const float* X, float* Y, int B, int H, int W, int C, void* stream) {
diff --git a/tris_amd/csrc/splitk_defer.h b/tris_amd/csrc/splitk_defer.h
--- /dev/null
+++ b/tris_amd/csrc/splitk_defer.h
@@ -0,0 +1,69 @@
+#pragma once
+
+struct TrisSplitkDefer {
+  int armed;
+  int pending;
+  const float* ws;
+  long ws_bytes;
+  int S, M, N;
+  long ldc;
+  float alpha;
+  const float* bias;
+  int bias_mode, act;
+  const float* resid;
+  long ldr;
+  float* C;
+  unsigned* amax;
+  const int* m_limit;
+  void* stream;
+};
+
+struct TrisSlabIn {
+  const float* ws;
+  long total;
+  int S, N;
+  float alpha;
+  const float* bias;
+  int bias_mode, act;
+  const float* resid;
+  long ldr;
+  float* C;
+  unsigned* amax;
+};
+
+#ifdef __HIPCC__
+__device__ __forceinline__ float4 slab_row4(const TrisSlabIn& p, long row, int col0) {
+  const long idx = row * p.N + col0;
+  const long total = p.total;
+  const float* ws = p.ws;
+  const int S = p.S;
+  float v[4];
+#pragma unroll
+  for (int t = 0; t < 4; ++t) v[t] = 0.f;
+  int s = 0;
+  for (; s + 3 < S; s += 4) {
+    const float4 a = *reinterpret_cast<const float4*>(ws + (long)s * total + idx), b = *reinterpret_cast<const float4*>(ws + (long)(s + 1) * total + idx);
+    const float4 c = *reinterpret_cast<const float4*>(ws + (long)(s + 2) * total + idx), d = *reinterpret_cast<const float4*>(ws + (long)(s + 3) * total + idx);
+    v[0] = (((v[0] + a.x) + b.x) + c.x) + d.x;
+    v[1] = (((v[1] + a.y) + b.y) + c.y) + d.y;
+    v[2] = (((v[2] + a.z) + b.z) + c.z) + d.z;
+    v[3] = (((v[3] + a.w) + b.w) + c.w) + d.w;
+  }
+  for (; s < S; ++s) {
+    const float4 a = *reinterpret_cast<const float4*>(ws + (long)s * total + idx);
+    v[0] += a.x; v[1] += a.y; v[2] += a.z; v[3] += a.w;
+  }
+#pragma unroll
+  for (int t = 0; t < 4; ++t) {
+    const int col = col0 + t;
+    float x = v[t] * p.alpha;
+    if (p.bias_mode == 1) x += p.bias[col];
+    else if (p.bias_mode == 2) x += p.bias[row];
+    if (p.act == 1) x = fmaxf(x, 0.f);
+    else if (p.act == 2) x = x / (1.0f + expf(-1.702f * x));
+    if (p.resid) x += p.resid[row * p.ldr + col];
+    v[t] = x;
+  }
+  return make_float4(v[0], v[1], v[2], v[3]);
+}
+#endif
diff --git a/tris_amd/ops.py b/tris_amd/ops.py
--- a/tris_amd/ops.py
+++ b/tris_amd/ops.py
@@ -396,7 +396,7 @@
 
 
 def gemm(A, B, C, M, N, K, lda, ldb, ldc, tA, tB, batch=1, sA=0, sB=0, sC=0, bias=None, bias_mode=0, resid=None,
-         ldr=0, sR=0, act=0, alpha=1.0, use_ws=True, pre_out=None, dact=None, w_a=False, w_b=False, w_bt=False, mark=True):
+         ldr=0, sR=0, act=0, alpha=1.0, use_ws=True, pre_out=None, dact=None, w_a=False, w_b=False, w_bt=False, mark=True, defer=False):
     _chk(A, B, C, bias, resid)
     if pre_out is not None or dact is not None or batch != 1 or _BATCH_INVARIANT:
         A, B = unplanes(A), unplanes(B)
@@ -440,12 +440,17 @@
         tk = splitk_tickets()
         if tk is not None:
             call("tris_splitk_tickets_next", tk.data_ptr(), tk.numel())
+    defer = bool(defer and ws is not None and cfg.chain_fuse)
+    if defer:
+        call("tris_splitk_defer_next", 1)
     _timed("gemm", 2.0 * M * N * K * batch, lambda: call(
         "tris_gemm_f32", pA, pB, P(C), M, N, K, lda, ldb, ldc, int(tA), int(tB), batch, sA, sB, sC, P(bias),
         bias_mode, P(resid), ldr, sR, act, float(alpha), P(ws), 0 if ws is None else ws.numel() * 4, _stream()),
         tag=(f"{'T' if tA else 'N'}{'T' if tB else 'N'} M{M} N{N} K{K} b{batch}" if _PROF_SHAPES else None),
         nbytes=4.0 * ((M * K if (sA == 0 and batch > 1) else batch * M * K) + batch * K * N
                       + batch * M * N * (2 if resid is not None else 1)))
+    if defer:
+        _lib.DEFER.deferred = query("tris_splitk_deferred")
     return C
 
 
@@ -1006,8 +1011,9 @@
 
     @staticmethod
     def forward(ctx, x, w, b, resid, act, stats=False, grad_box=None, grad_box_out=None, grad_box_res=None, bn_link=None,
-                act_link=None):
+                act_link=None, ln_in=False):
         _chk(x, w, b, resid)
+        ctx.ln_in = ln_in
         ctx.grad_box, ctx.grad_box_out, ctx.grad_box_res = grad_box, grad_box_out, grad_box_res
         ctx.act_link = act_link
         ctx.bn_link = bn_link if (bn_link is not None and x.is_contiguous() and bn_link.x.shape == x.shape) else None
@@ -1063,6 +1069,22 @@
             box.consumed = True
             if box.value is not None:
                 extra, box.value = box.value, None
+
+        def param_grads():
+            dw = None
+            if ctx.needs_input_grad[1]:
+                if _sink(pw) is not None:
+                    on_wgrad_stream(lambda: gemm(dy, x, _sink(pw), N, K, M, N, K, K, True, False, mark=False), dy, x, sink=_sink(pw))
+                else:
+                    dw = _emit(pw, lambda o: gemm(dy, x, o, N, K, M, N, K, K, True, False, mark=False), True)
+            db = None
+            if ctx.has_b:
+                db = _emit(pb, lambda o: colsum(dy, M, N, o), ctx.needs_input_grad[2], reads=(dy,))
+            return dw, db
+        defer = bool(ctx.ln_in and cfg.chain_fuse and ctx.needs_input_grad[0] and ctx.bn_link is None and ctx.act_link is None
+                     and ctx.grad_box_out is None and pl_word(dy) is None)
+        if defer:
+            dw, db = param_grads()
         if ctx.needs_input_grad[0]:
             dx = torch.empty_like(x)
             link, fused = ctx.bn_link, False
@@ -1095,21 +1117,14 @@
                 if gemm(dy, w, dx, M, K, N, N, K, K, False, False, dact=alink.pre) is not False:
                     fused = alink.applied = True
             if not fused:
-                gemm(dy, w, dx, M, K, N, N, K, K, False, False, resid=extra, ldr=K, w_b=True, w_bt=True)
+                gemm(dy, w, dx, M, K, N, N, K, K, False, False, resid=extra, ldr=K, w_b=True, w_bt=True, defer=defer)
         elif extra is not None:
             raise RuntimeError("a residual gradient was handed to a layer whose input needs no gradient")
         if dx is not None and ctx.grad_box_out is not None and ctx.grad_box_out.deposit(dx):
             dx = None
-        dw = None
-        if ctx.needs_input_grad[1]:
-            if _sink(pw) is not None:
-                on_wgrad_stream(lambda: gemm(dy, x, _sink(pw), N, K, M, N, K, K, True, False, mark=False), dy, x, sink=_sink(pw))
-            else:
-                dw = _emit(pw, lambda o: gemm(dy, x, o, N, K, M, N, K, K, True, False, mark=False), True)
-        db = None
-        if ctx.has_b:
-            db = _emit(pb, lambda o: colsum(dy, M, N, o), ctx.needs_input_grad[2], reads=(dy,))
-        return dx, dw, db, d_res, None, None, None, None, None, None, None
+        if not defer:
+            dw, db = param_grads()
+        return dx, dw, db, d_res, None, None, None, None, None, None, None, None
 
 
 def linear(x, w, b=None, resid=None, act=0, stats=False, grad_box=None, grad_box_out=None, grad_box_res=None, act_link=False):
@@ -1117,7 +1132,7 @@
     if link is not None and not (torch.is_grad_enabled() and x.requires_grad and _bn_bwd_fuse_enabled()):
         link = None
     alink = getattr(x, "_act_link", None) if (act_link and torch.is_grad_enabled() and x.requires_grad) else None
-    return LinearFn.apply(x, w, b, resid, act, stats, grad_box, grad_box_out, grad_box_res, link, alink)
+    return LinearFn.apply(x, w, b, resid, act, stats, grad_box, grad_box_out, grad_box_res, link, alink, getattr(x, "_ln_sole", False))
 
 
 class _ActLink:
@@ -1130,8 +1145,9 @@
 class LinearQGeluFn(torch.autograd.Function):
 
     @staticmethod
-    def forward(ctx, x, w, b):
+    def forward(ctx, x, w, b, ln_in=False):
         _chk(x, w, b)
+        ctx.ln_in = ln_in
         x = x.contiguous()
         K = x.shape[-1]
         N = w.numel() // K
@@ -1153,24 +1169,32 @@
         M, N, K = ctx.dims
         dy = dy.contiguous()
         dpre = dy if ctx.link.applied else ew("TRIS_EW_QGELU_BWD", dy, pre)
+
+        def param_grads():
+            dw = None
+            if ctx.needs_input_grad[1]:
+                if _sink(pw) is not None:
+                    on_wgrad_stream(lambda: gemm(dpre, x, _sink(pw), N, K, M, N, K, K, True, False, mark=False), dpre, x, sink=_sink(pw))
+                else:
+                    dw = _emit(pw, lambda o: gemm(dpre, x, o, N, K, M, N, K, K, True, False, mark=False), True)
+            db = None
+            if ctx.has_b:
+                db = _emit(pb, lambda o: colsum(dpre, M, N, o), ctx.needs_input_grad[2], reads=(dpre,))
+            return dw, db
+        defer = bool(ctx.ln_in and cfg.chain_fuse and ctx.needs_input_grad[0])
+        if defer:
+            dw, db = param_grads()
         dx = None
         if ctx.needs_input_grad[0]:
             dx = torch.empty_like(x)
-            gemm(dpre, w, dx, M, K, N, N, K, K, False, False)
-        dw = None
-        if ctx.needs_input_grad[1]:
-            if _sink(pw) is not None:
-                on_wgrad_stream(lambda: gemm(dpre, x, _sink(pw), N, K, M, N, K, K, True, False, mark=False), dpre, x, sink=_sink(pw))
-            else:
-                dw = _emit(pw, lambda o: gemm(dpre, x, o, N, K, M, N, K, K, True, False, mark=False), True)
-        db = None
-        if ctx.has_b:
-            db = _emit(pb, lambda o: colsum(dpre, M, N, o), ctx.needs_input_grad[2], reads=(dpre,))
-        return dx, dw, db
+            gemm(dpre, w, dx, M, K, N, N, K, K, False, False, defer=defer)
+        if not defer:
+            dw, db = param_grads()
+        return dx, dw, db, None
 
 
 def linear_qgelu(x, w, b=None):
-    return LinearQGeluFn.apply(x, w, b)
+    return LinearQGeluFn.apply(x, w, b, getattr(x, "_ln_sole", False))
 
 
 class MatmulFn(torch.autograd.Function):
@@ -1724,6 +1748,9 @@
     def backward(ctx, dy):
         x, g, b, st = ctx.saved_tensors
         rows, W = ctx.dims
+        slabs = getattr(_lib.DEFER, "deferred", 0) != 0
+        if slabs and (dy.data_ptr() != _lib.DEFER.deferred or not dy.is_contiguous()):
+            _lib.defer_fail("a LayerNorm backward over another gradient tensor")
         dy = dy.contiguous()
         dx = torch.empty_like(x) if ctx.needs_input_grad[0] else None
         box, extra = ctx.grad_box, None
@@ -1736,15 +1763,17 @@
         need_p = ctx.needs_input_grad[1] or ctx.needs_input_grad[2]
         ws = workspace(query("tris_layernorm_bwd_workspace_bytes", rows, W))
         sg, sb = _sink(ctx.params[0]), _sink(ctx.params[1])
+        def launch(pdg, pdb):
+            h2_mark_next(dx)
+            if slabs:
+                call("tris_layernorm_bwd_slabs_f32", P(dy), P(x), P(g), P(st), P(st, rows), P(dx), pdg, pdb, rows, W, P(extra), _stream())
+            else:
+                call("tris_layernorm_bwd_f32", P(dy), P(x), P(g), P(st), P(st, rows), P(dx), pdg, pdb, rows, W, P(ws), P(extra), _stream())
         if need_p and sg is not None and sb is not None and sg.is_contiguous() and sb.is_contiguous():
-            h2_mark_next(dx)
-            call("tris_layernorm_bwd_f32", P(dy), P(x), P(g), P(st), P(st, rows), P(dx), P(sg), P(sb), rows, W, P(ws),
-                 P(extra), _stream())
+            launch(P(sg), P(sb))
             return dx, None, None, None, None
         dgb = torch.empty(2, W, device=x.device, dtype=torch.float32) if need_p else None
-        h2_mark_next(dx)
-        call("tris_layernorm_bwd_f32", P(dy), P(x), P(g), P(st), P(st, rows), P(dx), P(dgb), P(dgb, W),
-             rows, W, P(ws), P(extra), _stream())
+        launch(P(dgb), P(dgb, W))
         dg = _emit(ctx.params[0], lambda o: o.copy_(dgb[0]), ctx.needs_input_grad[1])
         db = _emit(ctx.params[1], lambda o: o.copy_(dgb[1]), ctx.needs_input_grad[2])
         return dx, dg, db, None, None
@@ -1752,6 +1781,12 @@
 
 def layer_norm(x, g, b, eps=1e-5, grad_box=None):
     return LayerNormFn.apply(x, g, b, eps, grad_box)
+
+
+def ln_sole(h):
+    if cfg.chain_fuse and torch.is_grad_enabled() and h.requires_grad:
+        h._ln_sole = True
+    return h
 
 
 class MhaFn(torch.autograd.Function):
@@ -1819,6 +1854,8 @@
             w_qkv, w_do = _h2_amax(qkv), _h2_amax(do)
         h2_mark_next(dqkv)
         if w_qkv is not None and w_do is not None:
+            if not cfg.chain_fuse:
+                call("tris_mha_h2_bwd_split_next")
             call("tris_mha_h2_bwd_f32", P(qkv), P(out), P(do), P(lse), P(delta), P(dqkv), w_qkv, w_do, N, L, W, heads, causal, _stream())
         else:
             call("tris_mha_mfma_bwd_f32", P(qkv), P(out), P(do), P(lse), P(delta), P(dqkv), N, L, W, heads, causal, _stream())
```

Result: no change. 1369 img/s, median of 6 (+0.7%).
